# TigreGotico/phoonnx

Hardware: AMD Instinct MI355X
Metric: audio samples/sec (22.05 kHz), batch-32 256-phoneme utterances (higher is better)
Workload: dtype f32 (f16x3 split: fp32 operands as two fp16 planes, three MFMA products, fp32 accumulate)

## Files before the change

include/vitsmi.h:

```cpp
#ifndef VITSMI_H
#define VITSMI_H

#include <stddef.h>
#include <stdint.h>

#ifdef __cplusplus
extern "C" {
#endif

typedef struct vits_handle vits_handle;

enum {
    VITS_OK = 0,
    VITS_E_IO = -1,
    VITS_E_FORMAT = -2,
    VITS_E_ARG = -3,
    VITS_E_DEVICE = -4,
    VITS_E_NOMEM = -5,
    VITS_E_RANGE = -6
};

#define VITS_MAX_DIMS 4


// ... 309 lines not shown
                                 const vits_noise *noise, const vits_controls *ctl, const vits_stream_format *fmt,
                                 const vits_stream_shaping *shaping, const vits_stream_onset *onsets, int chunk_frames,
                                 vits_enc_chunk_trim_fn fn, void *user);
int vits_run_vocoder_chunked_enc_trimmed(vits_handle *h, const float *z, int B, int F, const int64_t *sid,
                                         const vits_stream_format *fmt, const vits_stream_shaping *shaping,
                                         const vits_stream_onset *onsets, int chunk_frames, vits_enc_chunk_trim_fn fn, void *user);

int vits_warp_emit_end(const vits_warp_seg *segs, int n_segs, int64_t n_in, int64_t n_out, int64_t X, int64_t *ready);
int vits_glide_emit_end(const vits_glide_seg *segs, int n_segs, int64_t n_in, int64_t n_out, int64_t X, int64_t *ready);
int64_t vits_warp_stream_cap(int64_t piece_samples, int64_t S_w);
int vits_run_chunked_glided(vits_handle *h, const int64_t *ids, const int64_t *lens, int B, int T, const int64_t *sid,
                            const vits_noise *noise, const vits_controls *ctl, const vits_contour *contour, int chunk_frames,
                            vits_chunk_fn fn, void *user);
int vits_run_chunked_enc_glided(vits_handle *h, const int64_t *ids, const int64_t *lens, int B, int T, const int64_t *sid,
                                const vits_noise *noise, const vits_controls *ctl, const vits_stream_format *fmt,
                                const vits_stream_shaping *shaping, const vits_stream_onset *onsets, const vits_contour *contour,
                                int chunk_frames, vits_enc_chunk_trim_fn fn, void *user);

enum { VITS_FIT_MET = 0, VITS_FIT_FLOOR = 1, VITS_FIT_CEIL = 2, VITS_FIT_KEPT = 3 };
typedef struct {
    const int32_t *group;
    int n_groups;
    const int64_t *target_frames;
    const int32_t *mode;
} vits_fit;
int vits_fit_plan(const float *w, const int64_t *lens, int B, int T, const vits_fit *fit, int64_t *durations, double *scale,
                  int64_t *frames, int32_t *status);
int vits_run_async_fitted(vits_handle *h, const int64_t *ids, const int64_t *lens, int B, int T, const int64_t *sid,
                          const vits_noise *noise, const vits_controls *ctl, const vits_fit *fit);
int vits_run_chunked_fitted(vits_handle *h, const int64_t *ids, const int64_t *lens, int B, int T, const int64_t *sid,
                            const vits_noise *noise, const vits_controls *ctl, const vits_fit *fit, int chunk_frames,
                            vits_chunk_fn fn, void *user);
int vits_run_chunked_enc_fitted(vits_handle *h, const int64_t *ids, const int64_t *lens, int B, int T, const int64_t *sid,
                                const vits_noise *noise, const vits_controls *ctl, const vits_stream_format *fmt,
                                const vits_stream_shaping *shaping, const vits_stream_onset *onsets, const vits_fit *fit,
                                int chunk_frames, vits_enc_chunk_trim_fn fn, void *user);
int vits_last_fit(vits_handle *h, double *scale, int64_t *frames, int32_t *status, int n);

int vits_reserve(vits_handle *h, int B, int T, int F);
int vits_get_stats(vits_handle *h, vits_stats *out);

typedef struct {
    char kernel[128];
    double flops, bytes;
    float ms;
    int stage;
    int cin, cout, k, dil, t;
} vits_launch_record;
int vits_launch_records(vits_handle *h, vits_launch_record *buf, int n);

void *vits_stream(vits_handle *h);


int vits_test_conv1d(int device_id, const float *x, int B, int Cin, int T, const float *w, const float *bias,
                     int Cout, int K, int dil, int pad_l, int flags, float slope, float *out);
int vits_bench_conv1d(int device_id, int B, int Cin, int Cout, int T, int K, int dil, int hint, int iters,
                      int cfg_override, int ck_override, float *ms_out);
int vits_test_conv_transpose1d(int device_id, const float *x, int B, int Cin, int T, const float *w,
                               const float *bias, int Cout, int K, int stride, float *out);
enum {
    VITS_CONV_PRO_LRELU = 1, VITS_CONV_PRO_MASK = 2, VITS_CONV_EPI_RELU = 4, VITS_CONV_EPI_MASK = 8, VITS_CONV_EPI_RES = 16,
    VITS_CONV_EPI_ACC = 32, VITS_CONV_EPI_DIV = 64, VITS_CONV_EPI_COUPLING = 128, VITS_CONV_EPI_WN = 256,
    VITS_CONV_EPI_WN_FIRST = 512
};
typedef struct {
    int B, Cin, T, Cout;
    int K, dil, pad_l;
    int stride;
    int hint, cfg, ck;
    int flags;
    float slope, div, oslope, oslope2;
    int wn_split;
    const float *x;
    const float *w, *bias;
    const int64_t *lens;
    const float *bias_b;
    int bias_b_stride;
    const float *res;
    int x_cstride;
    int out_cstride;
    int out_rows, out_row0;
    const float *old_out, *old_out2;
    float sentinel;
    float *out, *out2;
    int pl_rows;
    float *planes_out;
    char kernel[128];
    int cfg_used, ck_used;
} vits_test_conv_epi_args;
int vits_test_conv1d_epi(int device_id, vits_test_conv_epi_args *a);
int vits_test_wn_gate(int device_id, const float *a, int B, int H, int T, int form, float *acts);
int vits_test_cond_matvec(int device_id, const float *emb_g, int n_speakers, int gin, const int64_t *sid, int B,
                          const float *W, const float *bias, int rows, float *out);
int vits_test_conv1d_sx(int device_id, const float *x, int B, int Cin, int T, const float *w, const float *bias,
                        int Cout, int K, int dil, int pad_l, int flags, float slope, float *out);
enum { VITS_SX_EPI_RES = 1, VITS_SX_EPI_ACC = 2, VITS_SX_EPI_DIV = 4, VITS_SX_EPI_NO_RAW_STORE = 8 };
enum { VITS_SX_BF16X6 = 0, VITS_SX_F16X3 = 1, VITS_SX_F16 = 2 };
typedef struct {
    int B, Cin, T, Cout;
    int K, dil, pad_l;
    int stride;
    int precision;
    int force16, no_s16, min_cfg;
    int run_cfg;
    int flags;
    const float *x;
    const float *w, *bias;
    const float *res;
    int res_is_x;
    int res_planes;
    float res_slope;
    const float *old_out;
    const float *bias_b;
    int bias_b_stride;
    float div, oslope, oslope2, islope;
    const int64_t *lens;
    int rag_add, rag_mul;
    float sentinel;
    float *out;
    float *planes_out;
    float *res_seen;
    char kernel[128];
    int pack_cfg, run_cfg_used, rawin, s16, ck;
    float peak;
} vits_test_conv_sx_epi_args;
int vits_test_conv1d_sx_epi(int device_id, vits_test_conv_sx_epi_args *a);
int vits_test_conv1d_sx_planar(int device_id, const float *x, int B, int Cin, int T, const float *w, const float *bias,
                               int Cout, int K, int dil, int flags, const int64_t *lens, const float *old, int row_split,
                               int pl_rows, float *out, float *planes_out);
long long vits_test_set_sx_small_max(long long wgs);
int vits_test_conv1d_sx_gate(int device_id, const float *x, int B, int Cin, int T, const float *w, const float *bias,
                             const float *bias_b, int Cout, int K, int dil, int flags, float *out);
int vits_test_conv_transpose1d_sx(int device_id, const float *x, int B, int Cin, int T, const float *w,
                                  const float *bias, int Cout, int K, int stride, float *out);
int vits_bench_conv1d_sx(int device_id, int B, int Cin, int Cout, int T, int K, int dil, int dbg, int iters,
                         float *ms_out);
int vits_test_conv_pair_sx(int device_id, const float *x, int B, int C, int T, const float *w1, const float *b1,
                           const float *w2, const float *b2, int K, int dil1, int dil2, int chain, float slope, float *out,
                           float *ms_out);
enum { VITS_PAIR_EPI_ACC = 1, VITS_PAIR_EPI_DIV = 2 };
typedef struct {
    int B, C, T, K, dil1, dil2, chain;
    int flags;
    float slope, div;
    const float *x;
    const float *w1, *b1, *w2, *b2;
    const int64_t *lens;
    const float *out_init;
    float *out;
    char kernel[128];
    int BNo;
} vits_test_conv_pair_sx_epi_args;
int vits_test_conv_pair_sx_epi(int device_id, vits_test_conv_pair_sx_epi_args *a);
int vits_test_split_identity(const float *x, int64_t n, uint16_t *h1_old, uint16_t *h1_fused);
int64_t vits_test_split_identity_sweep(uint32_t first, uint64_t count, uint32_t *first_bad);
int vits_test_split_forms(int device_id, const float *x, int n, float slope, int form, uint16_t *h0, uint16_t *h1, float *pk,
                          float *rec);
enum { VITS_P16_EPI_ACC = 1, VITS_P16_EPI_DIV = 2, VITS_P16_EPI_RAW = 4, VITS_P16_EPI_PLANES = 8 };
typedef struct {
    int B, C, T, K, dil1, dil2, chain;
    int precision;
    int flags;
    float slope, div, sentinel;
    const float *x;
    const float *w1, *b1, *w2, *b2;
    const float *old_out;
    const float *x_tail;
    const int64_t *lens;
    int rag_add, rag_mul;
    float *out;
    float *planes_out;
    float *x_seen;
    float *ms_out;
    char kernel[128];
    int BN, BNo, ovl;
    float peak;
    int guard_ok;
} vits_test_conv_pair16_epi_args;
int vits_test_conv_pair16_epi(int device_id, vits_test_conv_pair16_epi_args *a);
int vits_test_attention(int device_id, const float *qkv, int B, int C, int T, int n_heads, const float *rel_k,
                        const float *rel_v, int window, const int64_t *lens, float *out);
int vits_test_attention16(int device_id, const float *qkv, int B, int C, int T, int n_heads, const float *rel_k,
                          const float *rel_v, int window, const int64_t *lens, float *out, uint16_t *out_planes, int kernel,
                          int reps, float *ms_out);
typedef struct {
    int kernel;
    const float *qkv;
    const uint16_t *qkv_planes;
    int B, C, T, n_heads, window;
    const float *rel_k, *rel_v;
    const int64_t *lens;
    int want_out;
    int want_planes;
    int ns, qt;
    int kh;
    float *out;
    uint16_t *out_planes;
    float peak;
    char kernel_name[128];
} vits_test_attention_form_args;
int vits_test_attention_form(int device_id, vits_test_attention_form_args *a);

int vits_test_resample(int device_id, const float *x, const int64_t *lens, int B, int S, int in_rate, int out_rate, float *y,
                       int64_t S_out);
int vits_test_resample_pieces(int device_id, const float *x, const int64_t *lens, int B, int S, int in_rate, int out_rate,
                              int piece_samples, float *y, int64_t S_out, int64_t *ranges, int max_ranges);
int vits_test_resample_rows(int device_id, const float *x, const int64_t *lens, int B, int S, int in_rate,
                            const int32_t *out_rates, float *y, size_t y_elems, int64_t *n_out);
int vits_test_warp(int device_id, const float *x, const int64_t *counts, int B, int S, const vits_warp_seg *segs,
                   const int32_t *seg_first , float *y, int S_w);
int vits_test_glide(int device_id, const float *x, const int64_t *counts, int B, int S, const vits_glide_seg *segs,
                    const int32_t *seg_first , float *y, int S_w);
int vits_test_warp_pieces(int device_id, const float *x, const int64_t *counts, int B, int S, const vits_warp_seg *segs,
                          const int32_t *seg_first , const int64_t *piece_bounds, int n_pieces, float *y, int S_w,
                          int64_t *ranges, int max_ranges);
int vits_test_glide_pieces(int device_id, const float *x, const int64_t *counts, int B, int S, const vits_glide_seg *segs,
                           const int32_t *seg_first , const int64_t *piece_bounds, int n_pieces, float *y, int S_w,
                           int64_t *ranges, int max_ranges);
int vits_test_warp_rate(int device_id, const float *x, const int64_t *counts, int B, int S, const vits_warp_seg *segs,
                        const int32_t *seg_first , const int32_t *in_rates, const int32_t *out_rates, int n_lo, int n_hi,
                        float *y);
int vits_test_glide_rate(int device_id, const float *x, const int64_t *counts, int B, int S, const vits_glide_seg *segs,
                         const int32_t *seg_first , const int32_t *in_rates, const int32_t *out_rates, int n_lo, int n_hi,
                        float *y);

int vits_test_warp_rate_pieces(int device_id, const float *x, const int64_t *counts, int B, int S, const vits_warp_seg *segs,
                               const int32_t *seg_first , int in_rate, int out_rate, const int64_t *piece_bounds,
                               int n_pieces, float *y, int S_w, int64_t *ranges, int max_ranges);
int vits_test_glide_rate_pieces(int device_id, const float *x, const int64_t *counts, int B, int S, const vits_glide_seg *segs,
                                const int32_t *seg_first , int in_rate, int out_rate, const int64_t *piece_bounds,
                                int n_pieces, float *y, int S_w, int64_t *ranges, int max_ranges);

int vits_test_durations(int device_id, const float *logw, const int64_t *dur, const int64_t *lens, int B, int T, float length_scale,
                        const float *rows, const float *token_rate, float *w_ceil, int32_t *cum, int32_t *y_len);
int vits_test_fit_durations(int device_id, const float *w, const int64_t *lens, int B, int T, const vits_fit *fit, float *w_ceil,
                            int32_t *cum, int32_t *y_len, double *scale, int64_t *frames, int32_t *status);
int vits_test_expand_prior(int device_id, const float *m_logs, int B, int C, int T, const int32_t *cum, const int64_t *lens,
                           const int32_t *y_len, int F, const float *noise, int64_t noise_stride, int noise_frames,
                           float noise_scale, const float *rows, const uint64_t *seeds, float *z_p);
int vits_test_fill_normal(int device_id, int64_t n, uint64_t seed, uint64_t stream_id, float *out);
int vits_test_fill_normal_rows(int device_id, int B, int channels, int T, const uint64_t *seeds, uint32_t stream, const float *rows,
                               int col, float *out);
int vits_test_post_conv(int device_id, const float *x, int B, int C, int T, const float *w, int K, float slope, const int64_t *vlen,
                        int hop, int kernel, float *out);

int vits_test_layernorm(int device_id, const float *x, const float *out_init, int B, int C, int T, const float *gamma,
                        const float *beta, const int64_t *lens, int flags, int form, int in_place, const float *dw_w,
                        const float *dw_b, int K, int dil, float *out, uint16_t *planes);
typedef struct vits_test_dds_layer {
    const float *dw_w, *dw_b;
    const float *ln1_g, *ln1_b;
    const float *pw_w, *pw_b;
    const float *ln2_g, *ln2_b;
    int32_t dil;
} vits_test_dds_layer;
int vits_test_dds(int device_id, int form, const float *x, int B, int C, int T, const int64_t *lens, int n_layers,
                  const vits_test_dds_layer *layers, int mask_out, const float *head_cond, const float *head_z, int head_ch,
                  const float *head_w, const float *head_b, const float *tail_w, const float *tail_b, int tail_rows, float *out);
int vits_test_cf_pre(int device_id, const float *z, int ch, const float *w, const float *bias, const float *cond, int B, int C, int T,
                     float *out);
int vits_test_rqs_inverse(int device_id, const float *pr, const float *z, int B, int T, const int64_t *lens, int ch0, int nb,
                          float sqrt_c, float *out);
int vits_test_ea_logw(int device_id, const float *z, int ch, float m0, float logs0, const int64_t *lens, int B, int T, float *out);

int vits_test_deliver(int device_id, const float *x, const int64_t *counts, int B, int S, const vits_segment *segs, int n_segs,
                      int n_streams, int encoding, void *dst, size_t dst_bytes, int64_t *stream_samples, int64_t *stream_offsets);

int vits_test_deliver_trimmed(int device_id, const float *x, const int64_t *counts, int B, int S, const vits_segment *segs,
                              const vits_trim *trims, int n_segs, int n_streams, int encoding, void *dst, size_t dst_bytes,
                              int64_t *stream_samples, int64_t *stream_offsets, int64_t *kept_first, int64_t *kept_count);

int vits_test_loudness_blocks(int device_id, const float *x, const int64_t *counts, const int64_t *firsts, int B, int S,
                              int sample_rate, float *e, size_t e_cap, int32_t *n_sub, int32_t *chunk);

int vits_test_deliver_leveled(int device_id, const float *x, const int64_t *counts, int B, int S, const vits_segment *segs,
                              const vits_trim *trims, const vits_level *levels, int n_segs, int n_streams, int encoding,
                              int sample_rate, void *dst, size_t dst_bytes, int64_t *stream_samples, int64_t *stream_offsets,
                              int64_t *kept_first, int64_t *kept_count, double *loudness, float *gain);

int vits_test_deliver_shaped(int device_id, const float *x, const int64_t *counts, int B, int S, const vits_segment *segs,
                             const vits_trim *trims, const vits_level *levels, const vits_shape *shapes, const vits_env_point *points,
                             int64_t n_points, int n_segs, int n_streams, int encoding, int sample_rate, void *dst, size_t dst_bytes,
                             int64_t *stream_samples, int64_t *stream_offsets, int64_t *kept_first, int64_t *kept_count,
                             double *loudness, float *gain);

int vits_test_deliver_limited(int device_id, const float *x, const int64_t *counts, int B, int S, const vits_segment *segs,
                              const vits_trim *trims, const vits_level *levels, const vits_shape *shapes, const vits_env_point *points,
                              int64_t n_points, const vits_limit *limits, int n_segs, int n_streams, int encoding, int sample_rate,
                              void *dst, size_t dst_bytes, int64_t *stream_samples, int64_t *stream_offsets, int64_t *kept_first,
                              int64_t *kept_count, double *loudness, float *gain);

int vits_test_stream_pack(int device_id, const float *x, const int64_t *counts, int B, int S, int piece_samples,
                          const vits_stream_format *fmt, void *bytes, size_t bytes_cap, int64_t *pitches, int32_t *valid,
                          float *peaks, int max_pieces);

int vits_test_stream_pack_shaped(int device_id, const float *x, const int64_t *counts, int B, int S, int piece_samples,
                                 const vits_stream_format *fmt, const vits_stream_shaping *shaping, void *bytes, size_t bytes_cap,
                                 int64_t *pitches, int32_t *valid, float *peaks, int64_t *firsts, int64_t *ns, int max_pieces);

int vits_test_stream_pack_trimmed(int device_id, const float *x, const int64_t *counts, int B, int S, int piece_samples,
                                  const vits_stream_format *fmt, const vits_stream_shaping *shaping, const vits_stream_onset *onsets,
                                  void *bytes, size_t bytes_cap, int64_t *pitches, int32_t *valid, int32_t *skip, float *peaks,
                                  int64_t *firsts, int64_t *ns, int32_t *start, int max_pieces);

#ifdef __cplusplus
}
// ... 3 lines not shown
```

phoonnx_amd/_ffi.py:

```python
import ctypes as C
import os

import numpy as np

from . import audio_encoding

_HERE = os.path.dirname(os.path.abspath(__file__))
_LIB = None

VITS_MAX_DIMS = 4


class VitsNoise(C.Structure):
    _fields_ = [("noise_dp", C.c_void_p), ("noise_z", C.c_void_p), ("noise_z_stride", C.c_int64),
                ("seed", C.c_uint64)]


class VitsOutput(C.Structure):
    _fields_ = [("data", C.POINTER(C.c_float)), ("dims", C.c_int64 * 4), ("y_lengths", C.POINTER(C.c_int64))]


class VitsStats(C.Structure):
    _fields_ = [("conv_flops", C.c_double), ("conv_bytes", C.c_double), ("dec_flops", C.c_double),
                ("dec_bytes", C.c_double), ("flow_flops", C.c_double), ("enc_flops", C.c_double),
                ("dp_flops", C.c_double), ("conv_ms", C.c_float), ("dec_ms", C.c_float), ("flow_ms", C.c_float),
                ("enc_ms", C.c_float), ("dp_ms", C.c_float), ("total_ms", C.c_float), ("conv_launches", C.c_int),
                ("total_launches", C.c_int), ("sx_flops", C.c_double), ("sx_ms", C.c_float), ("sx_launches", C.c_int),
                ("f16_peak_max", C.c_float), ("f16_peak_min", C.c_float), ("f16_tracked", C.c_int),
                ("f16_saturated", C.c_int), ("sx_bytes", C.c_double)]


class VitsLaunchRecord(C.Structure):
    _fields_ = [("kernel", C.c_char * 128), ("flops", C.c_double), ("bytes", C.c_double), ("ms", C.c_float),
                ("stage", C.c_int), ("cin", C.c_int), ("cout", C.c_int), ("k", C.c_int), ("dil", C.c_int), ("t", C.c_int)]


class VitsTestConvEpiArgs(C.Structure):
    _fields_ = [(n, C.c_int) for n in ("B", "Cin", "T", "Cout", "K", "dil", "pad_l", "stride", "hint", "cfg", "ck", "flags")] + \
               [(n, C.c_float) for n in ("slope", "div", "oslope", "oslope2")] + [("wn_split", C.c_int)] + \
               [(n, C.c_void_p) for n in ("x", "w", "bias", "lens", "bias_b")] + [("bias_b_stride", C.c_int), ("res", C.c_void_p)] + \
               [(n, C.c_int) for n in ("x_cstride", "out_cstride", "out_rows", "out_row0")] + \
               [("old_out", C.c_void_p), ("old_out2", C.c_void_p), ("sentinel", C.c_float), ("out", C.c_void_p), ("out2", C.c_void_p),
                ("pl_rows", C.c_int), ("planes_out", C.c_void_p), ("kernel", C.c_char * 128), ("cfg_used", C.c_int), ("ck_used", C.c_int)]


class VitsTestConvSxEpiArgs(C.Structure):
    _fields_ = [(n, C.c_int) for n in ("B", "Cin", "T", "Cout", "K", "dil", "pad_l", "stride", "precision", "force16", "no_s16",
                                       "min_cfg", "run_cfg", "flags")] + \
               [(n, C.c_void_p) for n in ("x", "w", "bias", "res")] + \
               [("res_is_x", C.c_int), ("res_planes", C.c_int), ("res_slope", C.c_float), ("old_out", C.c_void_p),
                ("bias_b", C.c_void_p), ("bias_b_stride", C.c_int)] + \
               [(n, C.c_float) for n in ("div", "oslope", "oslope2", "islope")] + \
               [("lens", C.c_void_p), ("rag_add", C.c_int), ("rag_mul", C.c_int), ("sentinel", C.c_float), ("out", C.c_void_p),
                ("planes_out", C.c_void_p), ("res_seen", C.c_void_p), ("kernel", C.c_char * 128)] + \
               [(n, C.c_int) for n in ("pack_cfg", "run_cfg_used", "rawin", "s16", "ck")] + [("peak", C.c_float)]


class VitsTestConvPair16EpiArgs(C.Structure):
    _fields_ = [(n, C.c_int) for n in ("B", "C", "T", "K", "dil1", "dil2", "chain", "precision", "flags")] + \
               [(n, C.c_float) for n in ("slope", "div", "sentinel")] + \
               [(n, C.c_void_p) for n in ("x", "w1", "b1", "w2", "b2", "old_out", "x_tail", "lens")] + \
               [("rag_add", C.c_int), ("rag_mul", C.c_int)] + \
               [(n, C.c_void_p) for n in ("out", "planes_out", "x_seen", "ms_out")] + [("kernel", C.c_char * 128)] + \
               [(n, C.c_int) for n in ("BN", "BNo", "ovl")] + [("peak", C.c_float), ("guard_ok", C.c_int)]


class VitsTestConvPairSxEpiArgs(C.Structure):
    _fields_ = [(n, C.c_int) for n in ("B", "C", "T", "K", "dil1", "dil2", "chain", "flags")] + \
               [(n, C.c_float) for n in ("slope", "div")] + \
               [(n, C.c_void_p) for n in ("x", "w1", "b1", "w2", "b2", "lens", "out_init", "out")] + \
               [("kernel", C.c_char * 128), ("BNo", C.c_int)]


class VitsTestAttentionFormArgs(C.Structure):
    _fields_ = [("kernel", C.c_int), ("qkv", C.c_void_p), ("qkv_planes", C.c_void_p)] + \
               [(n, C.c_int) for n in ("B", "C", "T", "n_heads", "window")] + \
               [(n, C.c_void_p) for n in ("rel_k", "rel_v", "lens")] + \
               [(n, C.c_int) for n in ("want_out", "want_planes", "ns", "qt", "kh")] + \
               [("out", C.c_void_p), ("out_planes", C.c_void_p), ("peak", C.c_float), ("kernel_name", C.c_char * 128)]


class VitsOpenOptions(C.Structure):
    _fields_ = [("device_id", C.c_int), ("gen_precision", C.c_char_p), ("arena_dev", C.c_void_p),
                ("arena_bytes", C.c_size_t), ("host_only", C.c_int), ("layout_only", C.c_int)]


class VitsControls(C.Structure):
    _fields_ = [("scales_rows", C.c_void_p), ("seeds", C.c_void_p), ("durations", C.c_void_p), ("token_rate", C.c_void_p)]


class VitsFit(C.Structure):
    _fields_ = [("group", C.c_void_p), ("n_groups", C.c_int), ("target_frames", C.c_void_p), ("mode", C.c_void_p)]


VITS_FIT_MET, VITS_FIT_FLOOR, VITS_FIT_CEIL, VITS_FIT_KEPT = 0, 1, 2, 3


class VitsWarpSeg(C.Structure):
    _fields_ = [("n0", C.c_int64), ("pos0", C.c_int64), ("k", C.c_int64), ("step", C.c_int32), ("c", C.c_int32),
                ("half_taps", C.c_int32), ("pad_", C.c_int32)]


class VitsIntonation(C.Structure):
    _fields_ = [("token_semitones", C.c_void_p), ("compensate", C.c_int)]


class VitsGlideSeg(C.Structure):
    _fields_ = [("n0", C.c_int64), ("pos0", C.c_int64), ("k", C.c_int64), ("step0", C.c_int32), ("step1", C.c_int32),
                ("pad_", C.c_int32 * 2)]


class VitsContour(C.Structure):
    _fields_ = [("token_semitones", C.c_void_p), ("token_semitones_end", C.c_void_p), ("compensate", C.c_int)]


class VitsSegment(C.Structure):
    _fields_ = [("row", C.c_int32), ("stream", C.c_int32), ("lead_samples", C.c_int64), ("normalize", C.c_int32),
                ("volume", C.c_float)]


class VitsTrim(C.Structure):
    _fields_ = [("mode", C.c_int32), ("threshold", C.c_float), ("keep_lead", C.c_int32), ("keep_tail", C.c_int32),
                ("tail_samples", C.c_int64)]


class VitsTestDdsLayer(C.Structure):
    _fields_ = [("dw_w", C.c_void_p), ("dw_b", C.c_void_p), ("ln1_g", C.c_void_p), ("ln1_b", C.c_void_p), ("pw_w", C.c_void_p),
                ("pw_b", C.c_void_p), ("ln2_g", C.c_void_p), ("ln2_b", C.c_void_p), ("dil", C.c_int32)]


class VitsLevel(C.Structure):
    _fields_ = [("mode", C.c_int32), ("target_lufs", C.c_float), ("max_gain_db", C.c_float), ("peak_ceiling", C.c_float)]


class VitsEnvPoint(C.Structure):
    _fields_ = [("pos", C.c_int32), ("gain", C.c_float)]


class VitsShape(C.Structure):
    _fields_ = [("fade_in", C.c_int32), ("fade_out", C.c_int32), ("curve", C.c_int32), ("n_points", C.c_int32),
                ("first_point", C.c_int64)]


class VitsLimit(C.Structure):
    _fields_ = [("mode", C.c_int32), ("ceiling", C.c_float), ("lookahead", C.c_int32), ("reserved", C.c_int32)]


class VitsStreamFormat(C.Structure):
    _fields_ = [("encoding", C.c_int32), ("ref_peak", C.c_void_p), ("volume", C.c_void_p)]


class VitsStreamShaping(C.Structure):
    pass


STREAM_PLAN_FN = C.CFUNCTYPE(C.c_int, C.c_void_p, C.c_int, C.c_int, C.POINTER(C.c_int64), C.POINTER(C.c_int64), C.POINTER(VitsStreamShaping))

VitsStreamShaping._fields_ = [("shapes", C.c_void_p), ("points", C.c_void_p), ("n_points", C.c_int64), ("ceiling", C.c_void_p),
                              ("lookahead", C.c_int32), ("reserved", C.c_int32), ("plan", STREAM_PLAN_FN), ("plan_user", C.c_void_p)]


class VitsStreamOnset(C.Structure):
    _fields_ = [("mode", C.c_int32), ("threshold", C.c_float), ("keep_lead", C.c_int32), ("reserved", C.c_int32)]


ENCODINGS = {name: (code, audio_encoding.DTYPES[name]) for code, name in enumerate(audio_encoding.ENCODINGS)}


CHUNK_FN = C.CFUNCTYPE(C.c_int, C.c_void_p, C.POINTER(C.c_float), C.c_int, C.c_int64, C.c_int64, C.c_int64)

ENC_CHUNK_FN = C.CFUNCTYPE(C.c_int, C.c_void_p, C.c_void_p, C.c_int, C.c_int64, C.c_int64, C.c_int64, C.POINTER(C.c_int32),
                           C.POINTER(C.c_float), C.c_int64)

ENC_CHUNK_TRIM_FN = C.CFUNCTYPE(C.c_int, C.c_void_p, C.c_void_p, C.c_int, C.c_int64, C.c_int64, C.c_int64, C.POINTER(C.c_int32),
                                C.POINTER(C.c_int32), C.POINTER(C.c_float), C.c_int64)

VITS_E_RANGE = -6


EXPORTS = [
    "vits_open", "vits_open_with_arena", "vits_open_host", "vits_open_layout", "vits_open_opts", "vits_close",
    "vits_run_chunked", "vits_run_vocoder_chunked", "vits_last_error", "vits_num_inputs",
    "vits_input_name", "vits_meta", "vits_hparam", "vits_arena_bytes", "vits_arena_host", "vits_arena_device",
    "vits_run", "vits_free_output", "vits_run_device", "vits_sync", "vits_last_y_lengths", "vits_last_pcm16", "vits_run_vocoder",
    "vits_tap",
    "vits_set_timing", "vits_set_tails", "vits_reserve", "vits_get_stats", "vits_stream", "vits_test_conv1d", "vits_test_conv_transpose1d",
    "vits_test_attention", "vits_test_attention16", "vits_bench_conv1d", "vits_test_conv1d_sx", "vits_test_conv1d_sx_planar", "vits_test_conv1d_sx_gate", "vits_test_set_sx_small_max",
    "vits_test_conv_transpose1d_sx",
    "vits_bench_conv1d_sx", "vits_test_conv_pair_sx", "vits_fetch_output", "vits_run_async", "vits_host_alloc", "vits_host_free",
    "vits_launch_records", "vits_run_async_rows", "vits_run_device_rows", "vits_run_chunked_rows",
    "vits_run_async_ctl", "vits_run_chunked_ctl", "vits_last_durations",
    "vits_set_output_rate", "vits_last_sample_counts", "vits_resample_plan", "vits_test_resample", "vits_test_resample_pieces",
    "vits_set_output_rates", "vits_last_sample_rates", "vits_test_resample_rows",
    "vits_run_async_warped", "vits_last_token_spans", "vits_warp_token", "vits_warp_plan", "vits_test_warp",
    "vits_run_async_glided", "vits_glide_token", "vits_glide_cutoff", "vits_glide_plan", "vits_test_glide",
    "vits_warp_emit_end", "vits_glide_emit_end", "vits_warp_stream_cap", "vits_run_chunked_glided", "vits_run_chunked_enc_glided",
    "vits_test_warp_pieces", "vits_test_glide_pieces",
    "vits_set_pitch_at_rate", "vits_warp_token_rate", "vits_warp_plan_rate", "vits_glide_plan_rate", "vits_glide_cutoff_rate", "vits_glide_pos_rate",
    "vits_rate_identity_spans", "vits_test_warp_rate", "vits_test_glide_rate",
    "vits_warp_emit_end_rate", "vits_glide_emit_end_rate", "vits_identity_emit_end_rate", "vits_warp_stream_cap_rate",
    "vits_test_warp_rate_pieces", "vits_test_glide_rate_pieces",
    "vits_fit_plan", "vits_run_async_fitted", "vits_run_chunked_fitted", "vits_run_chunked_enc_fitted", "vits_last_fit",
    "vits_test_fit_durations",
    "vits_test_durations", "vits_test_expand_prior", "vits_test_fill_normal", "vits_test_fill_normal_rows", "vits_test_post_conv",
    "vits_delivery_plan", "vits_deliver", "vits_test_deliver",
    "vits_trim_range", "vits_delivery_plan_trimmed", "vits_deliver_trimmed", "vits_test_deliver_trimmed",
    "vits_loudness_filter", "vits_loudness_gate", "vits_level_gain", "vits_delivery_plan_leveled", "vits_deliver_leveled",
    "vits_test_loudness_blocks", "vits_test_deliver_leveled",
    "vits_shape_check", "vits_shape_gain", "vits_deliver_shaped", "vits_test_deliver_shaped",
    "vits_limit_check", "vits_limit_gains", "vits_deliver_limited", "vits_test_deliver_limited",
    "vits_run_chunked_enc", "vits_run_vocoder_chunked_enc", "vits_test_stream_pack",
    "vits_stream_shaping_check", "vits_stream_emit_range", "vits_run_chunked_enc_shaped", "vits_run_vocoder_chunked_enc_shaped",
    "vits_test_stream_pack_shaped",
    "vits_stream_onset_check", "vits_stream_onset_start", "vits_run_chunked_enc_trimmed", "vits_run_vocoder_chunked_enc_trimmed",
    "vits_test_stream_pack_trimmed",
    "vits_test_layernorm", "vits_test_dds", "vits_test_cf_pre", "vits_test_rqs_inverse", "vits_test_ea_logw",
    "vits_test_conv1d_epi", "vits_test_wn_gate", "vits_test_cond_matvec", "vits_test_conv1d_sx_epi",
    "vits_test_conv_pair16_epi", "vits_test_attention_form", "vits_test_conv_pair_sx_epi", "vits_test_split_forms", "vits_test_split_identity", "vits_test_split_identity_sweep",
]


G2P_EXPORTS = ["g2p_open", "g2p_close", "g2p_last_error", "g2p_hparam", "g2p_num_outputs", "g2p_output_name", "g2p_bucket",
               "g2p_run", "g2p_generate", "g2p_generate_batch", "g2p_test_forced_steps", "g2p_test_linear", "g2p_test_step",
               "g2p_test_attention", "g2p_test_rmsnorm", "g2p_test_argmax"]


def lib_path():
    return os.environ.get("VITSMI_LIB") or os.path.join(_HERE, "libvitsmi.so")


def load():
    global _LIB
    if _LIB is not None:
        return _LIB
    path = lib_path()
    if not os.environ.get("VITSMI_LIB"):
        from . import build as _build
        if _build.stale():
            try:
                _build.build()
            except Exception as e:
                raise RuntimeError(f"{path} is missing or was not built from the sources in this tree (source_sha "
                                   f"{_build.source_sha()} vs recorded {_build.read_build_info().get('source_sha')}) "
                                   f"and cannot be rebuilt here: {e}") from e
    lib = C.CDLL(path)
    vp, i64p, f32p = C.c_void_p, C.POINTER(C.c_int64), C.POINTER(C.c_float)
    lib.vits_open.argtypes = [C.c_char_p, C.c_int, C.POINTER(vp)]
    lib.vits_open_with_arena.argtypes = [C.c_char_p, C.c_int, vp, C.c_size_t, C.POINTER(vp)]
    lib.vits_open_host.argtypes = [C.c_char_p, C.POINTER(vp)]
    lib.vits_open_layout.argtypes = [C.c_char_p, C.POINTER(vp)]
    lib.vits_open_opts.argtypes = [C.c_char_p, C.POINTER(VitsOpenOptions), C.POINTER(vp)]
    lib.vits_run_chunked.argtypes = [vp, vp, vp, C.c_int, C.c_int, vp, vp, C.POINTER(VitsNoise), C.c_int, CHUNK_FN, vp]
    lib.vits_run_vocoder_chunked.argtypes = [vp, vp, C.c_int, C.c_int, vp, C.c_int, CHUNK_FN, vp]
    lib.vits_close.argtypes = [vp]
    lib.vits_close.restype = None
    lib.vits_last_error.argtypes = [vp]
    lib.vits_last_error.restype = C.c_char_p
    lib.vits_num_inputs.argtypes = [vp]
    lib.vits_input_name.argtypes = [vp, C.c_int]
    lib.vits_input_name.restype = C.c_char_p
    lib.vits_meta.argtypes = [vp, C.c_char_p, C.c_char_p, C.c_size_t]
    lib.vits_hparam.argtypes = [vp, C.c_char_p, i64p]
    lib.vits_arena_bytes.argtypes = [vp]
    lib.vits_arena_bytes.restype = C.c_size_t
    lib.vits_arena_host.argtypes = [vp]
    lib.vits_arena_host.restype = vp
    lib.vits_arena_device.argtypes = [vp]
    lib.vits_arena_device.restype = vp
    run_args = [vp, vp, vp, C.c_int, C.c_int, vp, vp, C.POINTER(VitsNoise), C.POINTER(VitsOutput)]
    lib.vits_run.argtypes = run_args
    lib.vits_run_device.argtypes = run_args
    lib.vits_run_async.argtypes = run_args[:-1]
    lib.vits_run_async_rows.argtypes = run_args[:-1] + [vp]
    lib.vits_run_device_rows.argtypes = run_args[:-1] + [vp, C.POINTER(VitsOutput)]
    lib.vits_run_chunked_rows.argtypes = [vp, vp, vp, C.c_int, C.c_int, vp, vp, C.POINTER(VitsNoise), vp, C.c_int, CHUNK_FN, vp]
    lib.vits_run_async_ctl.argtypes = [vp, vp, vp, C.c_int, C.c_int, vp, C.POINTER(VitsNoise), C.POINTER(VitsControls)]
    lib.vits_run_chunked_ctl.argtypes = [vp, vp, vp, C.c_int, C.c_int, vp, C.POINTER(VitsNoise), C.POINTER(VitsControls),
                                         C.c_int, CHUNK_FN, vp]
    lib.vits_run_chunked_enc.argtypes = [vp, vp, vp, C.c_int, C.c_int, vp, C.POINTER(VitsNoise), C.POINTER(VitsControls),
                                         C.POINTER(VitsStreamFormat), C.c_int, ENC_CHUNK_FN, vp]
    lib.vits_run_vocoder_chunked_enc.argtypes = [vp, vp, C.c_int, C.c_int, vp, C.POINTER(VitsStreamFormat), C.c_int, ENC_CHUNK_FN, vp]
    lib.vits_stream_shaping_check.argtypes = [C.POINTER(VitsStreamShaping), C.POINTER(VitsStreamFormat), C.c_int]
    lib.vits_stream_emit_range.argtypes = [C.c_int64, C.c_int64, C.c_int, C.c_int64, C.c_int, i64p, i64p]
    lib.vits_run_chunked_enc_shaped.argtypes = [vp, vp, vp, C.c_int, C.c_int, vp, C.POINTER(VitsNoise), C.POINTER(VitsControls),
                                                C.POINTER(VitsStreamFormat), C.POINTER(VitsStreamShaping), C.c_int, ENC_CHUNK_FN, vp]
    lib.vits_run_vocoder_chunked_enc_shaped.argtypes = [vp, vp, C.c_int, C.c_int, vp, C.POINTER(VitsStreamFormat),
                                                        C.POINTER(VitsStreamShaping), C.c_int, ENC_CHUNK_FN, vp]
    lib.vits_test_stream_pack_shaped.argtypes = [C.c_int, vp, vp, C.c_int, C.c_int, C.c_int, C.POINTER(VitsStreamFormat),
                                                 C.POINTER(VitsStreamShaping), vp, C.c_size_t, vp, vp, vp, vp, vp, C.c_int]
    lib.vits_stream_onset_check.argtypes = [C.POINTER(VitsStreamOnset), C.POINTER(VitsStreamFormat), C.c_int]
    lib.vits_stream_onset_start.argtypes = [C.c_int64, C.c_int64, C.c_int64, i64p]
    lib.vits_run_chunked_enc_trimmed.argtypes = [vp, vp, vp, C.c_int, C.c_int, vp, C.POINTER(VitsNoise), C.POINTER(VitsControls),
                                                 C.POINTER(VitsStreamFormat), C.POINTER(VitsStreamShaping), C.POINTER(VitsStreamOnset),
                                                 C.c_int, ENC_CHUNK_TRIM_FN, vp]
    lib.vits_run_vocoder_chunked_enc_trimmed.argtypes = [vp, vp, C.c_int, C.c_int, vp, C.POINTER(VitsStreamFormat),
                                                         C.POINTER(VitsStreamShaping), C.POINTER(VitsStreamOnset), C.c_int,
                                                         ENC_CHUNK_TRIM_FN, vp]
    lib.vits_test_stream_pack_trimmed.argtypes = [C.c_int, vp, vp, C.c_int, C.c_int, C.c_int, C.POINTER(VitsStreamFormat),
                                                  C.POINTER(VitsStreamShaping), C.POINTER(VitsStreamOnset), vp, C.c_size_t, vp, vp, vp, vp,
                                                  vp, vp, vp, C.c_int]
    lib.vits_test_stream_pack.argtypes = [C.c_int, vp, vp, C.c_int, C.c_int, C.c_int, C.POINTER(VitsStreamFormat), vp, C.c_size_t,
                                          vp, vp, vp, C.c_int]
    lib.vits_last_durations.argtypes = [vp, i64p, C.c_size_t]
    lib.vits_set_output_rate.argtypes = [vp, C.c_int, C.c_int]
    lib.vits_last_sample_counts.argtypes = [vp, i64p, C.c_int]
    lib.vits_resample_plan.argtypes = [C.c_int, C.c_int, i64p, i64p, i64p, vp, C.c_size_t]
    lib.vits_test_resample.argtypes = [C.c_int, vp, vp, C.c_int, C.c_int, C.c_int, C.c_int, vp, C.c_int64]
    lib.vits_test_resample_pieces.argtypes = [C.c_int, vp, vp, C.c_int, C.c_int, C.c_int, C.c_int, C.c_int, vp, C.c_int64, vp, C.c_int]
    lib.vits_set_output_rates.argtypes = [vp, C.c_int, vp, C.c_int]
    lib.vits_last_sample_rates.argtypes = [vp, vp, C.c_int]
    lib.vits_test_resample_rows.argtypes = [C.c_int, vp, vp, C.c_int, C.c_int, C.c_int, vp, vp, C.c_size_t, vp]
    lib.vits_run_async_warped.argtypes = [vp, vp, vp, C.c_int, C.c_int, vp, C.POINTER(VitsNoise), C.POINTER(VitsControls),
                                          C.POINTER(VitsIntonation)]
    lib.vits_last_token_spans.argtypes = [vp, i64p, C.c_size_t]
    lib.vits_warp_token.argtypes = [C.c_float, i64p, i64p, C.POINTER(C.c_int32)]
    lib.vits_warp_plan.argtypes = [vp, vp, C.c_int, C.c_int, vp, vp, i64p]
    lib.vits_test_warp.argtypes = [C.c_int, vp, vp, C.c_int, C.c_int, vp, vp, vp, C.c_int]
    lib.vits_run_async_glided.argtypes = [vp, vp, vp, C.c_int, C.c_int, vp, C.POINTER(VitsNoise), C.POINTER(VitsControls),
                                          C.POINTER(VitsContour)]
    lib.vits_glide_token.argtypes = [C.c_float, C.c_float, i64p, i64p, C.POINTER(C.c_float)]
    lib.vits_glide_cutoff.argtypes = [C.c_int64, i64p, C.POINTER(C.c_int32)]
    lib.vits_glide_plan.argtypes = [vp, vp, vp, C.c_int, C.c_int, vp, vp, i64p]
    lib.vits_test_glide.argtypes = [C.c_int, vp, vp, C.c_int, C.c_int, vp, vp, vp, C.c_int]
    for name in ("vits_warp_emit_end", "vits_glide_emit_end"):
        getattr(lib, name).argtypes = [vp, C.c_int, C.c_int64, C.c_int64, C.c_int64, i64p]
    lib.vits_warp_stream_cap.argtypes = [C.c_int64, C.c_int64]
    lib.vits_warp_stream_cap.restype = C.c_int64
    lib.vits_run_chunked_glided.argtypes = [vp, vp, vp, C.c_int, C.c_int, vp, C.POINTER(VitsNoise), C.POINTER(VitsControls),
                                            C.POINTER(VitsContour), C.c_int, CHUNK_FN, vp]
    lib.vits_run_chunked_enc_glided.argtypes = [vp, vp, vp, C.c_int, C.c_int, vp, C.POINTER(VitsNoise), C.POINTER(VitsControls),
                                                C.POINTER(VitsStreamFormat), C.POINTER(VitsStreamShaping), C.POINTER(VitsStreamOnset),
                                                C.POINTER(VitsContour), C.c_int, ENC_CHUNK_TRIM_FN, vp]
    for name in ("vits_test_warp_pieces", "vits_test_glide_pieces"):
        getattr(lib, name).argtypes = [C.c_int, vp, vp, C.c_int, C.c_int, vp, vp, vp, C.c_int, vp, C.c_int, vp, C.c_int]
    lib.vits_set_pitch_at_rate.argtypes = [vp, C.c_int]
    lib.vits_warp_token_rate.argtypes = [C.c_float, C.c_int64, C.c_int64, i64p, i64p, C.POINTER(C.c_int32)]
    lib.vits_warp_plan_rate.argtypes = [vp, vp, C.c_int, C.c_int, C.c_int64, C.c_int64, vp, vp, i64p]
    lib.vits_glide_plan_rate.argtypes = [vp, vp, vp, C.c_int, C.c_int, C.c_int64, C.c_int64, vp, vp, i64p]
    lib.vits_glide_cutoff_rate.argtypes = [C.c_int64, i64p, C.POINTER(C.c_int32)]
    lib.vits_glide_pos_rate.argtypes = [vp, C.c_int64, i64p, i64p]
    lib.vits_rate_identity_spans.argtypes = [vp, C.c_int, C.c_int, C.c_int64, C.c_int64, C.c_int64, vp, i64p]
    for name in ("vits_warp_emit_end_rate", "vits_glide_emit_end_rate"):
        getattr(lib, name).argtypes = [vp, C.c_int, C.c_int64, C.c_int64, C.c_int64, C.c_int, i64p]
    lib.vits_identity_emit_end_rate.argtypes = [C.c_int64, C.c_int64, C.c_int64, C.c_int64, C.c_int64, i64p]
    lib.vits_warp_stream_cap_rate.argtypes = [C.c_int64, C.c_int64, C.c_int64, C.c_int]
    lib.vits_warp_stream_cap_rate.restype = C.c_int64
    for name in ("vits_test_warp_rate_pieces", "vits_test_glide_rate_pieces"):
        getattr(lib, name).argtypes = [C.c_int, vp, vp, C.c_int, C.c_int, vp, vp, C.c_int, C.c_int, vp, C.c_int, vp, C.c_int, vp, C.c_int]
    for name in ("vits_test_warp_rate", "vits_test_glide_rate"):
        getattr(lib, name).argtypes = [C.c_int, vp, vp, C.c_int, C.c_int, vp, vp, vp, vp, C.c_int, C.c_int, vp]
    lib.vits_fit_plan.argtypes = [vp, vp, C.c_int, C.c_int, C.POINTER(VitsFit), vp, vp, vp, vp]
    lib.vits_run_async_fitted.argtypes = [vp, vp, vp, C.c_int, C.c_int, vp, C.POINTER(VitsNoise), C.POINTER(VitsControls),
                                          C.POINTER(VitsFit)]
    lib.vits_run_chunked_fitted.argtypes = [vp, vp, vp, C.c_int, C.c_int, vp, C.POINTER(VitsNoise), C.POINTER(VitsControls),
                                            C.POINTER(VitsFit), C.c_int, CHUNK_FN, vp]
    lib.vits_run_chunked_enc_fitted.argtypes = [vp, vp, vp, C.c_int, C.c_int, vp, C.POINTER(VitsNoise), C.POINTER(VitsControls),
                                                C.POINTER(VitsStreamFormat), C.POINTER(VitsStreamShaping), C.POINTER(VitsStreamOnset),
                                                C.POINTER(VitsFit), C.c_int, ENC_CHUNK_TRIM_FN, vp]
    lib.vits_last_fit.argtypes = [vp, vp, vp, vp, C.c_int]
    lib.vits_test_fit_durations.argtypes = [C.c_int, vp, vp, C.c_int, C.c_int, C.POINTER(VitsFit), vp, vp, vp, vp, vp, vp]
    lib.vits_test_durations.argtypes = [C.c_int, vp, vp, vp, C.c_int, C.c_int, C.c_float, vp, vp, vp, vp, vp]
    lib.vits_test_expand_prior.argtypes = [C.c_int, vp, C.c_int, C.c_int, C.c_int, vp, vp, vp, C.c_int, vp, C.c_int64, C.c_int,
                                           C.c_float, vp, vp, vp]
    lib.vits_test_fill_normal.argtypes = [C.c_int, C.c_int64, C.c_uint64, C.c_uint64, vp]
    lib.vits_test_fill_normal_rows.argtypes = [C.c_int, C.c_int, C.c_int, C.c_int, vp, C.c_uint32, vp, C.c_int, vp]
    lib.vits_test_post_conv.argtypes = [C.c_int, vp, C.c_int, C.c_int, C.c_int, vp, C.c_int, C.c_float, vp, C.c_int, C.c_int, vp]
    lib.vits_test_layernorm.argtypes = [C.c_int, vp, vp, C.c_int, C.c_int, C.c_int, vp, vp, vp, C.c_int, C.c_int, C.c_int, vp, vp,
                                        C.c_int, C.c_int, vp, vp]
    lib.vits_test_dds.argtypes = [C.c_int, C.c_int, vp, C.c_int, C.c_int, C.c_int, vp, C.c_int, C.POINTER(VitsTestDdsLayer), C.c_int,
                                  vp, vp, C.c_int, vp, vp, vp, vp, C.c_int, vp]
    lib.vits_test_cf_pre.argtypes = [C.c_int, vp, C.c_int, vp, vp, vp, C.c_int, C.c_int, C.c_int, vp]
    lib.vits_test_rqs_inverse.argtypes = [C.c_int, vp, vp, C.c_int, C.c_int, vp, C.c_int, C.c_int, C.c_float, vp]
    lib.vits_test_ea_logw.argtypes = [C.c_int, vp, C.c_int, C.c_float, C.c_float, vp, C.c_int, C.c_int, vp]
    lib.vits_delivery_plan.argtypes = [vp, C.c_int, vp, C.c_int, C.c_int, C.c_int, vp, vp, i64p]
    lib.vits_deliver.argtypes = [vp, vp, C.c_int, C.c_int, C.c_int, vp, C.c_size_t, vp, vp]
    lib.vits_test_deliver.argtypes = [C.c_int, vp, vp, C.c_int, C.c_int, vp, C.c_int, C.c_int, C.c_int, vp, C.c_size_t, vp, vp]
    lib.vits_trim_range.argtypes = [C.c_int64, C.c_int64, C.c_int64, C.POINTER(VitsTrim), i64p, i64p]
    lib.vits_delivery_plan_trimmed.argtypes = [vp, C.c_int, vp, vp, C.c_int, C.c_int, C.c_int, vp, vp, i64p]
    lib.vits_deliver_trimmed.argtypes = [vp, vp, vp, C.c_int, C.c_int, C.c_int, vp, C.c_size_t, vp, vp, vp, vp]
    lib.vits_test_deliver_trimmed.argtypes = [C.c_int, vp, vp, C.c_int, C.c_int, vp, vp, C.c_int, C.c_int, C.c_int, vp, C.c_size_t,
                                              vp, vp, vp, vp]
    lib.vits_loudness_filter.argtypes = [C.c_int, vp, vp]
    lib.vits_loudness_gate.argtypes = [vp, vp, C.c_int, C.c_int32, vp, vp, vp, vp]
    lib.vits_level_gain.argtypes = [C.c_double, C.c_float, C.POINTER(VitsLevel), C.POINTER(C.c_float)]
    lib.vits_delivery_plan_leveled.argtypes = [vp, C.c_int, vp, vp, vp, C.c_int, C.c_int, C.c_int, C.c_int, vp, vp, i64p]
    lib.vits_deliver_leveled.argtypes = [vp, vp, vp, vp, C.c_int, C.c_int, C.c_int, C.c_int, vp, C.c_size_t, vp, vp, vp, vp, vp, vp]
    lib.vits_test_loudness_blocks.argtypes = [C.c_int, vp, vp, vp, C.c_int, C.c_int, C.c_int, vp, C.c_size_t, vp, vp]
    lib.vits_test_deliver_leveled.argtypes = [C.c_int, vp, vp, C.c_int, C.c_int, vp, vp, vp, C.c_int, C.c_int, C.c_int, C.c_int, vp,
                                              C.c_size_t, vp, vp, vp, vp, vp, vp]
    lib.vits_shape_check.argtypes = [vp, C.c_int, vp, C.c_int64]
    lib.vits_shape_gain.argtypes = [C.POINTER(VitsShape), vp, C.c_int64, C.c_int64, C.c_int64, C.POINTER(C.c_float)]
    lib.vits_deliver_shaped.argtypes = [vp, vp, vp, vp, vp, vp, C.c_int64, C.c_int, C.c_int, C.c_int, C.c_int, vp, C.c_size_t, vp, vp, vp,
                                        vp, vp, vp]
    lib.vits_test_deliver_shaped.argtypes = [C.c_int, vp, vp, C.c_int, C.c_int, vp, vp, vp, vp, vp, C.c_int64, C.c_int, C.c_int, C.c_int,
                                             C.c_int, vp, C.c_size_t, vp, vp, vp, vp, vp, vp]
    lib.vits_limit_check.argtypes = [vp, vp, C.c_int]
    lib.vits_limit_gains.argtypes = [vp, C.c_int64, C.POINTER(VitsLimit), vp]
    lib.vits_deliver_limited.argtypes = [vp, vp, vp, vp, vp, vp, C.c_int64, vp, C.c_int, C.c_int, C.c_int, C.c_int, vp, C.c_size_t, vp,
                                         vp, vp, vp, vp, vp]
    lib.vits_test_deliver_limited.argtypes = [C.c_int, vp, vp, C.c_int, C.c_int, vp, vp, vp, vp, vp, C.c_int64, vp, C.c_int, C.c_int,
                                              C.c_int, C.c_int, vp, C.c_size_t, vp, vp, vp, vp, vp, vp]
    lib.vits_free_output.argtypes = [vp, C.POINTER(VitsOutput)]
    lib.vits_free_output.restype = None
    lib.vits_sync.argtypes = [vp]
    lib.vits_last_y_lengths.argtypes = [vp, i64p, C.c_int]
    lib.vits_last_pcm16.argtypes = [vp, C.c_int, C.c_float, vp, C.c_size_t]
    lib.vits_run_vocoder.argtypes = [vp, vp, C.c_int, C.c_int, vp, C.POINTER(VitsOutput)]
    lib.vits_tap.argtypes = [vp, C.c_char_p, vp, C.c_size_t, i64p]
    lib.vits_set_timing.argtypes = [vp, C.c_int]
    lib.vits_set_tails.argtypes = [vp, C.c_int]
    lib.vits_reserve.argtypes = [vp, C.c_int, C.c_int, C.c_int]
    lib.vits_get_stats.argtypes = [vp, C.POINTER(VitsStats)]
    lib.vits_stream.argtypes = [vp]
    lib.vits_stream.restype = vp
    lib.vits_fetch_output.argtypes = [vp, vp, C.c_size_t, C.c_size_t]
    lib.vits_host_alloc.argtypes = [C.c_size_t]
    lib.vits_host_alloc.restype = vp
    lib.vits_host_free.argtypes = [vp]
    lib.vits_host_free.restype = None
    lib.vits_launch_records.argtypes = [vp, C.POINTER(VitsLaunchRecord), C.c_int]
    lib.vits_test_conv1d.argtypes = [C.c_int, vp, C.c_int, C.c_int, C.c_int, vp, vp, C.c_int, C.c_int, C.c_int,
                                     C.c_int, C.c_int, C.c_float, vp]
    lib.vits_test_conv_transpose1d.argtypes = [C.c_int, vp, C.c_int, C.c_int, C.c_int, vp, vp, C.c_int, C.c_int,
                                               C.c_int, vp]
    lib.vits_test_attention.argtypes = [C.c_int, vp, C.c_int, C.c_int, C.c_int, C.c_int, vp, vp, C.c_int, vp, vp]
    lib.vits_test_attention16.argtypes = [C.c_int, vp, C.c_int, C.c_int, C.c_int, C.c_int, vp, vp, C.c_int, vp, vp, vp,
                                          C.c_int, C.c_int, f32p]
    lib.vits_bench_conv1d.argtypes = [C.c_int] * 11 + [f32p]
    lib.vits_test_conv1d_sx.argtypes = lib.vits_test_conv1d.argtypes
    lib.vits_test_conv_transpose1d_sx.argtypes = lib.vits_test_conv_transpose1d.argtypes
    lib.vits_test_conv1d_sx_planar.argtypes = [C.c_int, vp, C.c_int, C.c_int, C.c_int, vp, vp, C.c_int, C.c_int, C.c_int, C.c_int,
                                               vp, vp, C.c_int, C.c_int, vp, vp]
    lib.vits_test_set_sx_small_max.argtypes = [C.c_longlong]
    lib.vits_test_set_sx_small_max.restype = C.c_longlong
    lib.vits_test_conv1d_sx_gate.argtypes = [C.c_int, vp, C.c_int, C.c_int, C.c_int, vp, vp, vp, C.c_int, C.c_int, C.c_int, C.c_int, vp]
    lib.vits_bench_conv1d_sx.argtypes = [C.c_int] * 9 + [f32p]
    lib.vits_test_conv1d_epi.argtypes = [C.c_int, C.POINTER(VitsTestConvEpiArgs)]
    lib.vits_test_conv1d_sx_epi.argtypes = [C.c_int, C.POINTER(VitsTestConvSxEpiArgs)]
    lib.vits_test_conv_pair16_epi.argtypes = [C.c_int, C.POINTER(VitsTestConvPair16EpiArgs)]
    lib.vits_test_conv_pair_sx_epi.argtypes = [C.c_int, C.POINTER(VitsTestConvPairSxEpiArgs)]
    lib.vits_test_split_identity.argtypes = [vp, C.c_int64, vp, vp]
    lib.vits_test_split_identity_sweep.argtypes = [C.c_uint32, C.c_uint64, C.POINTER(C.c_uint32)]
    lib.vits_test_split_identity_sweep.restype = C.c_int64
    lib.vits_test_split_forms.argtypes = [C.c_int, vp, C.c_int, C.c_float, C.c_int, vp, vp, vp, vp]
    lib.vits_test_attention_form.argtypes = [C.c_int, C.POINTER(VitsTestAttentionFormArgs)]
    lib.vits_test_wn_gate.argtypes = [C.c_int, vp, C.c_int, C.c_int, C.c_int, C.c_int, vp]
    lib.vits_test_cond_matvec.argtypes = [C.c_int, vp, C.c_int, C.c_int, vp, C.c_int, vp, vp, C.c_int, vp]
    lib.vits_test_conv_pair_sx.argtypes = [C.c_int, vp, C.c_int, C.c_int, C.c_int, vp, vp, vp, vp, C.c_int, C.c_int,
                                           C.c_int, C.c_int, C.c_float, vp, f32p]
    lib.g2p_open.argtypes = [C.c_char_p, C.c_int, C.POINTER(vp)]
    lib.g2p_close.argtypes = [vp]
    lib.g2p_close.restype = None
    lib.g2p_last_error.argtypes = [vp]
    lib.g2p_last_error.restype = C.c_char_p
    lib.g2p_hparam.argtypes = [vp, C.c_char_p, i64p]
    lib.g2p_num_outputs.argtypes = [vp]
    lib.g2p_output_name.argtypes = [vp, C.c_int]
    lib.g2p_output_name.restype = C.c_char_p
    lib.g2p_bucket.argtypes = [vp, C.c_int, C.c_int]
    lib.g2p_run.argtypes = [vp, vp, C.c_int, vp, vp, C.c_int, vp]
    lib.g2p_generate.argtypes = [vp, vp, C.c_int, C.c_int, C.c_int64, C.c_int64, vp, C.POINTER(C.c_int)]
    lib.g2p_generate_batch.argtypes = [vp, vp, vp, C.c_int, C.c_int, C.c_int64, C.c_int64, vp, vp]
    lib.g2p_test_forced_steps.argtypes = [vp, vp, vp, C.c_int, vp, C.c_int, vp]
    lib.g2p_test_linear.argtypes = [C.c_int, C.c_int, vp, vp, C.c_int, vp, C.c_int, C.c_int, vp, C.c_int64, C.c_int64, C.c_int, vp]
    lib.g2p_test_step.argtypes = [C.c_int, C.c_int, C.c_int, vp, vp, vp, C.c_int, vp, vp, C.c_int, C.c_float, C.c_float, vp, vp]
    lib.g2p_test_attention.argtypes = [C.c_int, vp, vp, C.c_int, C.c_int, vp, vp, C.c_int64, C.c_int, C.c_int64, vp, C.c_int, vp,
                                       C.c_int, C.c_int, C.c_int, C.c_int, vp, C.c_int, C.c_int, C.c_int]
    lib.g2p_test_rmsnorm.argtypes = [C.c_int, vp, vp, vp, C.c_int, C.c_int, C.c_int, C.c_int, C.c_float]
    lib.g2p_test_argmax.argtypes = [C.c_int, vp, C.c_int, C.c_int, C.c_int, C.c_int64, C.c_int, vp, vp, C.c_int64, C.c_int]
    _LIB = lib
    return lib


def ptr(a):
    return None if a is None else a.ctypes.data_as(C.c_void_p)


def last_error(h=None):
    return load().vits_last_error(h).decode("utf-8", "replace")
```

phoonnx_amd/csrc/conv_sx_pair.hip.hpp:

```cpp
#pragma once
#include <cstdlib>
#include "conv_geom.hpp"
#include "conv_sx_engine.hip.hpp"

namespace vitsmi {

struct SxPairArgs {
    const float *xr;
    float islope, mslope;
    int T;
    const u32x4 *wp1, *wp2;
    const float *bias1, *bias2;
    float wscale1, wscale2;
    float *out_raw;
    const float *zeros;
    int C, nchunks;
    int K1, dil1, pad1;
    int K2, dil2, pad2;
    int LW1;
    unsigned x_bytes;
    int LW2;
    unsigned y_chunk_bytes;
    int BNo, NT, B;
    int flags;
    float div;
    unsigned *peak;
    struct Chain {
        const u32x4 *wp1, *wp2;
        const float *bias1, *bias2;
        float wscale1, wscale2;
        int K1, dil1, K2, dil2;
        int xoff, yoff;
    } ch[3];
    int nchain;
    unsigned a_ring;
    unsigned bias_off;
    unsigned long long *prof;
    SxRagged rag;
    int xgs = 0;
};

#ifndef SX_PAIR_PROF
#define SX_PAIR_PROF 0
#endif
#ifndef SX_PAIR_SHARED_A
#define SX_PAIR_SHARED_A 0
#endif
#ifndef SX_PAIR_ALIAS
#define SX_PAIR_ALIAS 0
#endif
#ifndef SX_PAIR_DEPTH32
#define SX_PAIR_DEPTH32 2
#endif
#ifndef SX_PAIR_DEPTH64
#define SX_PAIR_DEPTH64 2
#endif
#ifndef SX_PAIR_EARLY_ACC
#define SX_PAIR_EARLY_ACC 0
#endif
#ifndef SX_PAIR_WGS32
#define SX_PAIR_WGS32 3
#endif
#ifndef SX_PAIR_EARLY32
#define SX_PAIR_EARLY32 1
#endif
#ifndef SX_PAIR_ST_SC1
#define SX_PAIR_ST_SC1 0
#endif
#ifndef SX_PAIR_INTERIOR
#define SX_PAIR_INTERIOR 1
#endif
#ifndef SX_PAIR_ONE_READ64
#define SX_PAIR_ONE_READ64 1
#endif
#ifndef SX_PAIR_ONE_READ32
#define SX_PAIR_ONE_READ32 1
#endif
template <int MW, int NW, int WM, int WN, int EPI, bool CHAIN, int NCH, bool INTR>
__device__ __forceinline__ void conv_sx_pair_body(const SxPairArgs &a, const int b, const int t0, const int TV, float &pk) {
    constexpr int BN = NW * WN * 32, NH = NW / 2;
    static_assert(NCH == 1 || (CHAIN && NW == 2 && (EPI & EPI_ACC) == 0), "fused chains: 32 channels, no external running sum");
    constexpr bool ONE_READ = NW == 4 ? SX_PAIR_ONE_READ64 != 0 : SX_PAIR_ONE_READ32 != 0;
    constexpr bool EARLY = ONE_READ || (NW == 2 && SX_PAIR_EARLY32);
    constexpr int DEPTH = NW == 2 ? SX_PAIR_DEPTH32 : SX_PAIR_DEPTH64;
    static_assert(DEPTH >= 2 && DEPTH <= 6, "wait_a covers up to five younger sets");
    constexpr bool ACC = (EPI & EPI_ACC) != 0 && SX_PAIR_EARLY_ACC;
    static_assert(!(ONE_READ && ACC), "the running sum is not pulled into the single-read prologue");
    static_assert(WM * WN == 4 && MW == 1 && BN == 256, "one block row per wave, 256 columns");
    constexpr int NPW = 2, STEPBYTES = WM * MW * NPW * 1024;
    constexpr int MAXCH = WM * 2;
    extern __shared__ __attribute__((aligned(16))) unsigned char lds_sx[];
    const int tid = threadIdx.x, lane = tid & 63;
    const int wave = __builtin_amdgcn_readfirstlane(tid >> 6);
    const int wm = wave / WN, wn = wave % WN;
    const int l31 = lane & 31, hi = lane >> 5;
    const int t1 = t0 - a.pad2;
    const int T = a.T, LW = a.LW1;
    const uint32_t lds0 = (uint32_t)(uintptr_t)lds_sx;
    const uint32_t XB = a.x_bytes;
    const char *wbase1 = reinterpret_cast<const char *>(a.wp1) + wm * (MW * NPW * 1024);
    const char *wbase2 = reinterpret_cast<const char *>(a.wp2) + wm * (MW * NPW * 1024);
    const float *xrb = a.xr + (int64_t)b * a.C * T;

    struct ASet {
        u32x4 fa[2];
    };
    const uint32_t voff0 = (uint32_t)lane * 16u;
    auto load_a = [&](ASet &f, const char *wb, int step) {
        const char *sb = wb + (int64_t)step * STEPBYTES;
        f.fa[0] = global_read128<0>(voff0, sb);
        f.fa[1] = global_read128<1024>(voff0, sb);
    };

    f32x4 pre[NW / 2][2][4], ad[EARLY && ACC ? NW / 2 : 1][2][4];
    auto load_res = [&](const float *base, f32x4 (*dst)[2][4]) {
        static_for<NW / 2>([&](auto R) {
            constexpr int rr = decltype(R)::value;
#pragma unroll
            for (int j = 0; j < 2; j++) {
                const int row0 = wm * 32;
                const int t = t1 + (wn * NW + rr * 2 + j) * 32 + l31;
                const int tl = t < 0 ? 0 : (t < T ? t : T - 1);
#pragma unroll
                for (int q = 0; q < 4; q++) {
                    if constexpr (INTR && EARLY) {
                        const char *rowb = reinterpret_cast<const char *>(base + (int64_t)((row0 >> 3) + q) * T * 8);
                        dst[rr][j][q] = __builtin_bit_cast(f32x4, global_read128<0>(((uint32_t)t * 8u + 4u * (uint32_t)hi) * 4u, rowb));
                        continue;
                    }
                    const float *p = base + ((int64_t)((row0 >> 3) + q) * T + tl) * 8 + 4 * hi;
                    if constexpr (EARLY) dst[rr][j][q] = __builtin_bit_cast(f32x4, global_read128_v<0>(p));
                    else dst[rr][j][q] = *reinterpret_cast<const f32x4 *>(p);
                }
            }
        });
    };
    auto load_pre = [&]() { load_res(xrb, pre); };

#if SX_PAIR_PROF
    auto stamp = [&]() {
        unsigned long long t;
        __builtin_amdgcn_sched_barrier(0);
        asm volatile("s_memtime %0\n\ts_waitcnt lgkmcnt(0)" : "=s"(t)::"memory");
        __builtin_amdgcn_sched_barrier(0);
        return t;
    };
    unsigned long long tp[8];
    tp[0] = stamp();
#endif
    if constexpr (NW == 2 && WM == 1 && NCH == 1 && SX_PAIR_SHARED_A != 0)
        for (int g = 0; g < 3; g++)
            if (g < ((a.nchunks * a.K1) >> 1)) {
                const int sub = wave >> 1, pl = wave & 1;
                lds_dma<16>(wbase1 + (int64_t)(2 * g + sub) * STEPBYTES + pl * 1024 + lane * 16,
                            reinterpret_cast<float *>(lds_sx + a.a_ring + (unsigned)((g * 2 + sub) * 2048 + pl * 1024)));
            }
    constexpr bool BIAS_LDS = NCH == 1;
    if constexpr (BIAS_LDS) {
        if (wave == 0) {
            constexpr int CC = WM * 32;
            const int k = lane - (lane >= CC / 4 ? CC / 4 : 0);
            const float *bp = lane < CC / 4 ? a.bias1 : a.bias2;
            const void *src = (bp && lane < CC / 2) ? static_cast<const void *>(bp + 4 * k) : static_cast<const void *>(a.zeros + 4 * (lane & 31));
            lds_dma<16>(src, reinterpret_cast<float *>(lds_sx + a.bias_off));
        }
    }
    auto bias_from_lds = [&](int conv, f32x4 (&bq)[4]) __attribute__((always_inline)) {
        u32x4 t4[4];
#pragma unroll
        for (int q = 0; q < 4; q++)
            asm volatile("ds_read_b128 %0, %1" : "=v"(t4[q]) : "v"(lds0 + a.bias_off + (uint32_t)(conv * (WM * 32) + wm * 32 + 8 * q + 4 * hi) * 4u) : "memory");
        asm volatile("s_waitcnt lgkmcnt(0)" ::: "memory");
        __builtin_amdgcn_sched_barrier(0);
#pragma unroll
        for (int q = 0; q < 4; q++) bq[q] = __builtin_bit_cast(f32x4, t4[q]);
    };
    constexpr int NXC = 3;
    if constexpr (ONE_READ) {
        constexpr int NXH = MAXCH, NG = 2 * MAXCH;
        const int HW = LW - 256, pad1 = a.pad1;
        const int nhc = HW * NG, nxh = (nhc + 255) >> 8;
        u32x4 hst[NXH][2];
        bool hin[NXH], hok[NXH];
        uint32_t hlds[NXH];
        const float *hp[NXH];
#pragma unroll
        for (int it = 0; it < NXH; it++) {
            const int h = it * 256 + tid;
            hin[it] = h < nhc;
            const int g = hin[it] ? h / HW : 0;
            const int c = hin[it] ? h - g * HW : 0;
            const int col = c < pad1 ? c : c + 256;
            const int t = t1 - pad1 + col;
            hok[it] = hin[it] && (INTR || (t >= 0 && t < TV));
            hp[it] = xrb + (hok[it] ? ((int64_t)g * T + t) * 8 : (int64_t)0);
            hlds[it] = lds0 + (uint32_t)(g >> 1) * XB + (uint32_t)((g & 1) * LW + col) * 16u;
        }
        static_for<NXH>([&](auto I) {
            constexpr int it = decltype(I)::value;
            if (it < nxh) {
                hst[it][0] = global_read128_v<0>(hp[it]);
                hst[it][1] = global_read128_v<16>(hp[it]);
            }
        });
        load_pre();
        const float isl = a.islope;
        static_for<NW>([&](auto N) {
            constexpr int n = decltype(N)::value;
            asm volatile("s_waitcnt vmcnt(%0)" ::"n"(4 * (NW - 1 - n)) : "memory");
            __builtin_amdgcn_sched_barrier(0);
#if SX_PAIR_PROF
            if constexpr (n == 0) tp[1] = stamp();
#endif
            if constexpr (n == 0) {
                static_for<NXH>([&](auto I) {
                    constexpr int it = decltype(I)::value;
                    if (it < nxh && hin[it]) {
                        float v[8];
#pragma unroll
                        for (int e = 0; e < 8; e++) {
                            const float x = (INTR || hok[it]) ? __uint_as_float(hst[it][e >> 2][e & 3]) : 0.f;
                            v[e] = lrelu_max(x, isl);
                        }
                        unsigned p0[4], p1[4];
#pragma unroll
                        for (int e = 0; e < 4; e++) sx_pair_split(v[2 * e], v[2 * e + 1], p0[e], p1[e], pk);
                        ds_write128(hlds[it], u32x4{p0[0], p0[1], p0[2], p0[3]});
                        ds_write128(hlds[it] + (uint32_t)(2 * LW) * 16u, u32x4{p1[0], p1[1], p1[2], p1[3]});
                    }
                });
            }
            const int col = (wn * NW + n) * 32 + l31;
            const int t = t1 + col;
            const bool ok = INTR || (t >= 0 && t < TV);
#pragma unroll
            for (int q = 0; q < 4; q++) {
                float v[4];
#pragma unroll
                for (int e = 0; e < 4; e++) {
                    const float x = ok ? pre[n / 2][n % 2][q][e] : 0.f;
                    v[e] = lrelu_max(x, isl);
                }
                unsigned wa[2], wb[2];
                sx_pair_split(v[0], v[1], wa[0], wa[1], pk);
                sx_pair_split(v[2], v[3], wb[0], wb[1], pk);
                const int g = 4 * wm + q;
                const uint32_t cell = lds0 + (uint32_t)(g >> 1) * XB + (uint32_t)((g & 1) * LW + pad1 + col) * 16u + 8u * hi;
                asm volatile("ds_write_b64 %0, %1" ::"v"(cell), "v"(u32x2{wa[0], wb[0]}) : "memory");
                asm volatile("ds_write_b64 %0, %1" ::"v"(cell + (uint32_t)(2 * LW) * 16u), "v"(u32x2{wa[1], wb[1]}) : "memory");
            }
            asm volatile("" : "+v"(pk));
        });
    } else {
        u32x4 xst[MAXCH][NXC][2];
        const int nxc = (2 * LW + 255) >> 8;
        uint32_t xroff[NXC];
        bool xrok[NXC];
        int xkh[NXC], xcol[NXC];
#pragma unroll
        for (int it = 0; it < NXC; it++) {
            const int i = it * 256 + tid;
            const int kh = (i >= LW ? 1 : 0) + (i >= 2 * LW ? 1 : 0);
            const int col = i - kh * LW;
            const int t = t1 - a.pad1 + col;
            xkh[it] = kh;
            xcol[it] = col;
            xrok[it] = it < nxc && kh < 2 && (INTR || (t >= 0 && t < TV));
            xroff[it] = xrok[it] ? (uint32_t)(((int64_t)kh * T + t) * 32) : 0u;
        }
        static_for<MAXCH>([&](auto CH) {
            constexpr int ch = decltype(CH)::value;
            const float *cbase = xrb + (int64_t)(2 * ch) * T * 8;
            static_for<NXC>([&](auto I) {
                constexpr int it = decltype(I)::value;
                if (it < nxc) {
                    xst[ch][it][0] = global_read128_x<0>(xroff[it], cbase);
                    xst[ch][it][1] = global_read128_x<16>(xroff[it], cbase);
                }
            });
        });
        if constexpr (EARLY) {
            load_pre();
            if constexpr (ACC) {
                load_res(a.out_raw + (int64_t)b * a.C * T, ad);
                asm volatile("s_waitcnt vmcnt(16)" ::: "memory");
            } else
                asm volatile("s_waitcnt vmcnt(8)" ::: "memory");
        } else
            asm volatile("s_waitcnt vmcnt(0)" ::: "memory");
#if SX_PAIR_PROF
        tp[1] = stamp();
#endif
        const float isl = a.islope;
        static_for<MAXCH>([&](auto CH) {
            constexpr int ch = decltype(CH)::value;
            static_for<NXC>([&](auto I) {
                constexpr int it = decltype(I)::value;
                if (it < nxc && xkh[it] < 2) {
                    float v[8];
#pragma unroll
                    for (int e = 0; e < 8; e++) {
                        const float x = xrok[it] ? __uint_as_float(xst[ch][it][e >> 2][e & 3]) : 0.f;
                        v[e] = lrelu_max(x, isl);
                    }
                    unsigned p0[4], p1[4];
#pragma unroll
                    for (int e = 0; e < 4; e++) sx_pair_split(v[2 * e], v[2 * e + 1], p0[e], p1[e], pk);
                    const uint32_t ad = lds0 + (uint32_t)ch * XB + (uint32_t)(xkh[it] * LW + xcol[it]) * 16u;
                    ds_write128(ad, u32x4{p0[0], p0[1], p0[2], p0[3]});
                    ds_write128(ad + (uint32_t)(2 * LW) * 16u, u32x4{p1[0], p1[1], p1[2], p1[3]});
                }
            });
        });
    }

    f32x16 acc[NW];
    auto zero_acc = [&]() {
#pragma unroll
        for (int n = 0; n < NW; n++)
#pragma unroll
            for (int r = 0; r < 16; r++) acc[n][r] = 0.f;
    };
    zero_acc();
    u32x4 fb[NW][2];
    auto load_b_half = [&](auto H, uint32_t rows, uint32_t pstride) {
        constexpr int h = decltype(H)::value;
        static_for<NH>([&](auto N) {
            constexpr int n = h * NH + decltype(N)::value;
            fb[n][0] = ds_read128<n * 512>(rows);
            fb[n][1] = ds_read128<n * 512>(rows + pstride);
        });
    };
    auto mma_half = [&](const ASet &f, auto H) {
        constexpr int h = decltype(H)::value;
#pragma unroll
        for (int c = 0; c < 3; c++)
#pragma unroll
            for (int n = h * NH; n < (h + 1) * NH; n++) {
                const f16x8 ga = c == 0 ? __builtin_bit_cast(f16x8, f.fa[1])
                                        : (c == 1 ? __builtin_bit_cast(f16x8, f.fa[0]) * (_Float16)0.00048828125f
                                                  : __builtin_bit_cast(f16x8, f.fa[0]));
                const f16x8 gb = __builtin_bit_cast(f16x8, fb[n][c == 1 ? 1 : 0]);
                acc[n] = __builtin_amdgcn_mfma_f32_32x32x16_f16(ga, gb, acc[n], 0, 0, 0);
            }
    };
    auto wait_lds_older_half = [&]() {
        if constexpr (NH * 2 == 2) asm volatile("s_waitcnt lgkmcnt(2)" ::: "memory");
        else asm volatile("s_waitcnt lgkmcnt(4)" ::: "memory");
    };
    const std::integral_constant<int, 0> H0{};
    const std::integral_constant<int, 1> H1{};

    auto wait_a = [&](int younger) {
        switch (younger) {
            case 0: asm volatile("s_waitcnt vmcnt(0)" ::: "memory"); break;
            case 1: asm volatile("s_waitcnt vmcnt(2)" ::: "memory"); break;
            case 2: asm volatile("s_waitcnt vmcnt(4)" ::: "memory"); break;
            case 3: asm volatile("s_waitcnt vmcnt(6)" ::: "memory"); break;
            case 4: asm volatile("s_waitcnt vmcnt(8)" ::: "memory"); break;
            default: asm volatile("s_waitcnt vmcnt(10)" ::: "memory"); break;
        }
    };
    auto run_conv = [&](ASet(&fs)[DEPTH + 1], const char *wb, int K, int dil, uint32_t rows0, uint32_t chunk_bytes,
                        uint32_t pstride) {
        constexpr int NS = DEPTH + 1;
        const int S = a.nchunks * K;
        int chunk = 0, tap = 0;
        static_for<DEPTH - 1>([&](auto I) {
            constexpr int i = decltype(I)::value + 1;
            if (i < S) load_a(fs[i], wb, i);
        });
        load_b_half(H0, rows0, pstride);
        load_b_half(H1, rows0, pstride);
        auto step = [&](ASet &fc, ASet &fload, int s) {
            const int left = S - 1 - s;
            wait_a(left < DEPTH - 1 ? left : DEPTH - 1);
            __builtin_amdgcn_sched_barrier(0);
            if (s + DEPTH < S && !SX_NOA) load_a(fload, wb, s + DEPTH);
            int ntap = tap + 1, nchunk = chunk;
            if (ntap == K) {
                ntap = 0;
                nchunk++;
            }
            const bool more = s + 1 < S;
            const uint32_t next = rows0 + (uint32_t)nchunk * chunk_bytes + (uint32_t)(ntap * dil) * 16u;
            __builtin_amdgcn_sched_barrier(0);
            wait_lds_older_half();
            __builtin_amdgcn_sched_barrier(0);
            mma_half(fc, H0);
            __builtin_amdgcn_sched_barrier(0);
            if (more) {
                load_b_half(H0, next, pstride);
                wait_lds_older_half();
            } else
                asm volatile("s_waitcnt lgkmcnt(0)" ::: "memory");
            __builtin_amdgcn_sched_barrier(0);
            mma_half(fc, H1);
            __builtin_amdgcn_sched_barrier(0);
            if (more) load_b_half(H1, next, pstride);
            __builtin_amdgcn_sched_barrier(0);
            tap = ntap;
            chunk = nchunk;
        };
        int s = 0;
        for (; s + NS <= S; s += NS)
            static_for<NS>([&](auto I) {
                constexpr int i = decltype(I)::value;
                step(fs[i], fs[(i + DEPTH) % NS], s + i);
            });
        __builtin_amdgcn_sched_barrier(0);
        asm volatile("s_waitcnt lgkmcnt(0)" ::: "memory");
        __builtin_amdgcn_sched_barrier(0);
        static_for<NS - 1>([&](auto I) {
            constexpr int i = decltype(I)::value;
            if (s + i < S) step(fs[i], fs[(i + DEPTH) % NS], s + i);
        });
    };

    constexpr bool SHA = NW == 2 && WM == 1 && NCH == 1 && SX_PAIR_SHARED_A != 0;
    constexpr int RG = 3;
    auto sha_dma = [&](const char *wb, int g) {
        const int sub = wave >> 1, pl = wave & 1;
        const char *src = wb + (int64_t)(2 * g + sub) * STEPBYTES + pl * 1024 + lane * 16;
        lds_dma<16>(src, reinterpret_cast<float *>(lds_sx + a.a_ring + (unsigned)(((g % RG) * 2 + sub) * 2048 + pl * 1024)));
    };
    auto sha_prefetch = [&](const char *wb, int K) {
        const int NG = (a.nchunks * K) >> 1;
#pragma unroll
        for (int g = 0; g < RG; g++)
            if (g < NG) sha_dma(wb, g);
    };
    auto wait_vm_le = [&](int n) {
        switch (n) {
            case 0: asm volatile("s_waitcnt vmcnt(0)" ::: "memory"); break;
            case 1: asm volatile("s_waitcnt vmcnt(1)" ::: "memory"); break;
            default: asm volatile("s_waitcnt vmcnt(2)" ::: "memory"); break;
        }
    };
    auto run_conv_sha = [&](ASet &fa0, ASet &fa1, const char *wb, int K, int dil, uint32_t rows0, uint32_t chunk_bytes,
                            uint32_t pstride) {
        const int S = a.nchunks * K, NG = S >> 1;
        const uint32_t alds = lds0 + a.a_ring + (uint32_t)lane * 16u;
        auto read_a = [&](ASet &f, int st) {
            const uint32_t ad = alds + (uint32_t)((((st >> 1) % RG) * 2 + (st & 1)) * 2048);
            f.fa[0] = ds_read128<0>(ad);
            f.fa[1] = ds_read128<1024>(ad);
        };
        int chunk = 0, tap = 0;
        wait_vm_le((NG < RG ? NG : RG) - 1);
        __builtin_amdgcn_s_barrier();
        __builtin_amdgcn_sched_barrier(0);
        read_a(fa0, 0);
        load_b_half(H0, rows0, pstride);
        load_b_half(H1, rows0, pstride);
        auto step = [&](ASet &fc, ASet &fload, int st, bool boundary) {
            int ntap = tap + 1, nchunk = chunk;
            if (ntap == K) {
                ntap = 0;
                nchunk++;
            }
            const bool more = st + 1 < S;
            const uint32_t next = rows0 + (uint32_t)nchunk * chunk_bytes + (uint32_t)(ntap * dil) * 16u;
            __builtin_amdgcn_sched_barrier(0);
            wait_lds_older_half();
            __builtin_amdgcn_sched_barrier(0);
            mma_half(fc, H0);
            __builtin_amdgcn_sched_barrier(0);
            if (more) {
                if (boundary && NG > RG) {
                    const int g = st >> 1;
                    const int last = g + RG - 1 < NG - 1 ? g + RG - 1 : NG - 1;
                    wait_vm_le(last - (g + 1));
                    __builtin_amdgcn_s_barrier();
                    __builtin_amdgcn_sched_barrier(0);
                    if (g + RG < NG) sha_dma(wb, g + RG);
                }
                read_a(fload, st + 1);
                load_b_half(H0, next, pstride);
                asm volatile("s_waitcnt lgkmcnt(4)" ::: "memory");
            } else
                asm volatile("s_waitcnt lgkmcnt(0)" ::: "memory");
            __builtin_amdgcn_sched_barrier(0);
            mma_half(fc, H1);
            __builtin_amdgcn_sched_barrier(0);
            if (more) load_b_half(H1, next, pstride);
            __builtin_amdgcn_sched_barrier(0);
            tap = ntap;
            chunk = nchunk;
        };
        for (int g = 0; g < NG; g++) {
            step(fa0, fa1, 2 * g, false);
            step(fa1, fa0, 2 * g + 1, true);
        }
    };

    struct ChainPar {
        const char *wb1, *wb2;
        const float *bias1, *bias2;
        float ws1, ws2;
        int K1, dil1, K2, dil2;
        uint32_t xoff, yoff;
    };
    auto chain_par = [&](int ci) {
        ChainPar c;
        if constexpr (NCH == 1) {
            c = ChainPar{wbase1, wbase2, a.bias1, a.bias2, a.wscale1, a.wscale2, a.K1, a.dil1, a.K2, a.dil2, 0u, 0u};
        } else {
            const auto &h = a.ch[ci];
            c = ChainPar{reinterpret_cast<const char *>(h.wp1) + wm * (MW * NPW * 1024),
                         reinterpret_cast<const char *>(h.wp2) + wm * (MW * NPW * 1024),
                         h.bias1, h.bias2, h.wscale1, h.wscale2, h.K1, h.dil1, h.K2, h.dil2, (uint32_t)h.xoff, (uint32_t)h.yoff};
        }
        return c;
    };
    static_assert(NCH == 1 || EARLY, "fused chains keep x in registers from the prologue on");
    const uint32_t ylds = NCH > 1 ? lds0 + (uint32_t)a.nchunks * XB : lds0;
    f32x4 xkeep[NCH > 1 ? NW / 2 : 1][2][4], tot[NCH > 1 ? NW / 2 : 1][2][4];
#if SX_PAIR_ALIAS
    ASet f1s[DEPTH + 1];
    ASet(&f2s)[DEPTH + 1] = f1s;
#else
    ASet f1s[DEPTH + 1], f2s[DEPTH + 1];
#endif
#pragma unroll 1
    for (int ci = 0; ci < NCH; ci++) {
    const ChainPar cp = chain_par(ci);
    if constexpr (NCH > 1) {
        if (ci > 0) {
#pragma unroll
            for (int rr = 0; rr < NW / 2; rr++)
#pragma unroll
                for (int j = 0; j < 2; j++)
#pragma unroll
                    for (int q = 0; q < 4; q++) pre[rr][j][q] = xkeep[rr][j][q];
            zero_acc();
        }
    }
    if constexpr (!SHA) load_a(f1s[0], cp.wb1, 0);
    if (ci == 0) {
        asm volatile("s_waitcnt lgkmcnt(0)" ::: "memory");
#if SX_PAIR_PROF
        tp[2] = stamp();
#endif
        __builtin_amdgcn_s_barrier();
#if SX_PAIR_PROF
        tp[3] = stamp();
#endif
    }
    __builtin_amdgcn_sched_barrier(0);
    if constexpr (SHA)
        run_conv_sha(f1s[0], f1s[1], cp.wb1, cp.K1, cp.dil1, lds0 + (uint32_t)(hi * LW + wn * (NW * 32) + l31 + (int)cp.xoff) * 16u,
                     XB, (uint32_t)(2 * LW) * 16u);
    else
        run_conv(f1s, cp.wb1, cp.K1, cp.dil1, lds0 + (uint32_t)(hi * LW + wn * (NW * 32) + l31 + (int)cp.xoff) * 16u, XB,
                 (uint32_t)(2 * LW) * 16u);

#if SX_PAIR_PROF
    tp[4] = stamp();
#endif
    if constexpr (CHAIN && !EARLY) load_pre();

    if constexpr (!SHA) load_a(f2s[0], cp.wb2, 0);
    asm volatile("s_waitcnt lgkmcnt(0)" ::: "memory");
    __builtin_amdgcn_s_barrier();
    __builtin_amdgcn_sched_barrier(0);
    if constexpr (SHA) sha_prefetch(cp.wb2, cp.K2);
    {
        const float wsc = cp.ws1, msl = a.mslope;
        const float *biasp = cp.bias1 ? cp.bias1 : a.zeros;
        const int b_on = cp.bias1 ? 1 : 0;
        const uint32_t YC = a.y_chunk_bytes, LW2 = (uint32_t)a.LW2;
        const int row0 = wm * 32;
        f32x4 bq[4];
        if constexpr (BIAS_LDS) bias_from_lds(0, bq);
        else {
#pragma unroll
            for (int q = 0; q < 4; q++) bq[q] = *reinterpret_cast<const f32x4 *>(biasp + (row0 + 8 * q + 4 * hi) * b_on);
        }
#pragma unroll
        for (int n = 0; n < NW; n++) {
            const int col = (wn * NW + n) * 32 + l31;
            const int t = t1 + col;
            const bool live = INTR || (t >= 0 && t < TV);
#pragma unroll
            for (int q = 0; q < 4; q++) {
                float o[4];
#pragma unroll
                for (int e = 0; e < 4; e++) {
                    float v = __builtin_fmaf(acc[n][4 * q + e], wsc, bq[q][e]);
                    if constexpr (CHAIN) {
                        if constexpr (NCH > 1) {
                            if (ci == 0) xkeep[n / 2][n % 2][q][e] = pre[n / 2][n % 2][q][e];
                        }
                        v += pre[n / 2][n % 2][q][e];
                        pre[n / 2][n % 2][q][e] = v;
                    }
                    o[e] = live ? fmaxf(v, v * msl) : 0.f;
                }
                unsigned wa[2], wb[2];
                sx_pair_split(o[0], o[1], wa[0], wa[1], pk);
                sx_pair_split(o[2], o[3], wb[0], wb[1], pk);
                const int g = 4 * wm + q;
                const uint32_t cell = ylds + (uint32_t)(g >> 1) * YC + ((uint32_t)(g & 1) * LW2 + (uint32_t)(col + a.pad2)) * 16u + 8u * hi;
                asm volatile("ds_write_b64 %0, %1" ::"v"(cell), "v"(u32x2{wa[0], wb[0]}) : "memory");
                asm volatile("ds_write_b64 %0, %1" ::"v"(cell + 2u * LW2 * 16u), "v"(u32x2{wa[1], wb[1]}) : "memory");
            }
            asm volatile("" : "+v"(pk));
        }
    }
    zero_acc();
    asm volatile("s_waitcnt lgkmcnt(0)" ::: "memory");
    __builtin_amdgcn_s_barrier();
    __builtin_amdgcn_sched_barrier(0);
#if SX_PAIR_PROF
    tp[5] = stamp();
#endif

    if constexpr (SHA)
        run_conv_sha(f2s[0], f2s[1], cp.wb2, cp.K2, cp.dil2, ylds + (uint32_t)(hi * a.LW2 + wn * (NW * 32) + l31 + (int)cp.yoff) * 16u,
                     a.y_chunk_bytes, (uint32_t)(2 * a.LW2) * 16u);
    else
        run_conv(f2s, cp.wb2, cp.K2, cp.dil2, ylds + (uint32_t)(hi * a.LW2 + wn * (NW * 32) + l31 + (int)cp.yoff) * 16u,
                 a.y_chunk_bytes, (uint32_t)(2 * a.LW2) * 16u);
#if SX_PAIR_PROF
    tp[6] = stamp();
#endif
    if constexpr (!CHAIN && !EARLY) load_pre();

    {
        constexpr int flags = EPI;
        float *rawb = a.out_raw + (int64_t)b * a.C * T;
        const float wsc = cp.ws2, rdiv = a.div;
        const float *biasp = cp.bias2 ? cp.bias2 : a.zeros;
        const int b_on = cp.bias2 ? 1 : 0;
        const int row0 = wm * 32;
        f32x4 bq[4];
        if constexpr (BIAS_LDS) bias_from_lds(1, bq);
        else {
#pragma unroll
            for (int q = 0; q < 4; q++) bq[q] = *reinterpret_cast<const f32x4 *>(biasp + (row0 + 8 * q + 4 * hi) * b_on);
        }
        static_for<NW / 2>([&](auto R) {
            constexpr int rr = decltype(R)::value;
            f32x4 adl[2][4];
            if constexpr ((flags & EPI_ACC) != 0 && !(EARLY && ACC)) {
#pragma unroll
                for (int j = 0; j < 2; j++) {
                    const int t = t1 + (wn * NW + rr * 2 + j) * 32 + l31;
                    const int tl = INTR ? t : (t < 0 ? 0 : (t < T ? t : T - 1));
#pragma unroll
                    for (int q = 0; q < 4; q++) {
                        if constexpr (INTR)
                            adl[j][q] = *reinterpret_cast<const f32x4 *>(reinterpret_cast<const char *>(rawb + (int64_t)((row0 >> 3) + q) * T * 8) +
                                                                         ((uint32_t)t * 8u + 4u * (uint32_t)hi) * 4u);
                        else adl[j][q] = *reinterpret_cast<const f32x4 *>(rawb + ((int64_t)((row0 >> 3) + q) * T + tl) * 8 + 4 * hi);
                    }
                }
            }
#pragma unroll
            for (int j = 0; j < 2; j++) {
                const int n = rr * 2 + j;
                const int col = (wn * NW + n) * 32 + l31;
                const int t = t1 + col;
                const bool kept = !(col < a.pad2 || col >= a.pad2 + a.BNo || (!INTR && t >= TV));
                if constexpr (NCH == 1) {
                    if (!kept) continue;
                }
#pragma unroll
                for (int q = 0; q < 4; q++) {
                    f32x4 v;
#pragma unroll
                    for (int e = 0; e < 4; e++) v[e] = __builtin_fmaf(acc[n][4 * q + e], wsc, bq[q][e]);
                    v += pre[rr][j][q];
                    if constexpr (NCH > 1) {
                        if (ci > 0) v += tot[rr][j][q];
                        tot[rr][j][q] = v;
                        if (ci < NCH - 1 || !kept) continue;
                    }
                    if constexpr ((flags & EPI_ACC) != 0) {
                        if constexpr (EARLY && ACC) v += ad[rr][j][q];
                        else v += adl[j][q];
                    }
                    if constexpr ((flags & EPI_DIV) != 0) {
#pragma unroll
                        for (int e = 0; e < 4; e++) v[e] = v[e] / rdiv;
                    }
#if SX_PAIR_ST_SC1
                    {
                        float *sp = rawb + ((int64_t)((row0 >> 3) + q) * T + t) * 8 + 4 * hi;
                        const f32x4 sv = v;
                        asm volatile("global_store_dwordx4 %0, %1, off sc1" ::"v"(sp), "v"(sv) : "memory");
                    }
#else
                    if constexpr (INTR)
                        *reinterpret_cast<f32x4 *>(reinterpret_cast<char *>(rawb + (int64_t)((row0 >> 3) + q) * T * 8) +
                                                   ((uint32_t)t * 8u + 4u * (uint32_t)hi) * 4u) = v;
                    else *reinterpret_cast<f32x4 *>(rawb + ((int64_t)((row0 >> 3) + q) * T + t) * 8 + 4 * hi) = v;
#endif
                }
            }
        });
    }
    }
#if SX_PAIR_PROF
    asm volatile("s_waitcnt vmcnt(0)" ::: "memory");
    tp[7] = stamp();
    if (a.prof && tid == 0) {
        for (int i = 0; i < 7; i++) atomicAdd(a.prof + i, tp[i + 1] - tp[i]);
        atomicAdd(a.prof + 7, 1ull);
    }
#endif
}

template <int MW, int NW, int WM, int WN, int EPI, bool CHAIN, int NCH = 1>
__global__ __launch_bounds__(256, (NW == 2 && !SX_PAIR_EARLY_ACC && NCH == 1) ? SX_PAIR_WGS32 : 2) void conv_sx_pair_kernel(SxPairArgs a) {
    const int wg_xcd = blockIdx.x & 7, wg_seq = blockIdx.x >> 3;
    const int tile_nb = __builtin_amdgcn_readfirstlane(sx_xcd_tile(wg_seq, wg_xcd, a.xgs));
    if (tile_nb >= a.NT * a.B) return;
    const int b = tile_nb / a.NT, t0 = (tile_nb - b * a.NT) * a.BNo;
    const int TV = __builtin_amdgcn_readfirstlane(sx_valid_cols(a.rag, b, a.T));
    if (t0 >= TV) return;
    const int xl = t0 - a.pad2 - a.pad1;
    const bool interior = SX_PAIR_INTERIOR != 0 && xl >= 0 && xl + a.LW1 <= TV;
    float pk = 0.f;
    if (interior) conv_sx_pair_body<MW, NW, WM, WN, EPI, CHAIN, NCH, true>(a, b, t0, TV, pk);
    else conv_sx_pair_body<MW, NW, WM, WN, EPI, CHAIN, NCH, false>(a, b, t0, TV, pk);
    if (a.peak) sx_publish_peak(a.peak, (int)blockIdx.x, pk);
}

template <int MW, int NW, int WM, int WN, int EPI, bool CHAIN, int NCH = 1>
inline hipError_t launch_conv_sx_pair_k(const SxPairArgs &a, dim3 grid, size_t lds, hipStream_t stream) {
    static std::atomic<uint64_t> attr_done{0};
    auto kern = conv_sx_pair_kernel<MW, NW, WM, WN, EPI, CHAIN, NCH>;
    if (hipError_t e = sx_allow_big_lds(reinterpret_cast<const void *>(kern), attr_done); e != hipSuccess) return e;
    if (g_launch_name_on)
        snprintf(g_launch_name, sizeof g_launch_name, "conv_sx_pair_kernel<%d, %d, %d, %d, %d, %s, %d>", MW, NW, WM, WN, EPI,
                 CHAIN ? "true" : "false", NCH);
    kern<<<grid, 256, lds, stream>>>(a);
    return hipGetLastError();
}

inline bool sx_pair_supported(int C, int cfg, int K1, int dil1, int K2, int dil2) {
    if (K1 < 3 || K2 < 3 || dil1 < 1 || dil2 < 1) return false;
    if (!((C == 64 && cfg == 1) || (C == 32 && cfg == 2))) return false;
    const int LW1 = 256 + (K1 - 1) * dil1;
    if (2 * LW1 > kSxRawStageCells) return false;
    const int halo2 = (K2 - 1) * dil2;
    static const int keep_min = [] {
        const char *e = std::getenv("VITSMI_PAIR_MIN_KEEP");
        return e ? std::atoi(e) : 160;
    }();
    if (halo2 % 2 || 256 - halo2 < keep_min) return false;
    static const int keep64 = [] {
        const char *e = std::getenv("VITSMI_PAIR_MIN_KEEP64");
        return e ? std::atoi(e) : 200;
    }();
    if (C == 64 && 256 - halo2 < keep64) return false;
    const size_t lds_y = (size_t)(C / 16) * 4 * (size_t)((256 + halo2 / 2 + 7) / 8 * 8) * 16 + (size_t)(halo2 / 2) * 16;
    const size_t lds_x = (size_t)(C / 16) * 4 * LW1 * 16;
    return (lds_y > lds_x ? lds_y : lds_x) <= kLdsTwoPerCu;
}

hipError_t launch_conv_sx_pair(SxPairArgs a, int cfg, int B, hipStream_t stream, bool chain = false);
hipError_t launch_conv_sx_mrf(SxPairArgs a, int B, hipStream_t stream);
#ifdef VITSMI_IMPL_PAIR
hipError_t launch_conv_sx_pair(SxPairArgs a, int cfg, int B, hipStream_t stream, bool chain) {
    a.LW1 = 256 + (a.K1 - 1) * a.dil1;
    a.x_bytes = (unsigned)((size_t)4 * a.LW1 * 16);
    if (a.dil2 < 1) a.dil2 = 1;
    const int halo2 = (a.K2 - 1) * a.dil2;
    if (a.pad2 * 2 != halo2) return hipErrorInvalidValue;
    a.LW2 = (256 + a.pad2 + 7) / 8 * 8;
    a.y_chunk_bytes = (unsigned)(4 * a.LW2 * 16);
    a.BNo = 256 - halo2;
    a.NT = (a.T + a.BNo - 1) / a.BNo;
    a.B = B;
    a.nchunks = a.C / 16;
    if (a.islope == 0.f) a.islope = 1.f;
    if (a.mslope == 0.f) a.mslope = 1.f;
    if (a.wscale1 == 0.f) a.wscale1 = 1.f;
    if (a.wscale2 == 0.f) a.wscale2 = 1.f;
    if ((long long)a.T * 64 + 64 >= (1ll << 32)) return hipErrorInvalidValue;
    const size_t lds_x = (size_t)a.nchunks * a.x_bytes, lds_y = (size_t)a.nchunks * a.y_chunk_bytes + (size_t)a.pad2 * 16;
    size_t lds = lds_x > lds_y ? lds_x : lds_y;
    if (lds > kLdsTwoPerCu || !sx_pair_supported(a.C, cfg, a.K1, a.dil1, a.K2, a.dil2)) return hipErrorInvalidValue;
    if (cfg != 1 && SX_PAIR_SHARED_A) {
        a.a_ring = (unsigned)((lds + 1023) / 1024 * 1024);
        lds = a.a_ring + 3 * 4096;
    }
    a.bias_off = (unsigned)((lds + 15) / 16 * 16);
    lds = a.bias_off + 1024;
    const long long nb = (long long)a.NT * B;
    if (nb == 0) return hipSuccess;
    a.xgs = a.NT >= (2 << sx_xcd_group_shift()) ? sx_xcd_group_shift() : 0;
    const long long per_round = 8ll << a.xgs;
    const long long wgs = (nb + per_round - 1) / per_round * per_round;
    if (wgs >= (1ll << 31)) return hipErrorInvalidValue;
    dim3 grid((unsigned)wgs, 1, 1);
    const int epi = a.flags & (EPI_ACC | EPI_DIV);
    if ((epi & EPI_DIV) && !(epi & EPI_ACC)) return hipErrorInvalidValue;
#define SX_PAIR_CASES(MW, NW, WM, WN, CH)                                                                        \
    switch (epi) {                                                                                               \
        case 0: return launch_conv_sx_pair_k<MW, NW, WM, WN, 0, CH>(a, grid, lds, stream);                       \
        case EPI_ACC: return launch_conv_sx_pair_k<MW, NW, WM, WN, EPI_ACC, CH>(a, grid, lds, stream);           \
        default: return launch_conv_sx_pair_k<MW, NW, WM, WN, EPI_ACC | EPI_DIV, CH>(a, grid, lds, stream);      \
    }
    if (cfg == 1) {
        if (chain) {
            SX_PAIR_CASES(1, 4, 2, 2, true)
        }
        SX_PAIR_CASES(1, 4, 2, 2, false)
    }
    if (chain) {
        SX_PAIR_CASES(1, 2, 1, 4, true)
    }
    SX_PAIR_CASES(1, 2, 1, 4, false)
#undef SX_PAIR_CASES
}
#endif

struct SxMrfGeom {
    int pad1, pad2, LW1, LW2;
    size_t lds;
};
inline bool sx_mrf_geom(int C, int n, const int *K1, const int *dil1, const int *K2, const int *dil2, SxMrfGeom *g) {
    if (C != 32 || n < 2 || n > 3) return false;
    int p1 = 0, p2 = 0;
    for (int i = 0; i < n; i++) {
        if (K1[i] < 3 || K2[i] < 3 || !(K1[i] & 1) || !(K2[i] & 1) || dil1[i] < 1 || dil2[i] < 1) return false;
        const int a1 = (K1[i] - 1) / 2 * dil1[i], a2 = (K2[i] - 1) / 2 * dil2[i];
        p1 = a1 > p1 ? a1 : p1;
        p2 = a2 > p2 ? a2 : p2;
    }
    const int LW1 = 256 + 2 * p1;
    if (2 * LW1 > kSxRawStageCells) return false;
    if (256 - 2 * p2 < 160) return false;
    const int LW2 = (256 + p2 + 7) / 8 * 8;
    const size_t lds = (size_t)(C / 16) * 4 * LW1 * 16 + (size_t)(C / 16) * 4 * LW2 * 16 + (size_t)p2 * 16;
    if (lds > kLdsTwoPerCu) return false;
    if (g) *g = SxMrfGeom{p1, p2, LW1, LW2, lds};
    return true;
}

#ifdef VITSMI_IMPL_PAIR
hipError_t launch_conv_sx_mrf(SxPairArgs a, int B, hipStream_t stream) {
    int K1[3], d1[3], K2[3], d2[3];
    if (a.nchain < 2 || a.nchain > 3) return hipErrorInvalidValue;
    for (int i = 0; i < a.nchain; i++) {
        K1[i] = a.ch[i].K1;
        d1[i] = a.ch[i].dil1;
        K2[i] = a.ch[i].K2;
        d2[i] = a.ch[i].dil2;
    }
    SxMrfGeom g;
    if (!sx_mrf_geom(a.C, a.nchain, K1, d1, K2, d2, &g)) return hipErrorInvalidValue;
    for (int i = 0; i < a.nchain; i++) {
        a.ch[i].xoff = g.pad1 - (K1[i] - 1) / 2 * d1[i];
        a.ch[i].yoff = g.pad2 - (K2[i] - 1) / 2 * d2[i];
        if (a.ch[i].wscale1 == 0.f) a.ch[i].wscale1 = 1.f;
        if (a.ch[i].wscale2 == 0.f) a.ch[i].wscale2 = 1.f;
    }
    a.pad1 = g.pad1;
    a.pad2 = g.pad2;
    a.LW1 = g.LW1;
    a.x_bytes = (unsigned)((size_t)4 * a.LW1 * 16);
    a.LW2 = g.LW2;
    a.y_chunk_bytes = (unsigned)(4 * a.LW2 * 16);
    a.BNo = 256 - 2 * g.pad2;
    a.NT = (a.T + a.BNo - 1) / a.BNo;
    a.B = B;
    a.nchunks = a.C / 16;
    if (a.islope == 0.f) a.islope = 1.f;
    if (a.mslope == 0.f) a.mslope = 1.f;
    if ((long long)a.T * 64 + 64 >= (1ll << 32)) return hipErrorInvalidValue;
    const long long nb = (long long)a.NT * B;
    if (nb == 0) return hipSuccess;
    a.xgs = a.NT >= (2 << sx_xcd_group_shift()) ? sx_xcd_group_shift() : 0;
    const long long per_round = 8ll << a.xgs;
    const long long wgs = (nb + per_round - 1) / per_round * per_round;
    if (wgs >= (1ll << 31)) return hipErrorInvalidValue;
    dim3 grid((unsigned)wgs, 1, 1);
    a.flags = EPI_DIV;
    if (a.nchain == 2) return launch_conv_sx_pair_k<1, 2, 1, 4, EPI_DIV, true, 2>(a, grid, g.lds, stream);
    return launch_conv_sx_pair_k<1, 2, 1, 4, EPI_DIV, true, 3>(a, grid, g.lds, stream);
}
#endif

}
```

phoonnx_amd/csrc/vitsmi.hip:

```cpp
#include <climits>
#include <hip/hip_runtime.h>

#include <cmath>
#include <cstdarg>
#include <chrono>
#include <cstdio>
#include <cstring>
#include <mutex>
#include <string>
#include <vector>

#include "../../include/vitsmi.h"
#include "conv_geom.hpp"
#include "conv_sx_engine.hip.hpp"
#include "conv_sx_pair.hip.hpp"
#include "conv_sx_pair16.hip.hpp"
#include "attention16.hip.hpp"
#include "conv_sx_small.hip.hpp"
#include "delivery.hip.hpp"
#include "delivery_run.hip.hpp"
#include "fit.hip.hpp"
#include "shape.hip.hpp"
#include "kernels.hip.hpp"
#include "loudness.hip.hpp"
// ... 593 lines not shown

void launch_durations(hipStream_t st, int B, int T, const float *logw, const int *len, float length_scale, const float *rows,
                      const float *token_rate, float *w_ceil, int *cum, int *y_len) {
    duration_kernel<<<B, 256, 0, st>>>(logw, len, length_scale, rows, token_rate, w_ceil, cum, y_len, T);
}

void launch_fit_weights(hipStream_t st, int B, int T, const float *logw, const int *len, float length_scale, const float *rows,
                        const float *token_rate, float *w) {
    fit_weight_kernel<<<dim3((T + 255) / 256, B), 256, 0, st>>>(logw, len, length_scale, rows, token_rate, w, T);
}

void launch_fit_durations(hipStream_t st, int B, int T, int G, const float *w, const int *len, const int *group, const int64_t *target,
                          const int *mode, float *w_ceil, int *cum, int *y_len, FitResult *res) {
    fit_duration_kernel<<<G, 256, 0, st>>>(w, len, group, target, mode, B, T, w_ceil, cum, y_len, res);
}

void launch_forced_durations(hipStream_t st, int B, int T, const int64_t *dur, const int *len, float *w_ceil, int *cum, int *y_len) {
    forced_duration_kernel<<<B, 256, 0, st>>>(dur, len, w_ceil, cum, y_len, T);
}

void launch_fill_normal_rows(hipStream_t st, int B, int channels, int T, float *out, const uint64_t *seeds, uint32_t stream,
                             const float *rows, int col) {
    fill_normal_rows_kernel<<<dim3((unsigned)(((T + 3) / 4 + 63) / 64), channels, B), 64, 0, st>>>(out, T, seeds, stream, rows, col);
}

void launch_fill_normal(hipStream_t st, float *out, int64_t n, uint64_t seed, uint64_t stream_id) {
    fill_normal_kernel<<<(unsigned)((n / 4 + 256) / 256), 256, 0, st>>>(out, n, seed, stream_id);
}

void launch_expand_prior(hipStream_t st, int B, int C, int T, int F, const float *m_p, const float *logs_p, int64_t bstride,
                         const int *cum, const int *len, const int *y_len, const float *noise, int64_t noise_stride,
                         float noise_scale, const float *rows, const uint64_t *seeds, float *z_p, int Fnoise) {
    expand_prior_strided_kernel<<<dim3((F + 255) / 256, (C + 3) / 4, B), 64, 0, st>>>(m_p, logs_p, bstride, cum, len, y_len, noise,
                                                                                     noise_stride, noise_scale, rows, seeds, z_p, C,
                                                                                     T, F, Fnoise);
}

size_t post_conv_lds(int C, int K) { return ((size_t)C * (256 + K - 1) + (size_t)C * K) * sizeof(float); }
void launch_post_conv(hipStream_t st, int B, int C, int K, int T, const float *x, const float *w, float *out, float slope,
                      const int *vlen, int hop) {
    const size_t lds = post_conv_lds(C, K);
    post_conv_tanh_kernel<<<dim3((T + 255) / 256, B), 256, lds, st>>>(x, w, out, C, K, T, slope, vlen, hop);
}

size_t post_conv_blocked_lds(int C, int K) { return (size_t)C * (256 + K - 1) * sizeof(float); }
void launch_post_conv_blocked(hipStream_t st, int B, int C, int K, int T, const float *x, const float *w, float *out, float slope,
                              const int *vlen, int hop, bool generic = false) {
    const size_t lds = post_conv_blocked_lds(C, K);
    if (K == 7 && !generic)
        post_conv_tanh_blocked_kernel<7><<<dim3((T + 255) / 256, B), 256, lds, st>>>(x, w, out, C, K, T, slope, vlen, hop);
    else
        post_conv_tanh_blocked_kernel<0><<<dim3((T + 255) / 256, B), 256, lds, st>>>(x, w, out, C, K, T, slope, vlen, hop);
}

void conv_sx_planar(Ctx &c, const ConvDesc &d, const uint16_t *x_pl, int T, float *out, uint16_t *out_pl, int flags,
                    SxOpt o = {}) {
    o.row_split = d.Cout;
    o.pl_rows = out_pl ? d.Cout : 0;
    conv_sx(c, d, x_pl, T, out, out_pl, SX_WN_RMW | flags, o);
}

void split_planes(Ctx &c, const float *x, uint16_t *pl, int C, int T, const int *len) {
    sx_split_planes_kernel<<<dim3((T + 255) / 256, C / 8, c.B), 256, 0, c.st>>>(x, (int64_t)C * T, T, len, pl, C, T, 1,
                                                                                range_slots(c.h, true));
    c.note(hipGetLastError());
    c.h->stats.total_launches++;
}

void fused_launch_end(Ctx &c, bool ev, const ConvDesc *const *members, int n, const ConvDesc &rec, int T, double fl, double by) {
    vits_stats &st = c.h->stats;
    if (ev) conv_event_end(c, true, fl, by, rec, T);
    for (int i = 0; i < n; i++) conv_account(c, *members[i], T);
    st.conv_launches -= n - 1;
    st.total_launches -= n - 1;
    st.sx_flops += fl;
    st.sx_bytes += by;
    st.sx_launches++;
}

bool sx_pair_ok(const vits_handle *h, const ConvDesc &c1, const ConvDesc &c2) {
    static const bool off = std::getenv("VITSMI_SX_NO_PAIR") != nullptr;
    return !off && h->gen_nprod == 2 && c1.f16 && c2.f16 && c1.rawin && c2.rawin && c1.cfg == c2.cfg && c1.ups == 1 &&
           c2.ups == 1 && c1.Cin == c1.Cout && c2.Cin == c2.Cout && c1.Cin == c2.Cin && c2.padL * 2 == (c2.K - 1) * c2.dil &&
           sx_pair_supported(c1.Cin, c1.cfg, c1.K, c1.dil, c2.K, c2.dil);
}

static SxPairArgs sx_pair_args(const ConvDesc &c1, const ConvDesc &c2, const float *A, const float *zeros, const float *x, int T, float *out,
                               int flags, float div, float slope, SxRagged rag, unsigned *peak) {
    SxPairArgs a{};
    const auto P = [A](int64_t off) { return off >= 0 ? A + off : nullptr; };
    a.xr = x;
    a.islope = slope;
    a.mslope = slope;
    a.T = T;
    a.wp1 = reinterpret_cast<const u32x4 *>(P(c1.w_off));
    a.wp2 = reinterpret_cast<const u32x4 *>(P(c2.w_off));
    a.bias1 = P(c1.b_off);
    a.bias2 = P(c2.b_off);
    a.wscale1 = c1.wscale;
    a.wscale2 = c2.wscale;
    a.out_raw = out;
    a.zeros = zeros;
    a.C = c1.Cin;
    a.K1 = c1.K;
    a.dil1 = c1.dil;
    a.pad1 = c1.padL;
    a.K2 = c2.K;
    a.dil2 = c2.dil;
    a.pad2 = c2.padL;
    a.flags = flags & (EPI_ACC | EPI_DIV);
    a.div = div;
    a.rag = rag;
    a.peak = peak;
    return a;
}

void conv_sx_pair(Ctx &c, const ConvDesc &c1, const ConvDesc &c2, const float *x, int T, float *out, int flags, float div,
                  float slope, bool chain = false) {
    vits_handle *h = c.h;
    SxPairArgs a = sx_pair_args(c1, c2, c.A, c.P(c.m.zeros_off), x, T, out, flags, div, slope, c.rag_at(T), range_slots(h, true));
#if SX_PAIR_PROF
    {
        static unsigned long long *rows = nullptr;
        static int idx = 0;
        if (!rows) {
            hipMalloc((void **)&rows, 64 * 8 * sizeof(unsigned long long));
            hipMemset(rows, 0, 64 * 8 * sizeof(unsigned long long));
        }
        if (h->stats.sx_launches == 0 || idx >= 64) idx = 0;
        a.prof = rows + (idx++ % 64) * 8;
        if (std::getenv("VITSMI_PAIR_PROF_DUMP") && idx == 1) {
            unsigned long long hrows[64 * 8];
            hipDeviceSynchronize();
            hipMemcpy(hrows, rows, sizeof hrows, hipMemcpyDeviceToHost);
            for (int r = 0; r < 64; r++)
                if (hrows[r * 8 + 7]) {
                    fprintf(stderr, "pairprof row %d wgs %llu:", r, hrows[r * 8 + 7]);
                    for (int i = 0; i < 7; i++) fprintf(stderr, " %.0f", (double)hrows[r * 8 + i] / (double)hrows[r * 8 + 7]);
                    fprintf(stderr, "\n");
                }
            hipMemset(rows, 0, sizeof hrows);
        }
    }
#endif
    const bool ev = conv_event_begin(c);
    c.note(launch_conv_sx_pair(a, c1.cfg, c.B, c.st, chain));
    const double wf = c.work_frac();
    const double fl = 2.0 * (c1.macs_per_t + c2.macs_per_t) * (double)T * c.B * wf;
    const double by = 4.0 * c.B * ((double)(c1.Cin + c1.Cout) * T + (double)(c2.Cin + c2.Cout) * T) * wf;
    const ConvDesc *const members[] = {&c1, &c2};
    fused_launch_end(c, ev, members, 2, c1, T, fl, by);
}

bool sx_pair16_ok(const vits_handle *h, const ConvDesc &c1, const ConvDesc &c2) {
    static const bool off = [] {
        const char *e = std::getenv("VITSMI_PAIR16");
        return (e && e[0] == '0') || std::getenv("VITSMI_SX_NO_PAIR") != nullptr;
    }();
    if (off || c1.Cin != c1.Cout || c2.Cin != c2.Cout || c1.Cin != c2.Cin || c1.ups != 1 || c2.ups != 1) return false;
    if (c1.padL * 2 != (c1.K - 1) * c1.dil || c2.padL * 2 != (c2.K - 1) * c2.dil) return false;
    const bool h1 = c1.h1 && c2.h1, f3 = c1.f16 && c2.f16 && c1.s16 && c2.s16 && !c1.rawin && !c2.rawin;
    if (!h1 && !f3) return false;
    if (c1.cfg != c2.cfg || c1.cfg != (c1.Cin == 64 ? 1 : 2)) return false;
    (void)h;
    return sx_pair16_plan(c1.Cin, h1 ? 1 : 2, c1.K, c1.dil, c2.K, c2.dil, nullptr) != 0;
}

static SxPair16Args sx_pair16_args(const ConvDesc &c1, const ConvDesc &c2, const float *A, const float *zeros, const uint16_t *x, int T,
                                   float *out_raw, uint16_t *out_pl, int flags, float div, float slope, SxRagged rag, unsigned *peak) {
    SxPair16Args a{};
    const int C = c1.Cin;
    const auto P = [A](int64_t off) { return off >= 0 ? A + off : nullptr; };
    a.xpl = x;
    a.x_bstride = (int64_t)3 * C * T;
    a.islope = a.mslope = a.oslope = slope;
    a.T = T;
    a.wp1 = reinterpret_cast<const u32x4 *>(P(c1.w_off));
    a.wp2 = reinterpret_cast<const u32x4 *>(P(c2.w_off));
    a.bias1 = P(c1.b_off);
    a.bias2 = P(c2.b_off);
    a.wscale1 = c1.wscale;
    a.wscale2 = c2.wscale;
    a.out_raw = out_raw;
    a.raw_bstride = (int64_t)C * T;
    a.out_pl = out_pl;
    a.pl_bstride = (int64_t)3 * C * T;
    a.zeros = zeros;
    a.K1 = c1.K; a.dil1 = c1.dil; a.pad1 = c1.padL;
    a.K2 = c2.K; a.dil2 = c2.dil; a.pad2 = c2.padL;
    a.flags = flags;
    a.div = div;
    a.rag = rag;
    a.peak = peak;
    return a;
}

void conv_sx_pair16(Ctx &c, const ConvDesc &c1, const ConvDesc &c2, const uint16_t *x, int T, float *out_raw, uint16_t *out_pl, int flags,
                    float div, float slope, bool chain) {
    const bool h1 = c1.h1;
    const int C = c1.Cin;
    vits_handle *h = c.h;
    const SxPair16Args a = sx_pair16_args(c1, c2, c.A, c.P(c.m.zeros_off), x, T, out_raw, out_pl, flags, div, slope, c.rag_at(T),
                                          range_slots(h, true));
    const double ebytes = h1 ? 2.0 : 4.0;
    const bool ev = conv_event_begin(c);
    c.note(launch_conv_sx_pair16(a, C, h1 ? 1 : 2, c.B, c.st, chain));
    const double fl = 2.0 * (c1.macs_per_t + c2.macs_per_t) * (double)T * c.B * c.work_frac();
    const double by = ebytes * c.B * ((double)(c1.Cin + c1.Cout) * T + (double)(c2.Cin + c2.Cout) * T) * c.work_frac();
    const ConvDesc *const members[] = {&c1, &c2};
    fused_launch_end(c, ev, members, 2, c1, T, fl, by);
}

bool sx_mrf_ok(const vits_handle *h, const UpStageDesc &stg) {
    const bool off = std::getenv("VITSMI_SX_MRF") == nullptr;
    const int n = (int)stg.rbs.size();
    if (off || n < 2 || n > 3) return false;
    int K1[3], d1[3], K2[3], d2[3];
    for (int j = 0; j < n; j++) {
        const auto &rb = stg.rbs[j];
        if (rb.type1 || rb.n != 2 || !sx_pair_ok(h, rb.c1[0], rb.c1[1]) || rb.c1[0].padL * 2 != (rb.c1[0].K - 1) * rb.c1[0].dil)
            return false;
        K1[j] = rb.c1[0].K;
        d1[j] = rb.c1[0].dil;
        K2[j] = rb.c1[1].K;
        d2[j] = rb.c1[1].dil;
    }
    return sx_mrf_geom(stg.rbs[0].c1[0].Cin, n, K1, d1, K2, d2, nullptr);
}

void conv_sx_mrf(Ctx &c, const UpStageDesc &stg, const float *x, int T, float *out, float slope) {
    const int n = (int)stg.rbs.size();
    SxPairArgs a{};
    a.xr = x;
    a.islope = slope;
    a.mslope = slope;
    a.T = T;
    a.out_raw = out;
    a.zeros = c.P(c.m.zeros_off);
    a.C = stg.rbs[0].c1[0].Cin;
    a.div = (float)n;
    a.nchain = n;
    double macs = 0, bytes = 0;
    const ConvDesc *members[6];
    for (int j = 0; j < n; j++) {
        const ConvDesc &c1 = stg.rbs[j].c1[0], &c2 = stg.rbs[j].c1[1];
        members[2 * j] = &c1;
        members[2 * j + 1] = &c2;
        auto &ch = a.ch[j];
        ch.wp1 = reinterpret_cast<const u32x4 *>(c.P(c1.w_off));
        ch.wp2 = reinterpret_cast<const u32x4 *>(c.P(c2.w_off));
        ch.bias1 = c.P(c1.b_off);
        ch.bias2 = c.P(c2.b_off);
        ch.wscale1 = c1.wscale;
        ch.wscale2 = c2.wscale;
        ch.K1 = c1.K;
        ch.dil1 = c1.dil;
        ch.K2 = c2.K;
        ch.dil2 = c2.dil;
        macs += c1.macs_per_t + c2.macs_per_t;
        bytes += 4.0 * ((double)(c1.Cin + c1.Cout) + (double)(c2.Cin + c2.Cout));
    }
    vits_handle *h = c.h;
    a.rag = c.rag_at(T);
    a.peak = range_slots(h, true);
    macs *= c.work_frac();
    bytes *= c.work_frac();
    const bool ev = conv_event_begin(c);
    c.note(launch_conv_sx_mrf(a, c.B, c.st));
    fused_launch_end(c, ev, members, 2 * n, stg.rbs[n - 1].c1[0], T, 2.0 * macs * (double)T * c.B, bytes * T * c.B);
}

void *pinned_get(vits_handle *h, size_t bytes) {
    PinnedPool &p = h->pin;
    if (!p.busy) {
        if (bytes > p.cap) {
            if (p.base) hipHostFree(p.base);
            p.base = nullptr;
            p.cap = 0;
            size_t want = bytes + bytes / 4 + 4096;
            if (hipHostMalloc((void **)&p.base, want) != hipSuccess) return nullptr;
            p.cap = want;
        }
        p.busy = true;
        return p.base;
    }
    void *q = nullptr;
    return hipHostMalloc(&q, bytes) == hipSuccess ? q : nullptr;
}

void pinned_put(vits_handle *h, void *q) {
    if (!q) return;
    if (h && q == h->pin.base) h->pin.busy = false;
    else hipHostFree(q);
}

enum LnForm : int { LN_FORM_TILE16 = 0, LN_FORM_TILE32 = 1, LN_FORM_COLUMN = 2 };
void launch_layernorm(hipStream_t st, int form, int B, int C, int T, const float *in, float *out, const float *gamma,
                      const float *beta, const int *len, int flags, uint16_t *planes, unsigned *peak) {
    if (form == LN_FORM_TILE16 && planes)
        ln_tile_kernel<0, true, 16><<<dim3((T + 15) / 16, B), 256, 0, st>>>(in, out, gamma, beta, len, C, T, flags, nullptr, nullptr, 1, 1,
                                                                              planes, peak);
    else if (form == LN_FORM_TILE32 && planes)
        ln_tile_kernel<0, true><<<dim3((T + 31) / 32, B), 256, 0, st>>>(in, out, gamma, beta, len, C, T, flags, nullptr, nullptr, 1, 1,
                                                                          planes, peak);
    else if (form == LN_FORM_TILE16)
        ln_tile_kernel<0, false, 16><<<dim3((T + 15) / 16, B), 256, 0, st>>>(in, out, gamma, beta, len, C, T, flags, nullptr, nullptr, 1, 1);
// ... 530 lines not shown
void run_generator_planes(vits_handle *h, Ctx &c, const float *z, int64_t z_bstride, int z_cstride, const int *ylen, int B,
                          int F, const float *dec_cond, const GenBufs &gb) {
    const Model &m = h->model;
    hipStream_t st = h->stream;
    uint16_t *const *stage_in = gb.stage_in, *y_pl = gb.y_pl, *const *raa = gb.raa, *tmp_pl = gb.tmp_pl;
    float *xs_raw = gb.xs_raw;
    rag_begin(h, c, ylen, B, F);
    const float S = 0.1f;
    const int nst = (int)m.ups.size();
    SxOpt act;
    act.oslope2 = S;
    sx_split_planes_kernel<<<dim3((F + 255) / 256, m.C / 8, B), 256, 0, st>>>(z, z_bstride, z_cstride, ylen, tmp_pl, m.C, F,
                                                                              m.gen_h1 ? 2 : 1, range_slots(h, true));
    c.note(hipGetLastError());
    h->stats.total_launches++;
    SxOpt pre = act;
    pre.bias_b = dec_cond;
    pre.bias_b_stride = m.C0;
    conv_sx(c, m.conv_pre, tmp_pl, F, nullptr, stage_in[0], 0, pre);
    const uint16_t *xa = stage_in[0];
    int T = F;
    for (int si = 0; si < nst; si++) {
        const auto &stg = m.ups[si];
        rag_margin(c, m.gen_rf_stage[si]);
        conv_sx(c, stg.up, xa, T, nullptr, y_pl, 0, act);
        T *= stg.u;
        uint16_t *xs_pl = stage_in[(si + 1) & 1];
        const int nk = (int)stg.rbs.size();
        const bool last_stage = si == nst - 1;
        for (int j = 0; j < nk; j++) {
            const auto &rbk = stg.rbs[j];
            auto step_out = [&](int q) {
                StepOut w{EPI_RES, nullptr, raa[q & 1]};
                if (q == rbk.n - 1) {
                    w.flags |= mrf_flags(j, nk);
                    w.raw = xs_raw;
                    w.pl = nullptr;
                    if (j == nk - 1 && !last_stage) {
                        w.pl = xs_pl;
                        if (nk > 1) w.flags |= SX_NO_RAW_STORE;
                        else w.raw = nullptr;
                    }
                }
                return w;
            };
            auto p16_flags = [](const StepOut &w) {
                return (w.flags & (EPI_ACC | EPI_DIV)) | (w.raw && !(w.flags & SX_NO_RAW_STORE) ? P16_HAS_RAW : 0) | (w.pl ? P16_HAS_PL : 0);
            };
            const uint16_t *cur = y_pl;
            for (int q = 0; q < rbk.n; q++) {
                StepOut w = step_out(q);
                SxOpt res = act;
                res.div = (float)nk;
                res.res_pl = cur;
                res.res_slope = S;
                if (rbk.type1) {
                    if (sx_pair16_ok(h, rbk.c1[q], rbk.c2[q]))
                        conv_sx_pair16(c, rbk.c1[q], rbk.c2[q], cur, T, w.raw, w.pl, p16_flags(w), (float)nk, S, false);
                    else {
                        conv_sx(c, rbk.c1[q], cur, T, nullptr, tmp_pl, 0, act);
                        conv_sx(c, rbk.c2[q], tmp_pl, T, w.raw, w.pl, w.flags, res);
                    }
                } else if (q + 1 < rbk.n && sx_pair16_ok(h, rbk.c1[q], rbk.c1[q + 1])) {
                    w = step_out(++q);
                    conv_sx_pair16(c, rbk.c1[q - 1], rbk.c1[q], cur, T, w.raw, w.pl, p16_flags(w), (float)nk, S, true);
                } else
                    conv_sx(c, rbk.c1[q], cur, T, w.raw, w.pl, w.flags, res);
                cur = w.pl;
            }
        }
        xa = xs_pl;
    }
    conv_post_sx(h, c, xs_raw, ylen, B, T, F, gb.out);
}

bool res_planes_on() {
    const char *e = std::getenv("VITSMI_F16X3_RES");
    return e ? std::string(e) != "raw" : true;
}

void run_generator_sx(vits_handle *h, Ctx &c, const float *z, int64_t z_bstride, int z_cstride, const int *ylen, int B,
                      int F, const float *dec_cond, const GenBufs &gb) {
    const Model &m = h->model;
    hipStream_t st = h->stream;
    uint16_t *const *stage_in = gb.stage_in, *y_pl = gb.y_pl, *const *raa = gb.raa, *tmp_pl = gb.tmp_pl;
    float *y_raw = gb.y_raw, *const *ra = gb.ra, *xs_raw = gb.xs_raw;
    float *tmp_raw = reinterpret_cast<float *>(tmp_pl), *xin_raw = reinterpret_cast<float *>(stage_in[0]);
    rag_begin(h, c, ylen, B, F);
    const float S = 0.1f;
    const int nst = (int)m.ups.size();
    SxOpt lrelu;
    lrelu.oslope2 = S;
    lrelu.islope = S;
    const void *zin;
    if (sx_raw_format(m.C)) {
        sx_block_kernel<<<dim3((F + 255) / 256, m.C / 8, B), 256, 0, st>>>(z, z_bstride, z_cstride, ylen, tmp_raw, m.C, F,
                                                                           range_slots(h, m.gen_f16));
        zin = tmp_raw;
    } else {
        sx_split_planes_kernel<<<dim3((F + 255) / 256, m.C / 8, B), 256, 0, st>>>(z, z_bstride, z_cstride, ylen, tmp_pl, m.C, F,
                                                                                  m.gen_f16 ? 1 : 0, range_slots(h, m.gen_f16));
        zin = tmp_pl;
    }
    c.note(hipGetLastError());
    h->stats.total_launches++;
    SxOpt pre;
    pre.bias_b = dec_cond;
    pre.bias_b_stride = m.C0;
    const void *xa;
    if (sx_raw_format(m.C0)) {
        conv_sx(c, m.conv_pre, zin, F, xin_raw, nullptr, 0, pre);
        xa = xin_raw;
    } else {
        pre.oslope2 = S;
        conv_sx(c, m.conv_pre, zin, F, nullptr, stage_in[0], 0, pre);
        xa = stage_in[0];
    }
    int T = F;
    for (int si = 0; si < nst; si++) {
        const auto &stg = m.ups[si];
        rag_margin(c, m.gen_rf_stage[si]);
        const bool fr = sx_raw_format(stg.C);
        SxOpt act;
        if (fr) act.islope = S;
        else act.oslope2 = S;
        bool rpl = !fr && h->gen_nprod == 2 && res_planes_on() && stg.up.s16;
        for (const auto &rbk : stg.rbs)
            for (int q = 0; q < rbk.n && rpl; q++) rpl = rbk.c1[q].s16 && rbk.c1[q].f16 && (!rbk.type1 || (rbk.c2[q].s16 && rbk.c2[q].f16));
        conv_sx(c, stg.up, xa, T, rpl ? nullptr : y_raw, fr ? nullptr : y_pl, 0, lrelu);
        T *= stg.u;
        uint16_t *xs_pl = stage_in[(si + 1) & 1];
        const int nk = (int)stg.rbs.size();
        const bool last_stage = si == nst - 1;
        if (fr && sx_mrf_ok(h, stg)) {
            conv_sx_mrf(c, stg, y_raw, T, xs_raw, S);
            xa = xs_raw;
            continue;
        }
        for (int j = 0; j < nk; j++) {
            const auto &rbk = stg.rbs[j];
            auto step_out = [&](int q) {
                StepOut w{EPI_RES, rpl ? nullptr : ra[q & 1], fr ? nullptr : raa[q & 1]};
                if (q == rbk.n - 1) {
                    w.flags |= mrf_flags(j, nk);
                    w.raw = xs_raw;
                    w.pl = nullptr;
                    if (j == nk - 1 && !last_stage && !fr) {
                        w.pl = xs_pl;
                        w.flags |= SX_NO_RAW_STORE;
                    }
                }
                return w;
            };
            const float *cur = y_raw;
            const uint16_t *cura = y_pl;
            for (int q = 0; q < rbk.n; q++) {
                StepOut w = step_out(q);
                if (rbk.type1 && fr && sx_pair_ok(h, rbk.c1[q], rbk.c2[q])) {
                    conv_sx_pair(c, rbk.c1[q], rbk.c2[q], cur, T, w.raw, w.flags, (float)nk, S);
                } else if (!rbk.type1 && fr && q + 1 < rbk.n && sx_pair_ok(h, rbk.c1[q], rbk.c1[q + 1])) {
                    w = step_out(++q);
                    conv_sx_pair(c, rbk.c1[q - 1], rbk.c1[q], cur, T, w.raw, w.flags, (float)nk, S, true);
                } else {
                    const void *in = fr ? static_cast<const void *>(cur) : static_cast<const void *>(cura);
                    SxOpt res = rbk.type1 || rpl ? act : lrelu;
                    res.div = (float)nk;
                    if (rpl) {
                        res.res_pl = cura;
                        res.res_slope = S;
                    } else
                        res.res = cur;
                    if (rbk.type1) {
                        conv_sx(c, rbk.c1[q], in, T, fr ? tmp_raw : nullptr, fr ? nullptr : tmp_pl, 0, act);
                        conv_sx(c, rbk.c2[q], tmp_pl, T, w.raw, w.pl, w.flags, res);
                    } else
                        conv_sx(c, rbk.c1[q], in, T, w.raw, w.pl, w.flags, res);
                }
                cur = w.raw;
                cura = w.pl;
            }
        }
        xa = (fr || last_stage) ? static_cast<const void *>(xs_raw) : static_cast<const void *>(xs_pl);
    }
    conv_post_sx(h, c, xs_raw, ylen, B, T, F, gb.out);
}

void run_generator_f32(vits_handle *h, Ctx &c, const float *z, int64_t z_bstride, int z_cstride, const int *ylen, int B,
                       int F, const float *dec_cond, const GenBufs &gb) {
    const Model &m = h->model;
    hipStream_t st = h->stream;
    float *const *reg = gb.reg;
    const float S = 0.1f;
    const int nst = (int)m.ups.size();
    ConvOpt gen;
    gen.slope = 1.f;
    ConvOpt mid = gen;
    mid.oslope = S;
    float *xa = reg[0];
    const int Fp = (F + 3) & ~3;
    ConvOpt pre = gen;
    pre.len = ylen;
    pre.bias_b = dec_cond;
    pre.bias_b_stride = m.C0;
    pre.oslope = S;
    pre.x_cstride = z_cstride;
    pre.out_cstride = Fp;
    conv(c, m.conv_pre, z, z_bstride, F, xa, (int64_t)m.C0 * Fp, ylen ? PRO_MASK : 0, pre);
    int T = F, Cc = m.C0, xs_idx = 0;
    int in_pitch = Fp;
    for (int si = 0; si < nst; si++) {
        const auto &stg = m.ups[si];
        float *y = reg[2], *ya = reg[3];
        const int To = T * stg.u;
        ConvOpt up = gen;
        up.out2 = ya;
        up.oslope2 = S;
        up.x_cstride = in_pitch;
        conv(c, stg.up, xa, (int64_t)Cc * in_pitch, T, y, (int64_t)stg.C * To, 0, up);
        in_pitch = To;
        T = To;
        Cc = stg.C;
        const int64_t sCT = (int64_t)Cc * T;
        xs_idx ^= 1;
        float *xs = reg[xs_idx];
        float *ra[2] = {reg[4], reg[6]}, *raa[2] = {reg[5], reg[7]}, *tmp = reg[8];
        const int nk = (int)stg.rbs.size();
        const float out_slope = si == nst - 1 ? 0.01f : S;
        for (int j = 0; j < nk; j++) {
            const auto &rbk = stg.rbs[j];
            const float *cur = y, *cura = ya;
            for (int q = 0; q < rbk.n; q++) {
                const bool last = q == rbk.n - 1;
                float *dst = last ? xs : ra[q & 1];
                const int fl = EPI_RES | (last ? mrf_flags(j, nk) : 0);
                ConvOpt res = gen;
                res.res = cur;
                res.res_bstride = sCT;
                res.div = (float)nk;
                res.oslope = last && j == nk - 1 ? out_slope : 1.f;
                res.out2 = last ? nullptr : raa[q & 1];
                res.oslope2 = S;
                if (rbk.type1) {
                    conv(c, rbk.c1[q], cura, sCT, T, tmp, sCT, 0, mid);
                    conv(c, rbk.c2[q], tmp, sCT, T, dst, sCT, fl, res);
                } else
                    conv(c, rbk.c1[q], cura, sCT, T, dst, sCT, fl, res);
                cur = dst;
                cura = res.out2;
            }
        }
        xa = xs;
    }
    h->S = T;
    h->d_out = gb.out;
    launch_post_conv(st, B, m.post_cin, m.post_k, T, xa, c.P(m.post_w), h->d_out, 1.0f, tail_len(h, ylen), T / F);
    conv_post_account(h, c, B, T);
}

int run_generator(vits_handle *h, Ctx &c, const float *z, int64_t z_bstride, int z_cstride, const int *ylen, int B,
                  int F, const float *dec_cond, const GenBufs &gb) {
    const Model &m = h->model;
    h->cur_stage = 3;
    stage_mark(h, 3);
    if (!m.gen_sx) run_generator_f32(h, c, z, z_bstride, z_cstride, ylen, B, F, dec_cond, gb);
    else if (m.gen_planes) run_generator_planes(h, c, z, z_bstride, z_cstride, ylen, B, F, dec_cond, gb);
    else run_generator_sx(h, c, z, z_bstride, z_cstride, ylen, B, F, dec_cond, gb);
    c.rag = SxRagged{nullptr, 0, 0};
    stage_mark(h, 4);
    return 0;
}

__global__ void chunk_len_kernel(const int *ylen, int *out, int B, int lo, int n) {
    const int b = blockIdx.x * blockDim.x + threadIdx.x;
    if (b < B) {
        const int v = ylen ? ylen[b] - lo : n;
        out[b] = v < 0 ? 0 : (v > n ? n : v);
    }
}


int resample_count(vits_handle *h, int64_t S_in, int &S_out) {
    const ResamplePlan &p = h->rs.plan;
    const int64_t so = p.count(S_in);
    S_out = (int)so;
    if (so <= INT_MAX) return 0;
    return fail(h, VITS_E_ARG, "%lld samples at %d Hz are %lld samples at %d Hz: more than a row admits (%d)", (long long)S_in, p.fi,
                (long long)so, p.fo, INT_MAX);
}

int resample_carve(vits_handle *h, int B, int64_t S_in, ResampleBufs &rb, int &S_out) {
    if (int rc = resample_count(h, S_in, S_out)) return rc;
    return slab_carve(h, h->io, "staging", [&](Carver &cv) { rb = carve_resample(cv, B, S_out, (int)h->rs.plan.K); });
}

int resample_run(vits_handle *h, const int *ylen, int B) {
    const ResamplePlan &p = h->rs.plan;
    const int S = h->S;
    ResampleBufs rb;
    int S_out = 0;
    if (int rc = resample_carve(h, B, S, rb, S_out)) return rc;
    hipStream_t st = h->stream;
    resample_counts_kernel<<<(B + 63) / 64, 64, 0, st>>>(ylen, h->model.hop, S, p.L, p.M, rb.n_in, rb.n_out, B);
    ResampleArgs a = resample_args(h->rs);
    a.x = h->d_out;
    a.x_pitch = S;
    a.x_n = S;
// ... 3131 lines not shown
            for (size_t i = (size_t)npl * CT; i < 3 * CT && ok; i++) ok = hp[(size_t)b * 3 * CT + i] == 0;
        p->guard_ok = ok ? 1 : 0;
    }
    {
        std::vector<unsigned> slots((size_t)kSxPeakSlots * kSxPeakStride);
        TCHECK(download(slots.data(), dpk, slots.size()));
        unsigned top = 0;
        for (int s = 0; s < kSxPeakSlots; s++) top = std::max(top, slots[(size_t)s * kSxPeakStride]);
        std::memcpy(&p->peak, &top, 4);
    }
#if P16_PROF
    {
        const size_t nwg = 1 << 17;
        unsigned long long *dprof = D.fill<unsigned long long>(nwg * 8);
        TCHECK(D.err);
        a.prof = dprof;
        TCHECK(go());
        TCHECK(hipDeviceSynchronize());
        std::vector<unsigned long long> hp(nwg * 8);
        TCHECK(download(hp.data(), dprof, nwg * 8));
        double sum[7] = {0, 0, 0, 0, 0, 0, 0};
        unsigned long long nt = 0, wgs = 0;
        for (size_t w = 0; w < nwg; w++)
            if (hp[w * 8 + 7]) {
                wgs++;
                nt += hp[w * 8 + 7];
                for (int i = 0; i < 7; i++) sum[i] += (double)hp[w * 8 + i];
            }
        fprintf(stderr, "p16prof C %d npl %d K %d wgs %llu tiles %llu | x wait %.0f  barrier %.0f  phase1 %.0f  hand-over %.0f  phase2 %.0f  epilogue %.0f  drain %.0f (cycles per TILE)\n",
                C, npl, K, wgs, nt, sum[0] / nt, sum[1] / nt, sum[2] / nt, sum[3] / nt, sum[4] / nt, sum[5] / nt, sum[6] / nt);
        a.prof = nullptr;
    }
#endif
    if (p->ms_out) TCHECK(time_launches(10, go, p->ms_out));
    return VITS_OK;
}

int vits_test_conv_pair_sx(int device_id, const float *x, int B, int C, int T, const float *w1, const float *b1,
                           const float *w2, const float *b2, int K, int dil1, int dil2, int chain, float slope, float *out,
                           float *ms_out) {
    if (int rc = test_dev(device_id)) return rc;
    const int kern = (chain >> 1) & 3;
    const bool from_plane = (chain & 8) != 0;
    chain &= 1;
    if (kern) {
        vits_test_conv_pair16_epi_args e{};
        e.B = B, e.C = C, e.T = T, e.K = K, e.dil1 = dil1, e.dil2 = dil2, e.chain = chain;
        e.precision = kern == 2 ? VITS_SX_F16 : VITS_SX_F16X3;
        e.flags = from_plane ? VITS_P16_EPI_PLANES : VITS_P16_EPI_RAW;
        e.slope = slope, e.div = 1.f, e.sentinel = 0.f;
        e.x = x, e.w1 = w1, e.b1 = b1, e.w2 = w2, e.b2 = b2;
        (from_plane ? e.planes_out : e.out) = out;
        e.ms_out = ms_out;
        return vits_test_conv_pair16_epi(device_id, &e);
    }
    ConvDesc d1, d2;
    std::vector<float> arena;
    const TestPack o = sx_test_pack(SxPack::F16X2);
    std::string e = pack_test_conv(w1, b1, C, C, K, dil1, dil1 * (K - 1) / 2, 3, &d1, &arena, o);
    if (e.empty()) e = pack_test_conv(w2, b2, C, C, K, dil2, dil2 * (K - 1) / 2, 3, &d2, &arena, o);
    if (!e.empty()) return fail(nullptr, VITS_E_ARG, "%s", e.c_str());
    const size_t n = (size_t)B * C * T;
    DevBufs D;
    if (!d1.rawin || !d2.rawin || d1.cfg != d2.cfg || !sx_pair_supported(C, d1.cfg, d1.K, d1.dil, d2.K, d2.dil))
        return fail(nullptr, VITS_E_ARG, "this conv pair cannot run fused (C %d, kernel %d, dilation %d)", C, K, dil1);
    float *dA = D.up(arena.data(), arena.size());
    float *dx = D.up(x, n, 16);
    float *dxr = D.alloc<float>(n, 16);
    float *draw = D.fill<float>(n, 0, 16);
    float *dout = D.alloc<float>(n, 16);
    TCHECK(D.err);
    sx_block_kernel<<<dim3((T + 255) / 256, C / 8, B), 256>>>(dx, (int64_t)C * T, T, nullptr, dxr, C, T);
    SxPairArgs a{};
    a.xr = dxr;
    a.islope = a.mslope = slope;
    a.T = T;
    a.wp1 = reinterpret_cast<const u32x4 *>(dA + d1.w_off);
    a.wp2 = reinterpret_cast<const u32x4 *>(dA + d2.w_off);
    a.bias1 = d1.b_off >= 0 ? dA + d1.b_off : nullptr;
    a.bias2 = d2.b_off >= 0 ? dA + d2.b_off : nullptr;
    a.wscale1 = d1.wscale;
    a.wscale2 = d2.wscale;
    a.out_raw = draw;
    a.zeros = dA;
    a.C = C;
    a.K1 = d1.K; a.dil1 = d1.dil; a.pad1 = d1.padL;
    a.K2 = d2.K; a.dil2 = d2.dil; a.pad2 = d2.padL;
    a.div = 1.f;
    auto go = [&] { return launch_conv_sx_pair(a, d1.cfg, B, nullptr, chain != 0); };
    TCHECK(go());
    TCHECK(hipDeviceSynchronize());
    if (ms_out) TCHECK(time_launches(10, go, ms_out));
    sx_unblock_kernel<<<dim3((T + 255) / 256, C / 8, B), 256>>>(draw, nullptr, dout, C, T, 1);
    TCHECK(hipGetLastError());
    TCHECK(hipDeviceSynchronize());
    TCHECK(download(out, dout, n));
    return VITS_OK;
}

int vits_test_conv_pair_sx_epi(int device_id, vits_test_conv_pair_sx_epi_args *p) {
    if (int rc = test_dev(device_id)) return rc;
    if (!p) return fail(nullptr, VITS_E_ARG, "no arguments");
    const auto bad = [](const char *why) { return fail(nullptr, VITS_E_ARG, "pair epilogue hook: %s", why); };
    const int B = p->B, C = p->C, T = p->T, K = p->K;
    if (B < 1 || C < 1 || T < 1 || K < 1 || p->dil1 < 1 || p->dil2 < 1 || !p->x || !p->w1 || !p->w2 || !p->out) return bad("bad shape or missing tensor");
    if (p->flags & ~(VITS_PAIR_EPI_ACC | VITS_PAIR_EPI_DIV)) return bad("unknown flag");
    if ((p->flags & VITS_PAIR_EPI_ACC) && !p->out_init) return bad("acc without out_init (the accumulate operand is the raw tensor's previous contents)");
    if (p->lens)
        for (int b = 0; b < B; b++)
            if (p->lens[b] < 0 || p->lens[b] > T) return bad("lens outside [0, T]");
    ConvDesc d1, d2;
    std::vector<float> arena;
    const TestPack o = sx_test_pack(SxPack::F16X2);
    std::string e = pack_test_conv(p->w1, p->b1, C, C, K, p->dil1, p->dil1 * (K - 1) / 2, 3, &d1, &arena, o);
    if (e.empty()) e = pack_test_conv(p->w2, p->b2, C, C, K, p->dil2, p->dil2 * (K - 1) / 2, 3, &d2, &arena, o);
    if (!e.empty()) return fail(nullptr, VITS_E_ARG, "%s", e.c_str());
    if (!d1.rawin || !d2.rawin || d1.cfg != d2.cfg || !sx_pair_supported(C, d1.cfg, d1.K, d1.dil, d2.K, d2.dil))
        return fail(nullptr, VITS_E_ARG, "this conv pair cannot run fused (C %d, kernel %d, dilations %d, %d)", C, K, p->dil1, p->dil2);
    const size_t n = (size_t)B * C * T;
    std::vector<int> l32(B);
    for (int b = 0; b < B; b++) l32[b] = p->lens ? (int)p->lens[b] : T;
    DevBufs D;
    float *dA = D.up(arena.data(), arena.size());
    float *dx = D.up(p->x, n, 16);
    float *dxr = D.alloc<float>(n, 16);
    float *dimg = p->out_init ? D.up(p->out_init, n, 16) : D.fill<float>(n, 0, 16);
    float *draw = D.alloc<float>(n, 16);
    float *dout = D.alloc<float>(n, 16);
    int *dlen = p->lens ? D.up(l32.data(), (size_t)B) : nullptr;
    TCHECK(D.err);
    const dim3 grid((T + 255) / 256, C / 8, B);
    sx_block_kernel<<<grid, 256>>>(dx, (int64_t)C * T, T, nullptr, dxr, C, T);
    sx_block_kernel<<<grid, 256>>>(dimg, (int64_t)C * T, T, nullptr, draw, C, T);
    TCHECK(hipGetLastError());
    const int kflags = ((p->flags & VITS_PAIR_EPI_ACC) ? EPI_ACC : 0) | ((p->flags & VITS_PAIR_EPI_DIV) ? EPI_DIV : 0);
    const SxRagged rag = dlen ? SxRagged{dlen, 0, 1} : SxRagged{nullptr, 0, 0};
    const SxPairArgs a = sx_pair_args(d1, d2, dA, dA, dxr, T, draw, kflags, p->div == 0.f ? 1.f : p->div, p->slope, rag, nullptr);
    const bool name_was_on = g_launch_name_on;
    g_launch_name_on = true;
    g_launch_name[0] = 0;
    const hipError_t le = launch_conv_sx_pair(a, d1.cfg, B, nullptr, p->chain != 0);
    g_launch_name_on = name_was_on;
    if (le != hipSuccess) return fail(nullptr, VITS_E_DEVICE, "pair epilogue hook: launch_conv_sx_pair: %s", hipGetErrorString(le));
    TCHECK(hipDeviceSynchronize());
    std::snprintf(p->kernel, sizeof p->kernel, "%s", g_launch_name);
    p->BNo = 256 - (d2.K - 1) * d2.dil;
    sx_unblock_kernel<<<grid, 256>>>(draw, nullptr, dout, C, T, 1);
    TCHECK(hipGetLastError());
    TCHECK(hipDeviceSynchronize());
    TCHECK(download(p->out, dout, n));
    return VITS_OK;
}

static inline void split_identity_one(float x, uint16_t *o, uint16_t *f) {
    const float v = std::fmin(std::fmax(x, -kF16Max), kF16Max);
    const _Float16 h0 = (_Float16)v;
    const _Float16 a = (_Float16)((v - (float)h0) * 2048.f);
    const _Float16 b = (_Float16)std::fmaf((float)h0, -2048.f, v * 2048.f);
    *o = __builtin_bit_cast(uint16_t, a);
    *f = __builtin_bit_cast(uint16_t, b);
}
int vits_test_split_identity(const float *x, int64_t n, uint16_t *h1_old, uint16_t *h1_fused) {
    if (!x || n < 0 || !h1_old || !h1_fused) return fail(nullptr, VITS_E_ARG, "split identity: missing array");
    for (int64_t i = 0; i < n; i++) split_identity_one(x[i], h1_old + i, h1_fused + i);
    return VITS_OK;
}
int64_t vits_test_split_identity_sweep(uint32_t first, uint64_t count, uint32_t *first_bad) {
    int64_t bad = 0;
    for (uint64_t k = 0; k < count; k++) {
        const uint32_t bits = first + (uint32_t)k;
        uint16_t o, f;
        split_identity_one(__builtin_bit_cast(float, bits), &o, &f);
        const bool nan_o = (o & 0x7fffu) > 0x7c00u, nan_f = (f & 0x7fffu) > 0x7c00u;
        if (o != f && !(nan_o && nan_f)) {
            if (bad == 0 && first_bad) *first_bad = bits;
            bad++;
        }
    }
    return bad;
}

int vits_test_split_forms(int device_id, const float *x, int n, float slope, int form, uint16_t *h0, uint16_t *h1, float *pk, float *rec) {
    if (int rc = test_dev(device_id)) return rc;
    if (!x || n < 2 || (n & 1) || !(slope > 0.f) || slope > 1.f || form < 0 || form > 1 || !h0 || !h1 || !pk || !rec)
        return fail(nullptr, VITS_E_ARG, "split forms hook: n even and >= 2, 0 < slope <= 1, form 0 or 1, every output given");
    DevBufs D;
    float *dx = D.up(x, (size_t)n);
    uint16_t *d0 = D.alloc<uint16_t>((size_t)n), *d1 = D.alloc<uint16_t>((size_t)n);
    float *dpk = D.alloc<float>((size_t)n / 2), *drec = D.alloc<float>((size_t)n);
    TCHECK(D.err);
    const unsigned blocks = (unsigned)((n / 2 + 255) / 256);
    if (form == 0) split_forms_kernel<0><<<blocks, 256>>>(dx, n, slope, 1.f / slope, d0, d1, dpk, drec);
    else split_forms_kernel<1><<<blocks, 256>>>(dx, n, slope, 1.f / slope, d0, d1, dpk, drec);
    TCHECK(hipGetLastError());
    TCHECK(hipDeviceSynchronize());
    TCHECK(download(h0, d0, (size_t)n));
    TCHECK(download(h1, d1, (size_t)n));
    TCHECK(download(pk, dpk, (size_t)n / 2));
    TCHECK(download(rec, drec, (size_t)n));
    return VITS_OK;
}

int vits_bench_conv1d_sx(int device_id, int B, int Cin, int Cout, int T, int K, int dil, int dbg, int iters,
                         float *ms_out) {
    if (int rc = test_dev(device_id)) return rc;
    std::vector<float> w((size_t)Cout * Cin * K), x((size_t)B * Cin * T);
    bench_fill(w, x);
    ConvDesc d;
    std::vector<float> arena;
    TestPack o = sx_test_pack((dbg & 64) ? SxPack::F16X1 : ((dbg & 128) ? SxPack::F16X2 : SxPack::BF16X3));
    o.sx.no_s16 = (dbg & (1 | 2 | 16 | 256)) != 0;
    std::string e = pack_test_conv(w.data(), nullptr, Cin, Cout, K, dil, dil * (K - 1) / 2, 3, &d, &arena, o);
    if (!e.empty()) return fail(nullptr, VITS_E_ARG, "%s", e.c_str());
    const size_t nx = x.size(), no = (size_t)B * Cout * T;
    DevBufs D;
    float *dA = D.up(arena.data(), arena.size());
    float *dx = D.up(x.data(), nx);
    uint16_t *dxp = D.alloc<uint16_t>(nx * 3);
    float *draw = D.alloc<float>(no);
    float *dres = D.fill<float>(no);
    uint16_t *dop = D.alloc<uint16_t>(no * 3);
    unsigned long long *dprof = (dbg & 16) ? D.fill<unsigned long long>(8) : nullptr;
    TCHECK(D.err);
    sx_split_planes_kernel<<<dim3((T + 255) / 256, Cin / 8, B), 256>>>(dx, (int64_t)Cin * T, T, nullptr, dxp, Cin, T,
                                                                       d.h1 ? 2 : (d.f16 ? 1 : 0));
    SxArgs a = sx_args(d, dA, dA, T);
    a.xp = reinterpret_cast<const u32x4 *>(dxp);
    a.out_pl = dop;
    a.oslope2 = 0.1f;
    a.flags = ((dbg & 1) ? DBG_NO_DMA : 0) | ((dbg & 2) ? DBG_NO_EPI : 0);
    if (dbg & 8) {
        a.flags |= EPI_RES;
        if (d.h1) {
            a.res_pl = reinterpret_cast<const uint16_t *>(dres);
            a.res_unslope = 10.f;
        } else {
            a.res = dres;
            a.out_raw = draw;
        }
    }
    if (d.rawin) {
        a.xr = dx;
        a.islope = 0.1f;
        a.out_pl = nullptr;
        a.out_raw = draw;
    }
    a.prof = dprof;
    auto go = [&] { return launch_conv_sx(a, d.cfg, B, nullptr, d.rawin, d.h1 ? 1 : (d.f16 ? 2 : 6)); };
    for (int i = 0; i < 2; i++) TCHECK(go());
    TCHECK(hipDeviceSynchronize());
    if (dprof) TCHECK(hipMemset(dprof, 0, 64));
    float ms = 0.f;
    TCHECK(time_launches(iters, go, &ms));
    if (ms_out) {
        ms_out[0] = ms;
        ms_out[1] = (float)d.cfg;
        ms_out[2] = 0.f;
        if (dprof) {
            unsigned long long hp[8];
            TCHECK(download(hp, dprof, 8));
            for (int i = 0; i < 5; i++) ms_out[3 + i] = hp[5] ? (float)((double)hp[i] / (double)hp[5]) : 0.f;
            ms_out[2] = hp[7] ? (float)((double)hp[6] / (double)hp[7] * 0.1) : 0.f;
        }
    }
    return VITS_OK;
}

int vits_test_attention(int device_id, const float *qkv, int B, int C, int T, int n_heads, const float *rel_k,
                        const float *rel_v, int window, const int64_t *lens, float *out) {
    if (int rc = test_dev(device_id)) return rc;
    if (window > 4 || C % n_heads) return fail(nullptr, VITS_E_ARG, "bad attention test arguments");
    int dk = C / n_heads;
    if (dk > kAttMaxHeadWidth) return fail(nullptr, VITS_E_ARG, "attention head width %d > %d is unsupported", dk, kAttMaxHeadWidth);
    size_t nq = (size_t)B * 3 * C * T, no = (size_t)B * C * T, nr = (size_t)(2 * window + 1) * dk;
    std::vector<int> l32(B);
    for (int b = 0; b < B; b++) l32[b] = (int)lens[b];
    DevBufs D;
    float *dq = D.up(qkv, nq);
    float *dout = D.alloc<float>(no);
    float *drk = D.up(rel_k, nr);
    float *drv = D.up(rel_v, nr);
    int *dlen = D.up(l32.data(), (size_t)B);
    TCHECK(D.err);
    launch_attention(nullptr, B, T, n_heads, dk, window, dq, dout, drk, drv, dlen, C);
    TCHECK(hipGetLastError());
    TCHECK(hipDeviceSynchronize());
    TCHECK(download(out, dout, no));
    return VITS_OK;
}

int vits_test_attention16(int device_id, const float *qkv, int B, int C, int T, int n_heads, const float *rel_k,
                          const float *rel_v, int window, const int64_t *lens, float *out, uint16_t *out_planes, int kernel,
                          int reps, float *ms_out) {
    if (int rc = test_dev(device_id)) return rc;
    if (window > 4 || C % n_heads || C % 8) return fail(nullptr, VITS_E_ARG, "bad attention test arguments");
    int dk = C / n_heads;
    if (kernel == 1 && !(dk % 32 == 0 && dk <= 96)) return fail(nullptr, VITS_E_ARG, "attention16 needs a head width of 32, 64 or 96");
    if (dk > kAttMaxHeadWidth) return fail(nullptr, VITS_E_ARG, "attention head width %d > %d is unsupported", dk, kAttMaxHeadWidth);
    size_t nq = (size_t)B * 3 * C * T, no = (size_t)B * C * T, nr = (size_t)(2 * window + 1) * dk;
    std::vector<int> l32(B);
    for (int b = 0; b < B; b++) l32[b] = (int)lens[b];
    DevBufs D;
    float *dq = D.up(qkv, nq);
    uint16_t *dqp = D.alloc<uint16_t>(nq * 3);
    uint16_t *dop = D.fill<uint16_t>(no * 3, 0xff);
    unsigned *dpk = D.fill<unsigned>((size_t)kSxPeakSlots * kSxPeakStride);
// ... 1164 lines not shown
```

Before: 144.5 million.

## Fuse all ResBlock1 conv-pair steps into one launch with halo recompute

```diff
diff --git a/include/vitsmi.h b/include/vitsmi.h
--- a/include/vitsmi.h
+++ b/include/vitsmi.h
@@ -485,6 +485,22 @@
     int BNo;
 } vits_test_conv_pair_sx_epi_args;
 int vits_test_conv_pair_sx_epi(int device_id, vits_test_conv_pair_sx_epi_args *a);
+typedef struct {
+    int B, C, T, K;
+    int dil1[3], dil2[3];
+    int flags;
+    float slope, div;
+    const float *x;
+    const float *w1[3], *b1[3], *w2[3], *b2[3];
+    const int64_t *lens;
+    const float *out_init;
+    float *out, *out_ref;
+    float peak, peak_ref;
+    char kernel[128];
+    int BNo;
+    float *ms_out, *ms_ref_out;
+} vits_test_conv_pair_steps_args;
+int vits_test_conv_pair_steps(int device_id, vits_test_conv_pair_steps_args *a);
 int vits_test_split_identity(const float *x, int64_t n, uint16_t *h1_old, uint16_t *h1_fused);
 int64_t vits_test_split_identity_sweep(uint32_t first, uint64_t count, uint32_t *first_bad);
 int vits_test_split_forms(int device_id, const float *x, int n, float slope, int form, uint16_t *h0, uint16_t *h1, float *pk,
diff --git a/phoonnx_amd/_ffi.py b/phoonnx_amd/_ffi.py
--- a/phoonnx_amd/_ffi.py
+++ b/phoonnx_amd/_ffi.py
@@ -70,6 +70,15 @@
                [(n, C.c_float) for n in ("slope", "div")] + \
                [(n, C.c_void_p) for n in ("x", "w1", "b1", "w2", "b2", "lens", "out_init", "out")] + \
                [("kernel", C.c_char * 128), ("BNo", C.c_int)]
+
+
+class VitsTestConvPairStepsArgs(C.Structure):
+    _fields_ = [(n, C.c_int) for n in ("B", "C", "T", "K")] + [("dil1", C.c_int * 3), ("dil2", C.c_int * 3), ("flags", C.c_int)] + \
+               [(n, C.c_float) for n in ("slope", "div")] + [("x", C.c_void_p)] + \
+               [(n, C.c_void_p * 3) for n in ("w1", "b1", "w2", "b2")] + \
+               [(n, C.c_void_p) for n in ("lens", "out_init", "out", "out_ref")] + \
+               [("peak", C.c_float), ("peak_ref", C.c_float), ("kernel", C.c_char * 128), ("BNo", C.c_int),
+                ("ms_out", C.c_void_p), ("ms_ref_out", C.c_void_p)]
 
 
 class VitsTestAttentionFormArgs(C.Structure):
@@ -216,7 +225,7 @@
     "vits_test_stream_pack_trimmed",
     "vits_test_layernorm", "vits_test_dds", "vits_test_cf_pre", "vits_test_rqs_inverse", "vits_test_ea_logw",
     "vits_test_conv1d_epi", "vits_test_wn_gate", "vits_test_cond_matvec", "vits_test_conv1d_sx_epi",
-    "vits_test_conv_pair16_epi", "vits_test_attention_form", "vits_test_conv_pair_sx_epi", "vits_test_split_forms", "vits_test_split_identity", "vits_test_split_identity_sweep",
+    "vits_test_conv_pair16_epi", "vits_test_attention_form", "vits_test_conv_pair_sx_epi", "vits_test_conv_pair_steps", "vits_test_split_forms", "vits_test_split_identity", "vits_test_split_identity_sweep",
 ]
 
 
@@ -439,6 +448,7 @@
     lib.vits_test_conv1d_sx_epi.argtypes = [C.c_int, C.POINTER(VitsTestConvSxEpiArgs)]
     lib.vits_test_conv_pair16_epi.argtypes = [C.c_int, C.POINTER(VitsTestConvPair16EpiArgs)]
     lib.vits_test_conv_pair_sx_epi.argtypes = [C.c_int, C.POINTER(VitsTestConvPairSxEpiArgs)]
+    lib.vits_test_conv_pair_steps.argtypes = [C.c_int, C.POINTER(VitsTestConvPairStepsArgs)]
     lib.vits_test_split_identity.argtypes = [vp, C.c_int64, vp, vp]
     lib.vits_test_split_identity_sweep.argtypes = [C.c_uint32, C.c_uint64, C.POINTER(C.c_uint32)]
     lib.vits_test_split_identity_sweep.restype = C.c_int64
diff --git a/phoonnx_amd/csrc/conv_sx_pair.hip.hpp b/phoonnx_amd/csrc/conv_sx_pair.hip.hpp
--- a/phoonnx_amd/csrc/conv_sx_pair.hip.hpp
+++ b/phoonnx_amd/csrc/conv_sx_pair.hip.hpp
@@ -38,6 +38,15 @@
     unsigned long long *prof;
     SxRagged rag;
     int xgs = 0;
+    struct Step {
+        const u32x4 *wp1, *wp2;
+        const float *bias1, *bias2;
+        float wscale1, wscale2;
+        int K1, dil1, pad1, K2, dil2, pad2;
+        int LW1, LW2;
+    } st[3];
+    int nsteps = 0, reach = 0;
+    unsigned zfill_off = 0, zfill_cells = 0;
 };
 
 #ifndef SX_PAIR_PROF
@@ -55,37 +64,22 @@
 #ifndef SX_PAIR_DEPTH64
 #define SX_PAIR_DEPTH64 2
 #endif
-#ifndef SX_PAIR_EARLY_ACC
-#define SX_PAIR_EARLY_ACC 0
-#endif
 #ifndef SX_PAIR_WGS32
 #define SX_PAIR_WGS32 3
 #endif
-#ifndef SX_PAIR_EARLY32
-#define SX_PAIR_EARLY32 1
-#endif
 #ifndef SX_PAIR_ST_SC1
 #define SX_PAIR_ST_SC1 0
 #endif
 #ifndef SX_PAIR_INTERIOR
 #define SX_PAIR_INTERIOR 1
 #endif
-#ifndef SX_PAIR_ONE_READ64
-#define SX_PAIR_ONE_READ64 1
-#endif
-#ifndef SX_PAIR_ONE_READ32
-#define SX_PAIR_ONE_READ32 1
-#endif
-template <int MW, int NW, int WM, int WN, int EPI, bool CHAIN, int NCH, bool INTR>
+template <int MW, int NW, int WM, int WN, int EPI, bool CHAIN, int NCH, bool INTR, bool STEPS = false>
 __device__ __forceinline__ void conv_sx_pair_body(const SxPairArgs &a, const int b, const int t0, const int TV, float &pk) {
     constexpr int BN = NW * WN * 32, NH = NW / 2;
     static_assert(NCH == 1 || (CHAIN && NW == 2 && (EPI & EPI_ACC) == 0), "fused chains: 32 channels, no external running sum");
-    constexpr bool ONE_READ = NW == 4 ? SX_PAIR_ONE_READ64 != 0 : SX_PAIR_ONE_READ32 != 0;
-    constexpr bool EARLY = ONE_READ || (NW == 2 && SX_PAIR_EARLY32);
+    static_assert(!STEPS || (!CHAIN && NCH == 1 && !SX_PAIR_SHARED_A), "fused steps: ResBlock1 steps of one chain, private weight streams");
     constexpr int DEPTH = NW == 2 ? SX_PAIR_DEPTH32 : SX_PAIR_DEPTH64;
     static_assert(DEPTH >= 2 && DEPTH <= 6, "wait_a covers up to five younger sets");
-    constexpr bool ACC = (EPI & EPI_ACC) != 0 && SX_PAIR_EARLY_ACC;
-    static_assert(!(ONE_READ && ACC), "the running sum is not pulled into the single-read prologue");
     static_assert(WM * WN == 4 && MW == 1 && BN == 256, "one block row per wave, 256 columns");
     constexpr int NPW = 2, STEPBYTES = WM * MW * NPW * 1024;
     constexpr int MAXCH = WM * 2;
@@ -94,7 +88,7 @@
     const int wave = __builtin_amdgcn_readfirstlane(tid >> 6);
     const int wm = wave / WN, wn = wave % WN;
     const int l31 = lane & 31, hi = lane >> 5;
-    const int t1 = t0 - a.pad2;
+    const int t1 = t0 - (STEPS ? a.reach : a.pad2);
     const int T = a.T, LW = a.LW1;
     const uint32_t lds0 = (uint32_t)(uintptr_t)lds_sx;
     const uint32_t XB = a.x_bytes;
@@ -112,7 +106,7 @@
         f.fa[1] = global_read128<1024>(voff0, sb);
     };
 
-    f32x4 pre[NW / 2][2][4], ad[EARLY && ACC ? NW / 2 : 1][2][4];
+    f32x4 pre[NW / 2][2][4];
     auto load_res = [&](const float *base, f32x4 (*dst)[2][4]) {
         static_for<NW / 2>([&](auto R) {
             constexpr int rr = decltype(R)::value;
@@ -123,14 +117,13 @@
                 const int tl = t < 0 ? 0 : (t < T ? t : T - 1);
 #pragma unroll
                 for (int q = 0; q < 4; q++) {
-                    if constexpr (INTR && EARLY) {
+                    if constexpr (INTR) {
                         const char *rowb = reinterpret_cast<const char *>(base + (int64_t)((row0 >> 3) + q) * T * 8);
                         dst[rr][j][q] = __builtin_bit_cast(f32x4, global_read128<0>(((uint32_t)t * 8u + 4u * (uint32_t)hi) * 4u, rowb));
                         continue;
                     }
                     const float *p = base + ((int64_t)((row0 >> 3) + q) * T + tl) * 8 + 4 * hi;
-                    if constexpr (EARLY) dst[rr][j][q] = __builtin_bit_cast(f32x4, global_read128_v<0>(p));
-                    else dst[rr][j][q] = *reinterpret_cast<const f32x4 *>(p);
+                    dst[rr][j][q] = __builtin_bit_cast(f32x4, global_read128_v<0>(p));
                 }
             }
         });
@@ -156,14 +149,18 @@
                             reinterpret_cast<float *>(lds_sx + a.a_ring + (unsigned)((g * 2 + sub) * 2048 + pl * 1024)));
             }
     constexpr bool BIAS_LDS = NCH == 1;
-    if constexpr (BIAS_LDS) {
+    auto bias_dma = [&](const float *b1, const float *b2) __attribute__((always_inline)) {
         if (wave == 0) {
             constexpr int CC = WM * 32;
             const int k = lane - (lane >= CC / 4 ? CC / 4 : 0);
-            const float *bp = lane < CC / 4 ? a.bias1 : a.bias2;
+            const float *bp = lane < CC / 4 ? b1 : b2;
             const void *src = (bp && lane < CC / 2) ? static_cast<const void *>(bp + 4 * k) : static_cast<const void *>(a.zeros + 4 * (lane & 31));
             lds_dma<16>(src, reinterpret_cast<float *>(lds_sx + a.bias_off));
         }
+    };
+    if constexpr (BIAS_LDS) bias_dma(a.bias1, a.bias2);
+    if constexpr (STEPS) {
+        for (unsigned i = (unsigned)tid; i < a.zfill_cells; i += 256u) ds_write128(lds0 + a.zfill_off + i * 16u, u32x4{0u, 0u, 0u, 0u});
     }
     auto bias_from_lds = [&](int conv, f32x4 (&bq)[4]) __attribute__((always_inline)) {
         u32x4 t4[4];
@@ -175,8 +172,7 @@
 #pragma unroll
         for (int q = 0; q < 4; q++) bq[q] = __builtin_bit_cast(f32x4, t4[q]);
     };
-    constexpr int NXC = 3;
-    if constexpr (ONE_READ) {
+    {
         constexpr int NXH = MAXCH, NG = 2 * MAXCH;
         const int HW = LW - 256, pad1 = a.pad1;
         const int nhc = HW * NG, nxh = (nhc + 255) >> 8;
@@ -250,67 +246,6 @@
                 asm volatile("ds_write_b64 %0, %1" ::"v"(cell + (uint32_t)(2 * LW) * 16u), "v"(u32x2{wa[1], wb[1]}) : "memory");
             }
             asm volatile("" : "+v"(pk));
-        });
-    } else {
-        u32x4 xst[MAXCH][NXC][2];
-        const int nxc = (2 * LW + 255) >> 8;
-        uint32_t xroff[NXC];
-        bool xrok[NXC];
-        int xkh[NXC], xcol[NXC];
-#pragma unroll
-        for (int it = 0; it < NXC; it++) {
-            const int i = it * 256 + tid;
-            const int kh = (i >= LW ? 1 : 0) + (i >= 2 * LW ? 1 : 0);
-            const int col = i - kh * LW;
-            const int t = t1 - a.pad1 + col;
-            xkh[it] = kh;
-            xcol[it] = col;
-            xrok[it] = it < nxc && kh < 2 && (INTR || (t >= 0 && t < TV));
-            xroff[it] = xrok[it] ? (uint32_t)(((int64_t)kh * T + t) * 32) : 0u;
-        }
-        static_for<MAXCH>([&](auto CH) {
-            constexpr int ch = decltype(CH)::value;
-            const float *cbase = xrb + (int64_t)(2 * ch) * T * 8;
-            static_for<NXC>([&](auto I) {
-                constexpr int it = decltype(I)::value;
-                if (it < nxc) {
-                    xst[ch][it][0] = global_read128_x<0>(xroff[it], cbase);
-                    xst[ch][it][1] = global_read128_x<16>(xroff[it], cbase);
-                }
-            });
-        });
-        if constexpr (EARLY) {
-            load_pre();
-            if constexpr (ACC) {
-                load_res(a.out_raw + (int64_t)b * a.C * T, ad);
-                asm volatile("s_waitcnt vmcnt(16)" ::: "memory");
-            } else
-                asm volatile("s_waitcnt vmcnt(8)" ::: "memory");
-        } else
-            asm volatile("s_waitcnt vmcnt(0)" ::: "memory");
-#if SX_PAIR_PROF
-        tp[1] = stamp();
-#endif
-        const float isl = a.islope;
-        static_for<MAXCH>([&](auto CH) {
-            constexpr int ch = decltype(CH)::value;
-            static_for<NXC>([&](auto I) {
-                constexpr int it = decltype(I)::value;
-                if (it < nxc && xkh[it] < 2) {
-                    float v[8];
-#pragma unroll
-                    for (int e = 0; e < 8; e++) {
-                        const float x = xrok[it] ? __uint_as_float(xst[ch][it][e >> 2][e & 3]) : 0.f;
-                        v[e] = lrelu_max(x, isl);
-                    }
-                    unsigned p0[4], p1[4];
-#pragma unroll
-                    for (int e = 0; e < 4; e++) sx_pair_split(v[2 * e], v[2 * e + 1], p0[e], p1[e], pk);
-                    const uint32_t ad = lds0 + (uint32_t)ch * XB + (uint32_t)(xkh[it] * LW + xcol[it]) * 16u;
-                    ds_write128(ad, u32x4{p0[0], p0[1], p0[2], p0[3]});
-                    ds_write128(ad + (uint32_t)(2 * LW) * 16u, u32x4{p1[0], p1[1], p1[2], p1[3]});
-                }
-            });
         });
     }
 
@@ -513,7 +448,6 @@
         }
         return c;
     };
-    static_assert(NCH == 1 || EARLY, "fused chains keep x in registers from the prologue on");
     const uint32_t ylds = NCH > 1 ? lds0 + (uint32_t)a.nchunks * XB : lds0;
     f32x4 xkeep[NCH > 1 ? NW / 2 : 1][2][4], tot[NCH > 1 ? NW / 2 : 1][2][4];
 #if SX_PAIR_ALIAS
@@ -522,9 +456,95 @@
 #else
     ASet f1s[DEPTH + 1], f2s[DEPTH + 1];
 #endif
+    ChainPar cp;
+    auto epilogue = [&](const int ci) __attribute__((always_inline)) {
+        constexpr int flags = EPI;
+        float *rawb = a.out_raw + (int64_t)b * a.C * T;
+        const float wsc = cp.ws2, rdiv = a.div;
+        const float *biasp = cp.bias2 ? cp.bias2 : a.zeros;
+        const int b_on = cp.bias2 ? 1 : 0;
+        const int row0 = wm * 32;
+        f32x4 bq[4];
+        if constexpr (BIAS_LDS) bias_from_lds(1, bq);
+        else {
+#pragma unroll
+            for (int q = 0; q < 4; q++) bq[q] = *reinterpret_cast<const f32x4 *>(biasp + (row0 + 8 * q + 4 * hi) * b_on);
+        }
+        static_for<NW / 2>([&](auto R) {
+            constexpr int rr = decltype(R)::value;
+            f32x4 adl[2][4];
+            if constexpr ((flags & EPI_ACC) != 0) {
+#pragma unroll
+                for (int j = 0; j < 2; j++) {
+                    const int t = t1 + (wn * NW + rr * 2 + j) * 32 + l31;
+                    const int tl = INTR ? t : (t < 0 ? 0 : (t < T ? t : T - 1));
+#pragma unroll
+                    for (int q = 0; q < 4; q++) {
+                        if constexpr (INTR)
+                            adl[j][q] = *reinterpret_cast<const f32x4 *>(reinterpret_cast<const char *>(rawb + (int64_t)((row0 >> 3) + q) * T * 8) +
+                                                                         ((uint32_t)t * 8u + 4u * (uint32_t)hi) * 4u);
+                        else adl[j][q] = *reinterpret_cast<const f32x4 *>(rawb + ((int64_t)((row0 >> 3) + q) * T + tl) * 8 + 4 * hi);
+                    }
+                }
+            }
+#pragma unroll
+            for (int j = 0; j < 2; j++) {
+                const int n = rr * 2 + j;
+                const int col = (wn * NW + n) * 32 + l31;
+                const int t = t1 + col;
+                const int kl = STEPS ? a.reach : a.pad2;
+                const bool kept = !(col < kl || col >= kl + a.BNo || (!INTR && t >= TV));
+                if constexpr (NCH == 1) {
+                    if (!kept) continue;
+                }
+#pragma unroll
+                for (int q = 0; q < 4; q++) {
+                    f32x4 v;
+#pragma unroll
+                    for (int e = 0; e < 4; e++) v[e] = __builtin_fmaf(acc[n][4 * q + e], wsc, bq[q][e]);
+                    v += pre[rr][j][q];
+                    if constexpr (NCH > 1) {
+                        if (ci > 0) v += tot[rr][j][q];
+                        tot[rr][j][q] = v;
+                        if (ci < NCH - 1 || !kept) continue;
+                    }
+                    if constexpr ((flags & EPI_ACC) != 0) {
+                        v += adl[j][q];
+                    }
+                    if constexpr ((flags & EPI_DIV) != 0) {
+#pragma unroll
+                        for (int e = 0; e < 4; e++) v[e] = v[e] / rdiv;
+                    }
+#if SX_PAIR_ST_SC1
+                    {
+                        float *sp = rawb + ((int64_t)((row0 >> 3) + q) * T + t) * 8 + 4 * hi;
+                        const f32x4 sv = v;
+                        asm volatile("global_store_dwordx4 %0, %1, off sc1" ::"v"(sp), "v"(sv) : "memory");
+                    }
+#else
+                    if constexpr (INTR)
+                        *reinterpret_cast<f32x4 *>(reinterpret_cast<char *>(rawb + (int64_t)((row0 >> 3) + q) * T * 8) +
+                                                   ((uint32_t)t * 8u + 4u * (uint32_t)hi) * 4u) = v;
+                    else *reinterpret_cast<f32x4 *>(rawb + ((int64_t)((row0 >> 3) + q) * T + t) * 8 + 4 * hi) = v;
+#endif
+                }
+            }
+        });
+    };
+    int sLW = LW, spad1 = a.pad1, spad2 = a.pad2, sLW2 = a.LW2, lo = 0;
+    uint32_t sXB = XB, sYC = a.y_chunk_bytes;
+    const int nloop = STEPS ? a.nsteps : NCH;
 #pragma unroll 1
-    for (int ci = 0; ci < NCH; ci++) {
-    const ChainPar cp = chain_par(ci);
+    for (int ci = 0; ci < nloop; ci++) {
+    cp = chain_par(ci);
+    if constexpr (STEPS) {
+        const auto &h = a.st[ci];
+        cp = ChainPar{reinterpret_cast<const char *>(h.wp1) + wm * (MW * NPW * 1024), reinterpret_cast<const char *>(h.wp2) + wm * (MW * NPW * 1024),
+                      h.bias1, h.bias2, h.wscale1, h.wscale2, h.K1, h.dil1, h.K2, h.dil2, 0u, 0u};
+        sLW = h.LW1, spad1 = h.pad1, spad2 = h.pad2, sLW2 = h.LW2;
+        sXB = (uint32_t)(4 * sLW) * 16u, sYC = (uint32_t)(4 * sLW2) * 16u;
+        if (ci > 0) lo += spad1;
+    }
     if constexpr (NCH > 1) {
         if (ci > 0) {
 #pragma unroll
@@ -536,7 +556,9 @@
             zero_acc();
         }
     }
-    if constexpr (!SHA) load_a(f1s[0], cp.wb1, 0);
+    if constexpr (!SHA) {
+        if (!STEPS || ci == 0) load_a(f1s[0], cp.wb1, 0);
+    }
     if (ci == 0) {
         asm volatile("s_waitcnt lgkmcnt(0)" ::: "memory");
 #if SX_PAIR_PROF
@@ -552,13 +574,12 @@
         run_conv_sha(f1s[0], f1s[1], cp.wb1, cp.K1, cp.dil1, lds0 + (uint32_t)(hi * LW + wn * (NW * 32) + l31 + (int)cp.xoff) * 16u,
                      XB, (uint32_t)(2 * LW) * 16u);
     else
-        run_conv(f1s, cp.wb1, cp.K1, cp.dil1, lds0 + (uint32_t)(hi * LW + wn * (NW * 32) + l31 + (int)cp.xoff) * 16u, XB,
-                 (uint32_t)(2 * LW) * 16u);
+        run_conv(f1s, cp.wb1, cp.K1, cp.dil1, lds0 + (uint32_t)(hi * sLW + wn * (NW * 32) + l31 + (int)cp.xoff) * 16u, sXB,
+                 (uint32_t)(2 * sLW) * 16u);
 
 #if SX_PAIR_PROF
     tp[4] = stamp();
 #endif
-    if constexpr (CHAIN && !EARLY) load_pre();
 
     if constexpr (!SHA) load_a(f2s[0], cp.wb2, 0);
     asm volatile("s_waitcnt lgkmcnt(0)" ::: "memory");
@@ -569,7 +590,7 @@
         const float wsc = cp.ws1, msl = a.mslope;
         const float *biasp = cp.bias1 ? cp.bias1 : a.zeros;
         const int b_on = cp.bias1 ? 1 : 0;
-        const uint32_t YC = a.y_chunk_bytes, LW2 = (uint32_t)a.LW2;
+        const uint32_t YC = sYC, LW2 = (uint32_t)sLW2;
         const int row0 = wm * 32;
         f32x4 bq[4];
         if constexpr (BIAS_LDS) bias_from_lds(0, bq);
@@ -581,7 +602,7 @@
         for (int n = 0; n < NW; n++) {
             const int col = (wn * NW + n) * 32 + l31;
             const int t = t1 + col;
-            const bool live = INTR || (t >= 0 && t < TV);
+            const bool live = (INTR || (t >= 0 && t < TV)) && (!STEPS || (col >= lo && col < 256 - lo));
 #pragma unroll
             for (int q = 0; q < 4; q++) {
                 float o[4];
@@ -601,7 +622,7 @@
                 sx_pair_split(o[0], o[1], wa[0], wa[1], pk);
                 sx_pair_split(o[2], o[3], wb[0], wb[1], pk);
                 const int g = 4 * wm + q;
-                const uint32_t cell = ylds + (uint32_t)(g >> 1) * YC + ((uint32_t)(g & 1) * LW2 + (uint32_t)(col + a.pad2)) * 16u + 8u * hi;
+                const uint32_t cell = ylds + (uint32_t)(g >> 1) * YC + ((uint32_t)(g & 1) * LW2 + (uint32_t)(col + spad2)) * 16u + 8u * hi;
                 asm volatile("ds_write_b64 %0, %1" ::"v"(cell), "v"(u32x2{wa[0], wb[0]}) : "memory");
                 asm volatile("ds_write_b64 %0, %1" ::"v"(cell + 2u * LW2 * 16u), "v"(u32x2{wa[1], wb[1]}) : "memory");
             }
@@ -620,88 +641,62 @@
         run_conv_sha(f2s[0], f2s[1], cp.wb2, cp.K2, cp.dil2, ylds + (uint32_t)(hi * a.LW2 + wn * (NW * 32) + l31 + (int)cp.yoff) * 16u,
                      a.y_chunk_bytes, (uint32_t)(2 * a.LW2) * 16u);
     else
-        run_conv(f2s, cp.wb2, cp.K2, cp.dil2, ylds + (uint32_t)(hi * a.LW2 + wn * (NW * 32) + l31 + (int)cp.yoff) * 16u,
-                 a.y_chunk_bytes, (uint32_t)(2 * a.LW2) * 16u);
+        run_conv(f2s, cp.wb2, cp.K2, cp.dil2, ylds + (uint32_t)(hi * sLW2 + wn * (NW * 32) + l31 + (int)cp.yoff) * 16u,
+                 sYC, (uint32_t)(2 * sLW2) * 16u);
 #if SX_PAIR_PROF
     tp[6] = stamp();
 #endif
-    if constexpr (!CHAIN && !EARLY) load_pre();
-
-    {
-        constexpr int flags = EPI;
-        float *rawb = a.out_raw + (int64_t)b * a.C * T;
-        const float wsc = cp.ws2, rdiv = a.div;
-        const float *biasp = cp.bias2 ? cp.bias2 : a.zeros;
-        const int b_on = cp.bias2 ? 1 : 0;
-        const int row0 = wm * 32;
-        f32x4 bq[4];
-        if constexpr (BIAS_LDS) bias_from_lds(1, bq);
-        else {
-#pragma unroll
-            for (int q = 0; q < 4; q++) bq[q] = *reinterpret_cast<const f32x4 *>(biasp + (row0 + 8 * q + 4 * hi) * b_on);
-        }
-        static_for<NW / 2>([&](auto R) {
-            constexpr int rr = decltype(R)::value;
-            f32x4 adl[2][4];
-            if constexpr ((flags & EPI_ACC) != 0 && !(EARLY && ACC)) {
-#pragma unroll
-                for (int j = 0; j < 2; j++) {
-                    const int t = t1 + (wn * NW + rr * 2 + j) * 32 + l31;
-                    const int tl = INTR ? t : (t < 0 ? 0 : (t < T ? t : T - 1));
-#pragma unroll
-                    for (int q = 0; q < 4; q++) {
-                        if constexpr (INTR)
-                            adl[j][q] = *reinterpret_cast<const f32x4 *>(reinterpret_cast<const char *>(rawb + (int64_t)((row0 >> 3) + q) * T * 8) +
-                                                                         ((uint32_t)t * 8u + 4u * (uint32_t)hi) * 4u);
-                        else adl[j][q] = *reinterpret_cast<const f32x4 *>(rawb + ((int64_t)((row0 >> 3) + q) * T + tl) * 8 + 4 * hi);
-                    }
-                }
-            }
-#pragma unroll
-            for (int j = 0; j < 2; j++) {
-                const int n = rr * 2 + j;
+
+    if constexpr (STEPS) {
+        if (ci + 1 < nloop) {
+            lo += spad2;
+            const auto &nx = a.st[ci + 1];
+            const int nLW = nx.LW1, npad1 = nx.pad1;
+            const uint32_t nXB = (uint32_t)(4 * nLW) * 16u;
+            const float wsc = cp.ws2, isl = a.islope;
+            f32x4 bq[4];
+            bias_from_lds(1, bq);
+            load_a(f1s[0], reinterpret_cast<const char *>(nx.wp1) + wm * (MW * NPW * 1024), 0);
+            asm volatile("s_waitcnt lgkmcnt(0)" ::: "memory");
+            __builtin_amdgcn_s_barrier();
+            __builtin_amdgcn_sched_barrier(0);
+            bias_dma(nx.bias1, nx.bias2);
+#pragma unroll
+            for (int n = 0; n < NW; n++) {
                 const int col = (wn * NW + n) * 32 + l31;
                 const int t = t1 + col;
-                const bool kept = !(col < a.pad2 || col >= a.pad2 + a.BNo || (!INTR && t >= TV));
-                if constexpr (NCH == 1) {
-                    if (!kept) continue;
-                }
+                const bool ok = (INTR || (t >= 0 && t < TV)) && col >= lo && col < 256 - lo;
 #pragma unroll
                 for (int q = 0; q < 4; q++) {
                     f32x4 v;
 #pragma unroll
                     for (int e = 0; e < 4; e++) v[e] = __builtin_fmaf(acc[n][4 * q + e], wsc, bq[q][e]);
-                    v += pre[rr][j][q];
-                    if constexpr (NCH > 1) {
-                        if (ci > 0) v += tot[rr][j][q];
-                        tot[rr][j][q] = v;
-                        if (ci < NCH - 1 || !kept) continue;
-                    }
-                    if constexpr ((flags & EPI_ACC) != 0) {
-                        if constexpr (EARLY && ACC) v += ad[rr][j][q];
-                        else v += adl[j][q];
-                    }
-                    if constexpr ((flags & EPI_DIV) != 0) {
-#pragma unroll
-                        for (int e = 0; e < 4; e++) v[e] = v[e] / rdiv;
-                    }
-#if SX_PAIR_ST_SC1
-                    {
-                        float *sp = rawb + ((int64_t)((row0 >> 3) + q) * T + t) * 8 + 4 * hi;
-                        const f32x4 sv = v;
-                        asm volatile("global_store_dwordx4 %0, %1, off sc1" ::"v"(sp), "v"(sv) : "memory");
-                    }
-#else
-                    if constexpr (INTR)
-                        *reinterpret_cast<f32x4 *>(reinterpret_cast<char *>(rawb + (int64_t)((row0 >> 3) + q) * T * 8) +
-                                                   ((uint32_t)t * 8u + 4u * (uint32_t)hi) * 4u) = v;
-                    else *reinterpret_cast<f32x4 *>(rawb + ((int64_t)((row0 >> 3) + q) * T + t) * 8 + 4 * hi) = v;
-#endif
+                    v += pre[n / 2][n % 2][q];
+                    pre[n / 2][n % 2][q] = v;
+                    float o[4];
+#pragma unroll
+                    for (int e = 0; e < 4; e++) o[e] = lrelu_max(ok ? v[e] : 0.f, isl);
+                    unsigned wa[2], wb[2];
+                    sx_pair_split(o[0], o[1], wa[0], wa[1], pk);
+                    sx_pair_split(o[2], o[3], wb[0], wb[1], pk);
+                    const int g = 4 * wm + q;
+                    const uint32_t cell = lds0 + (uint32_t)(g >> 1) * nXB + (uint32_t)((g & 1) * nLW + npad1 + col) * 16u + 8u * hi;
+                    asm volatile("ds_write_b64 %0, %1" ::"v"(cell), "v"(u32x2{wa[0], wb[0]}) : "memory");
+                    asm volatile("ds_write_b64 %0, %1" ::"v"(cell + (uint32_t)(2 * nLW) * 16u), "v"(u32x2{wa[1], wb[1]}) : "memory");
                 }
-            }
-        });
-    }
-    }
+                asm volatile("" : "+v"(pk));
+            }
+            zero_acc();
+            asm volatile("s_waitcnt vmcnt(0) lgkmcnt(0)" ::: "memory");
+            __builtin_amdgcn_s_barrier();
+            __builtin_amdgcn_sched_barrier(0);
+            continue;
+        }
+        break;
+    }
+    epilogue(ci);
+    }
+    if constexpr (STEPS) epilogue(nloop - 1);
 #if SX_PAIR_PROF
     asm volatile("s_waitcnt vmcnt(0)" ::: "memory");
     tp[7] = stamp();
@@ -712,32 +707,44 @@
 #endif
 }
 
-template <int MW, int NW, int WM, int WN, int EPI, bool CHAIN, int NCH = 1>
-__global__ __launch_bounds__(256, (NW == 2 && !SX_PAIR_EARLY_ACC && NCH == 1) ? SX_PAIR_WGS32 : 2) void conv_sx_pair_kernel(SxPairArgs a) {
+template <int MW, int NW, int WM, int WN, int EPI, bool CHAIN, int NCH = 1, bool STEPS = false>
+__global__ __launch_bounds__(256, (NW == 2 && NCH == 1) ? SX_PAIR_WGS32 : 2) void conv_sx_pair_kernel(SxPairArgs a) {
     const int wg_xcd = blockIdx.x & 7, wg_seq = blockIdx.x >> 3;
     const int tile_nb = __builtin_amdgcn_readfirstlane(sx_xcd_tile(wg_seq, wg_xcd, a.xgs));
     if (tile_nb >= a.NT * a.B) return;
     const int b = tile_nb / a.NT, t0 = (tile_nb - b * a.NT) * a.BNo;
     const int TV = __builtin_amdgcn_readfirstlane(sx_valid_cols(a.rag, b, a.T));
     if (t0 >= TV) return;
-    const int xl = t0 - a.pad2 - a.pad1;
+    const int xl = t0 - (STEPS ? a.reach : a.pad2) - a.pad1;
     const bool interior = SX_PAIR_INTERIOR != 0 && xl >= 0 && xl + a.LW1 <= TV;
     float pk = 0.f;
-    if (interior) conv_sx_pair_body<MW, NW, WM, WN, EPI, CHAIN, NCH, true>(a, b, t0, TV, pk);
-    else conv_sx_pair_body<MW, NW, WM, WN, EPI, CHAIN, NCH, false>(a, b, t0, TV, pk);
+    if (interior) conv_sx_pair_body<MW, NW, WM, WN, EPI, CHAIN, NCH, true, STEPS>(a, b, t0, TV, pk);
+    else conv_sx_pair_body<MW, NW, WM, WN, EPI, CHAIN, NCH, false, STEPS>(a, b, t0, TV, pk);
     if (a.peak) sx_publish_peak(a.peak, (int)blockIdx.x, pk);
 }
 
-template <int MW, int NW, int WM, int WN, int EPI, bool CHAIN, int NCH = 1>
+template <int MW, int NW, int WM, int WN, int EPI, bool CHAIN, int NCH = 1, bool STEPS = false>
 inline hipError_t launch_conv_sx_pair_k(const SxPairArgs &a, dim3 grid, size_t lds, hipStream_t stream) {
     static std::atomic<uint64_t> attr_done{0};
-    auto kern = conv_sx_pair_kernel<MW, NW, WM, WN, EPI, CHAIN, NCH>;
+    auto kern = conv_sx_pair_kernel<MW, NW, WM, WN, EPI, CHAIN, NCH, STEPS>;
     if (hipError_t e = sx_allow_big_lds(reinterpret_cast<const void *>(kern), attr_done); e != hipSuccess) return e;
     if (g_launch_name_on)
-        snprintf(g_launch_name, sizeof g_launch_name, "conv_sx_pair_kernel<%d, %d, %d, %d, %d, %s, %d>", MW, NW, WM, WN, EPI,
-                 CHAIN ? "true" : "false", NCH);
+        snprintf(g_launch_name, sizeof g_launch_name, "conv_sx_pair_kernel<%d, %d, %d, %d, %d, %s, %d%s>", MW, NW, WM, WN, EPI,
+                 CHAIN ? "true" : "false", NCH, STEPS ? ", true" : "");
     kern<<<grid, 256, lds, stream>>>(a);
     return hipGetLastError();
+}
+
+inline int sx_pair_keep_min(int C) {
+    static const int keep_min = [] {
+        const char *e = std::getenv("VITSMI_PAIR_MIN_KEEP");
+        return e ? std::atoi(e) : 160;
+    }();
+    static const int keep64 = [] {
+        const char *e = std::getenv("VITSMI_PAIR_MIN_KEEP64");
+        return e ? std::atoi(e) : 200;
+    }();
+    return C == 64 && keep64 > keep_min ? keep64 : keep_min;
 }
 
 inline bool sx_pair_supported(int C, int cfg, int K1, int dil1, int K2, int dil2) {
@@ -746,16 +753,7 @@
     const int LW1 = 256 + (K1 - 1) * dil1;
     if (2 * LW1 > kSxRawStageCells) return false;
     const int halo2 = (K2 - 1) * dil2;
-    static const int keep_min = [] {
-        const char *e = std::getenv("VITSMI_PAIR_MIN_KEEP");
-        return e ? std::atoi(e) : 160;
-    }();
-    if (halo2 % 2 || 256 - halo2 < keep_min) return false;
-    static const int keep64 = [] {
-        const char *e = std::getenv("VITSMI_PAIR_MIN_KEEP64");
-        return e ? std::atoi(e) : 200;
-    }();
-    if (C == 64 && 256 - halo2 < keep64) return false;
+    if (halo2 % 2 || 256 - halo2 < sx_pair_keep_min(C)) return false;
     const size_t lds_y = (size_t)(C / 16) * 4 * (size_t)((256 + halo2 / 2 + 7) / 8 * 8) * 16 + (size_t)(halo2 / 2) * 16;
     const size_t lds_x = (size_t)(C / 16) * 4 * LW1 * 16;
     return (lds_y > lds_x ? lds_y : lds_x) <= kLdsTwoPerCu;
@@ -763,7 +761,96 @@
 
 hipError_t launch_conv_sx_pair(SxPairArgs a, int cfg, int B, hipStream_t stream, bool chain = false);
 hipError_t launch_conv_sx_mrf(SxPairArgs a, int B, hipStream_t stream);
+
+struct SxPairStepsGeom {
+    int reach, BNo;
+    int LW1[3], LW2[3];
+    size_t x0_bytes, tile_bytes;
+};
+inline bool sx_pair_steps_geom(int C, int n, const int *K1, const int *dil1, const int *K2, const int *dil2, SxPairStepsGeom *g) {
+    if (n < 2 || n > 3) return false;
+    SxPairStepsGeom s{};
+    const size_t rows = (size_t)(C / 16) * 4;
+    for (int i = 0; i < n; i++) {
+        if (K1[i] < 3 || K2[i] < 3 || dil1[i] < 1 || dil2[i] < 1) return false;
+        const int h1 = (K1[i] - 1) * dil1[i], h2 = (K2[i] - 1) * dil2[i];
+        if (h1 % 2 || h2 % 2) return false;
+        s.LW1[i] = i == 0 ? 256 + h1 : (256 + h1 / 2 + 7) / 8 * 8;
+        s.LW2[i] = (256 + h2 / 2 + 7) / 8 * 8;
+        s.reach += (i == 0 ? 0 : h1 / 2) + h2 / 2;
+        const size_t tx = rows * s.LW1[i] * 16 + (i == 0 ? 0 : (size_t)(h1 / 2) * 16), ty = rows * s.LW2[i] * 16 + (size_t)(h2 / 2) * 16;
+        if (i == 0) s.x0_bytes = tx;
+        s.tile_bytes = std::max(s.tile_bytes, std::max(tx, ty));
+    }
+    s.BNo = 256 - 2 * s.reach;
+    if (g) *g = s;
+    return true;
+}
+inline bool sx_pair_steps_supported(int C, int cfg, int n, const int *K1, const int *dil1, const int *K2, const int *dil2, long long T = 0) {
+    static const bool off = std::getenv("VITSMI_PAIR_NO_STEPS") != nullptr;
+    if (off) return false;
+    if (!(C == 32 && cfg == 2)) return false;
+    SxPairStepsGeom g;
+    if (!sx_pair_steps_geom(C, n, K1, dil1, K2, dil2, &g)) return false;
+    if (2 * g.LW1[0] > kSxRawStageCells) return false;
+    constexpr int kStepsKeepMin = 224;
+    if (g.BNo < kStepsKeepMin || g.BNo < sx_pair_keep_min(C)) return false;
+    if (T * 64 + 64 >= (1ll << 32)) return false;
+    return g.tile_bytes + 1024 <= (size_t)kLdsTwoPerCu;
+}
+hipError_t launch_conv_sx_pair_steps(SxPairArgs a, int cfg, int B, hipStream_t stream);
 #ifdef VITSMI_IMPL_PAIR
+hipError_t launch_conv_sx_pair_steps(SxPairArgs a, int cfg, int B, hipStream_t stream) {
+    int K1[3], d1[3], K2[3], d2[3];
+    const int n = a.nsteps;
+    if (n < 2 || n > 3) return hipErrorInvalidValue;
+    for (int i = 0; i < n; i++) {
+        auto &s = a.st[i];
+        K1[i] = s.K1, d1[i] = s.dil1, K2[i] = s.K2, d2[i] = s.dil2;
+        if (s.pad1 * 2 != (s.K1 - 1) * s.dil1 || s.pad2 * 2 != (s.K2 - 1) * s.dil2) return hipErrorInvalidValue;
+        if (s.wscale1 == 0.f) s.wscale1 = 1.f;
+        if (s.wscale2 == 0.f) s.wscale2 = 1.f;
+    }
+    SxPairStepsGeom g;
+    if (!sx_pair_steps_supported(a.C, cfg, n, K1, d1, K2, d2, a.T) || !sx_pair_steps_geom(a.C, n, K1, d1, K2, d2, &g)) return hipErrorInvalidValue;
+    for (int i = 0; i < n; i++) a.st[i].LW1 = g.LW1[i], a.st[i].LW2 = g.LW2[i];
+    const auto &s0 = a.st[0];
+    a.wp1 = s0.wp1, a.wp2 = s0.wp2, a.bias1 = s0.bias1, a.bias2 = s0.bias2, a.wscale1 = s0.wscale1, a.wscale2 = s0.wscale2;
+    a.K1 = s0.K1, a.dil1 = s0.dil1, a.pad1 = s0.pad1, a.K2 = s0.K2, a.dil2 = s0.dil2, a.pad2 = s0.pad2;
+    a.LW1 = g.LW1[0];
+    a.x_bytes = (unsigned)((size_t)4 * a.LW1 * 16);
+    a.LW2 = g.LW2[0];
+    a.y_chunk_bytes = (unsigned)(4 * a.LW2 * 16);
+    a.reach = g.reach;
+    a.BNo = g.BNo;
+    a.NT = (a.T + a.BNo - 1) / a.BNo;
+    a.B = B;
+    a.nchunks = a.C / 16;
+    if (a.islope == 0.f) a.islope = 1.f;
+    a.mslope = a.islope;
+    a.zfill_off = (unsigned)g.x0_bytes;
+    a.zfill_cells = (unsigned)((g.tile_bytes - g.x0_bytes + 15) / 16);
+    a.bias_off = (unsigned)((g.tile_bytes + 15) / 16 * 16);
+    const size_t lds = a.bias_off + 1024;
+    const long long nb = (long long)a.NT * B;
+    if (nb == 0) return hipSuccess;
+    a.xgs = a.NT >= (2 << sx_xcd_group_shift()) ? sx_xcd_group_shift() : 0;
+    const long long per_round = 8ll << a.xgs;
+    const long long wgs = (nb + per_round - 1) / per_round * per_round;
+    if (wgs >= (1ll << 31)) return hipErrorInvalidValue;
+    dim3 grid((unsigned)wgs, 1, 1);
+    const int epi = a.flags & (EPI_ACC | EPI_DIV);
+    if ((epi & EPI_DIV) && !(epi & EPI_ACC)) return hipErrorInvalidValue;
+#define SX_PAIR_STEPS_CASES(NW, WM, WN)                                                                                  \
+    switch (epi) {                                                                                                       \
+        case 0: return launch_conv_sx_pair_k<1, NW, WM, WN, 0, false, 1, true>(a, grid, lds, stream);                    \
+        case EPI_ACC: return launch_conv_sx_pair_k<1, NW, WM, WN, EPI_ACC, false, 1, true>(a, grid, lds, stream);        \
+        default: return launch_conv_sx_pair_k<1, NW, WM, WN, EPI_ACC | EPI_DIV, false, 1, true>(a, grid, lds, stream);   \
+    }
+    SX_PAIR_STEPS_CASES(2, 1, 4)
+#undef SX_PAIR_STEPS_CASES
+}
+
 hipError_t launch_conv_sx_pair(SxPairArgs a, int cfg, int B, hipStream_t stream, bool chain) {
     a.LW1 = 256 + (a.K1 - 1) * a.dil1;
     a.x_bytes = (unsigned)((size_t)4 * a.LW1 * 16);
diff --git a/phoonnx_amd/csrc/vitsmi.hip b/phoonnx_amd/csrc/vitsmi.hip
--- a/phoonnx_amd/csrc/vitsmi.hip
+++ b/phoonnx_amd/csrc/vitsmi.hip
@@ -769,6 +769,53 @@
     fused_launch_end(c, ev, members, 2, c1, T, fl, by);
 }
 
+bool sx_pair_steps_ok(const vits_handle *h, const ResBlockDesc &rb, int T) {
+    if (!rb.type1 || rb.n != 3) return false;
+    int K1[3], d1[3], K2[3], d2[3];
+    for (int q = 0; q < rb.n; q++) {
+        const ConvDesc &c1 = rb.c1[q], &c2 = rb.c2[q];
+        if (!sx_pair_ok(h, c1, c2) || c1.padL * 2 != (c1.K - 1) * c1.dil || c1.Cin != rb.c1[0].Cin || c1.cfg != rb.c1[0].cfg) return false;
+        K1[q] = c1.K, d1[q] = c1.dil, K2[q] = c2.K, d2[q] = c2.dil;
+    }
+    return sx_pair_steps_supported(rb.c1[0].Cin, rb.c1[0].cfg, rb.n, K1, d1, K2, d2, T);
+}
+
+static SxPairArgs sx_pair_steps_args(const ConvDesc *c1, const ConvDesc *c2, int n, const float *A, const float *zeros, const float *x, int T,
+                                     float *out, int flags, float div, float slope, SxRagged rag, unsigned *peak) {
+    SxPairArgs a = sx_pair_args(c1[0], c2[0], A, zeros, x, T, out, flags, div, slope, rag, peak);
+    const auto P = [A](int64_t off) { return off >= 0 ? A + off : nullptr; };
+    a.nsteps = n;
+    for (int q = 0; q < n; q++) {
+        auto &s = a.st[q];
+        s.wp1 = reinterpret_cast<const u32x4 *>(P(c1[q].w_off));
+        s.wp2 = reinterpret_cast<const u32x4 *>(P(c2[q].w_off));
+        s.bias1 = P(c1[q].b_off);
+        s.bias2 = P(c2[q].b_off);
+        s.wscale1 = c1[q].wscale;
+        s.wscale2 = c2[q].wscale;
+        s.K1 = c1[q].K, s.dil1 = c1[q].dil, s.pad1 = c1[q].padL;
+        s.K2 = c2[q].K, s.dil2 = c2[q].dil, s.pad2 = c2[q].padL;
+    }
+    return a;
+}
+
+void conv_sx_pair_steps(Ctx &c, const ResBlockDesc &rb, const float *x, int T, float *out, int flags, float div, float slope) {
+    const SxPairArgs a = sx_pair_steps_args(rb.c1, rb.c2, rb.n, c.A, c.P(c.m.zeros_off), x, T, out, flags, div, slope,
+                                            c.rag_at(T), range_slots(c.h, true));
+    const bool ev = conv_event_begin(c);
+    c.note(launch_conv_sx_pair_steps(a, rb.c1[0].cfg, c.B, c.st));
+    const double wf = c.work_frac();
+    double macs = 0, by = 0;
+    const ConvDesc *members[6];
+    for (int q = 0; q < rb.n; q++) {
+        members[2 * q] = &rb.c1[q];
+        members[2 * q + 1] = &rb.c2[q];
+        macs += rb.c1[q].macs_per_t + rb.c2[q].macs_per_t;
+        by += 4.0 * ((double)(rb.c1[q].Cin + rb.c1[q].Cout) + (double)(rb.c2[q].Cin + rb.c2[q].Cout));
+    }
+    fused_launch_end(c, ev, members, 2 * rb.n, rb.c1[rb.n - 1], T, 2.0 * macs * (double)T * c.B * wf, by * T * c.B * wf);
+}
+
 bool sx_pair16_ok(const vits_handle *h, const ConvDesc &c1, const ConvDesc &c2) {
     static const bool off = [] {
         const char *e = std::getenv("VITSMI_PAIR16");
@@ -1605,6 +1652,11 @@
                 }
                 return w;
             };
+            if (fr && sx_pair_steps_ok(h, rbk, T)) {
+                const StepOut w = step_out(rbk.n - 1);
+                conv_sx_pair_steps(c, rbk, y_raw, T, w.raw, w.flags, (float)nk, S);
+                continue;
+            }
             const float *cur = y_raw;
             const uint16_t *cura = y_pl;
             for (int q = 0; q < rbk.n; q++) {
@@ -5042,6 +5094,104 @@
     return VITS_OK;
 }
 
+int vits_test_conv_pair_steps(int device_id, vits_test_conv_pair_steps_args *p) {
+    if (int rc = test_dev(device_id)) return rc;
+    if (!p) return fail(nullptr, VITS_E_ARG, "no arguments");
+    const auto bad = [](const char *why) { return fail(nullptr, VITS_E_ARG, "pair steps hook: %s", why); };
+    const int B = p->B, C = p->C, T = p->T, K = p->K, N = 3;
+    if (B < 1 || C < 1 || T < 1 || K < 1 || !p->x || !p->out || !p->out_ref) return bad("bad shape or missing tensor");
+    for (int q = 0; q < N; q++)
+        if (p->dil1[q] < 1 || p->dil2[q] < 1 || !p->w1[q] || !p->w2[q]) return bad("bad dilation or missing weights");
+    if (p->flags & ~(VITS_PAIR_EPI_ACC | VITS_PAIR_EPI_DIV)) return bad("unknown flag");
+    if ((p->flags & VITS_PAIR_EPI_ACC) && !p->out_init) return bad("acc without out_init (the accumulate operand is the raw tensor's previous contents)");
+    if (p->lens)
+        for (int b = 0; b < B; b++)
+            if (p->lens[b] < 0 || p->lens[b] > T) return bad("lens outside [0, T]");
+    ConvDesc d1[N], d2[N];
+    std::vector<float> arena;
+    const TestPack o = sx_test_pack(SxPack::F16X2);
+    std::string e;
+    for (int q = 0; q < N && e.empty(); q++) {
+        e = pack_test_conv(p->w1[q], p->b1[q], C, C, K, p->dil1[q], p->dil1[q] * (K - 1) / 2, 3, &d1[q], &arena, o);
+        if (e.empty()) e = pack_test_conv(p->w2[q], p->b2[q], C, C, K, p->dil2[q], p->dil2[q] * (K - 1) / 2, 3, &d2[q], &arena, o);
+    }
+    if (!e.empty()) return fail(nullptr, VITS_E_ARG, "%s", e.c_str());
+    int K1[N], dd1[N], K2[N], dd2[N];
+    bool can = true;
+    for (int q = 0; q < N; q++) {
+        can = can && d1[q].rawin && d2[q].rawin && d1[q].cfg == d1[0].cfg && d2[q].cfg == d1[0].cfg &&
+              sx_pair_supported(C, d1[q].cfg, d1[q].K, d1[q].dil, d2[q].K, d2[q].dil);
+        K1[q] = d1[q].K, dd1[q] = d1[q].dil, K2[q] = d2[q].K, dd2[q] = d2[q].dil;
+    }
+    if (!can || !sx_pair_steps_supported(C, d1[0].cfg, N, K1, dd1, K2, dd2, T))
+        return fail(nullptr, VITS_E_ARG, "these steps cannot run as one launch (C %d, kernel %d)", C, K);
+    const size_t n = (size_t)B * C * T;
+    std::vector<int> l32(B);
+    for (int b = 0; b < B; b++) l32[b] = p->lens ? (int)p->lens[b] : T;
+    DevBufs D;
+    float *dA = D.up(arena.data(), arena.size());
+    float *dx = D.up(p->x, n, 16);
+    float *dxr = D.alloc<float>(n, 16);
+    float *dimg = p->out_init ? D.up(p->out_init, n, 16) : D.fill<float>(n, 0, 16);
+    float *draw = D.alloc<float>(n, 16), *dref = D.alloc<float>(n, 16);
+    float *dtmp[2] = {D.fill<float>(n, 0, 16), D.fill<float>(n, 0, 16)};
+    float *dout = D.alloc<float>(n, 16);
+    int *dlen = p->lens ? D.up(l32.data(), (size_t)B) : nullptr;
+    const size_t npk = (size_t)kSxPeakSlots * kSxPeakStride;
+    unsigned *dpk = D.fill<unsigned>(npk), *dpk_ref = D.fill<unsigned>(npk);
+    TCHECK(D.err);
+    const dim3 grid((T + 255) / 256, C / 8, B);
+    sx_block_kernel<<<grid, 256>>>(dx, (int64_t)C * T, T, nullptr, dxr, C, T);
+    sx_block_kernel<<<grid, 256>>>(dimg, (int64_t)C * T, T, nullptr, draw, C, T);
+    sx_block_kernel<<<grid, 256>>>(dimg, (int64_t)C * T, T, nullptr, dref, C, T);
+    TCHECK(hipGetLastError());
+    const int kflags = ((p->flags & VITS_PAIR_EPI_ACC) ? EPI_ACC : 0) | ((p->flags & VITS_PAIR_EPI_DIV) ? EPI_DIV : 0);
+    const SxRagged rag = dlen ? SxRagged{dlen, 0, 1} : SxRagged{nullptr, 0, 0};
+    const float div = p->div == 0.f ? 1.f : p->div;
+    const SxPairArgs a = sx_pair_steps_args(d1, d2, N, dA, dA, dxr, T, draw, kflags, div, p->slope, rag, dpk);
+    auto fused = [&] { return launch_conv_sx_pair_steps(a, d1[0].cfg, B, nullptr); };
+    auto three = [&] {
+        const float *cur = dxr;
+        for (int q = 0; q < N; q++) {
+            float *dst = q == N - 1 ? dref : dtmp[q & 1];
+            const SxPairArgs s = sx_pair_args(d1[q], d2[q], dA, dA, cur, T, dst, q == N - 1 ? kflags : 0, div, p->slope, rag, dpk_ref);
+            if (hipError_t le = launch_conv_sx_pair(s, d1[q].cfg, B, nullptr); le != hipSuccess) return le;
+            cur = dst;
+        }
+        return hipSuccess;
+    };
+    const bool name_was_on = g_launch_name_on;
+    g_launch_name_on = true;
+    g_launch_name[0] = 0;
+    const hipError_t le = fused();
+    g_launch_name_on = name_was_on;
+    if (le != hipSuccess) return fail(nullptr, VITS_E_DEVICE, "pair steps hook: launch_conv_sx_pair_steps: %s", hipGetErrorString(le));
+    TCHECK(hipDeviceSynchronize());
+    std::snprintf(p->kernel, sizeof p->kernel, "%s", g_launch_name);
+    TCHECK(three());
+    TCHECK(hipDeviceSynchronize());
+    SxPairStepsGeom g;
+    sx_pair_steps_geom(C, N, K1, dd1, K2, dd2, &g);
+    p->BNo = g.BNo;
+    float *const src[2] = {draw, dref}, *const dst[2] = {p->out, p->out_ref};
+    unsigned *const pks[2] = {dpk, dpk_ref};
+    float *const pko[2] = {&p->peak, &p->peak_ref};
+    for (int i = 0; i < 2; i++) {
+        sx_unblock_kernel<<<grid, 256>>>(src[i], nullptr, dout, C, T, 1);
+        TCHECK(hipGetLastError());
+        TCHECK(hipDeviceSynchronize());
+        TCHECK(download(dst[i], dout, n));
+        std::vector<unsigned> slots(npk);
+        TCHECK(download(slots.data(), pks[i], slots.size()));
+        unsigned top = 0;
+        for (int s = 0; s < kSxPeakSlots; s++) top = std::max(top, slots[(size_t)s * kSxPeakStride]);
+        std::memcpy(pko[i], &top, 4);
+    }
+    if (p->ms_out) TCHECK(time_launches(10, fused, p->ms_out));
+    if (p->ms_ref_out) TCHECK(time_launches(10, three, p->ms_ref_out));
+    return VITS_OK;
+}
+
 static inline void split_identity_one(float x, uint16_t *o, uint16_t *f) {
     const float v = std::fmin(std::fmax(x, -kF16Max), kF16Max);
     const _Float16 h0 = (_Float16)v;
```

Result: no change. 145.1 million, median of 6 (+0.4%).
